# ocean1100/stereo_match

Hardware: AMD Instinct MI355X
Metric: stereo pairs/sec + Mpix·disp/sec, KITTI 1242×375 D=128 SGM, 1/2/4/8 GPU (higher is better)
Workload: dtype u8

## Files before the change

stereo_match_amd/csrc/sm_api.hip:

```cpp
#include <hip/hip_runtime.h>

#include <algorithm>
#include <cmath>
#include <cstdarg>
#include <cstdio>
#include <cstring>
#include <string>
#include <thread>
#include <type_traits>
#include <vector>

#include "../../include/stereo_match_amd.h"
#include "sm_cost.hpp"
#include "sm_paths.hpp"
#include "sm_post.hpp"
#include "sm_wls.hpp"
#include "sm_speckle.hpp"
#include "sm_reproject.hpp"
#include "sm_rectify.hpp"
#include "sm_nlm.hpp"
#include "sm_cloud.hpp"
#include "sm_bm.hpp"
#include "sm_wide.hpp"
#include "sm_sweep_host.hpp"
// ... 311 lines not shown
        return SM_OK;
    }
    int finish()
    {
        HIP_TRY(ctx, hipStreamSynchronize(ctx->stream));
        for (const Out& o : outs) std::memcpy(o.dst, (const uint8_t*)ctx->pin + o.off, o.bytes);
        return SM_OK;
    }
};
inline size_t stage_bytes(size_t bytes, int n = 1) { return (size_t)n * ((bytes + 255) & ~size_t(255)); }

int grid_for(size_t n)
{
    size_t g = (n + 255) / 256;
    return (int)std::min<size_t>(std::max<size_t>(g, 1), 8192);
}

size_t elem_bytes(const Norm& n) { return n.cost == SM_COST_CENSUS ? 1 : 2; }

const int kVdx[6] = {1, 0, -1, 1, 0, -1};
enum { DIRS_ALL = 0, DIRS_EW = 1, DIRS_EW_UP = 2 };
const int kVdy[6] = {1, 1, 1, -1, -1, -1};

constexpr size_t kRowLds = 65536;
constexpr size_t kSetBudget = size_t(32) << 30;
constexpr int kMaxGroup = 16;
bool sweep_fit_variant(sm_ctx* ctx, const Norm& n, int mode, int variant, struct SweepFit& f);
int sweep_min_pairs(sm_ctx* ctx, const Norm& n);
constexpr size_t kMallBudget = size_t(224) << 20;
constexpr int kMallMinPairs = 3;

struct Src {
    const uint8_t* L = nullptr;
    const uint8_t* R = nullptr;
    size_t pair_stride = 0;
    const float* vol = nullptr;
    size_t vol_pair = 0;
    float offset = 0.f, scale = 1.f;
    Src advance(int i) const
    {
        Src s = *this;
        if (L) s.L += (size_t)i * pair_stride;
        if (R) s.R += (size_t)i * pair_stride;
        if (vol) s.vol += (size_t)i * vol_pair;
        return s;
    }
};

int hybrid_slots(const Norm& n);

struct Geo {
    int H, W, stride, G;
    size_t vol, slot_bytes, L_pair, census_pair, cost_pair;
    bool sweep;
    bool lines;
    bool hybrid;
};

bool row_mode(const sm_ctx* ctx, const Norm& n)
{
    return SM_ABLATIONS && (ctx->dbg_flags & DBG_ROW) && n.D % 64 == 0 && n.D == n.Dv;
}
bool overlap(const sm_ctx* ctx) { return (ctx->dbg_flags & DBG_OVERLAP) != 0; }
bool use_cost8(const sm_ctx* ctx, const Norm& n)
{
    return n.cost == SM_COST_CENSUS && !(ctx->dbg_flags & DBG_NO_C8) && n.D <= 256;
}
hipStream_t stream_b(const sm_ctx* ctx)
{
    return ctx->wta_override ? ctx->wta_override : overlap(ctx) ? ctx->side : ctx->stream;
}

template <int DPLV, bool CENSUS, int VL, bool H16 = false>
int launch_paths_t(sm_ctx* ctx, const Norm& n, const Geo& g, BufSet& bs, int dirset)
{
    using LT = typename std::conditional<CENSUS, uint8_t, uint16_t>::type;
    constexpr int D = 16 * DPLV;
    constexpr bool WIDE = D % 64 == 0 && !H16;
    constexpr int LANESH = WIDE ? 64 : 16;
    constexpr int DPLH = D / LANESH;
    smk::PathsArgs pa{};
    pa.cl = (const uint64_t*)bs.census[0].p;
    pa.cr = (const uint64_t*)bs.census[1].p;
    pa.census_pair = g.census_pair;
    pa.cost = (const uint16_t*)bs.cost.p;
    pa.cost_pair = g.cost_pair;
    pa.cost8 = nullptr;
    if (use_cost8(ctx, n)) {
        pa.cost8 = (const uint8_t*)bs.cost.p;
        pa.cost_pair = g.vol;
    }
    pa.L = (uint8_t*)bs.L.p;
    pa.slot_bytes = g.slot_bytes;
    pa.L_pair_bytes = g.L_pair;
    pa.H = g.H;
    pa.W = g.W;
    pa.width1 = n.width1;
    pa.D = n.D;
    pa.minD = n.minD;
    pa.minX1 = n.minX1;
    pa.P1 = n.P1;
    pa.P2 = n.P2;
    pa.dbg = ctx->dbg_flags;
    const int lines_per_wg = 4 * (64 / LANESH);
    pa.hblocks = row_mode(ctx, n) ? 0 : (g.H + lines_per_wg - 1) / lines_per_wg;
    pa.nv = dirset == DIRS_ALL ? n.ndirs - 2 : dirset == DIRS_EW ? 0 : 3;
    const int k0 = dirset == DIRS_EW_UP ? 3 : 0;
    int blocks = 0;
    constexpr int LPWV = 64 / VL;
    for (int k = 0; k < pa.nv; k++) {
        const int dx = kVdx[k0 + k];
        pa.v_dx[k] = dx;
        pa.v_dy[k] = kVdy[k0 + k];
        pa.v_slot[k] = 2 + k;
        pa.v_line_lo[k] = dx > 0 ? -(g.H - 1) : 0;
        pa.v_nlines[k] = dx == 0 ? n.width1 : n.width1 + g.H - 1;
        pa.v_blk_start[k] = blocks;
        blocks += ((pa.v_nlines[k] + 8 * LPWV - 1) / (8 * LPWV)) * 2;
    }
    for (int k = pa.nv; k <= 6; k++) pa.v_blk_start[k] = blocks;
    dim3 grid(2 * pa.hblocks + blocks, g.G);
    if (ctx->fb_guard) {
        pa.guard = ctx->fb_guard;
        pa.nblocks = (int)grid.x;
        pa.npairs = g.G;
        grid = dim3(std::min<unsigned>(grid.x * g.G, 128u), 1);
    }
    StageTimer t(ctx, ctx->stream,
                 ctx->fb_guard ? SM_STAGE_FALLBACK : dirset == DIRS_EW ? SM_STAGE_HORIZONTAL : SM_STAGE_PATHS, g.G);
    if (ctx->fb_guard)
        hipLaunchKernelGGL((smk::k_sgm_paths<VL, DPLV * 16 / VL, LANESH, DPLH, CENSUS, LT, true>), grid, dim3(256), 0,
                           ctx->stream, pa);
    else
        hipLaunchKernelGGL((smk::k_sgm_paths<VL, DPLV * 16 / VL, LANESH, DPLH, CENSUS, LT>), grid, dim3(256), 0,
                           ctx->stream, pa);
    HIP_TRY(ctx, hipGetLastError());
    return SM_OK;
}

#ifndef WTA_NT
#define WTA_NT 1024
#endif
template <int DPLV, bool CENSUS>
int launch_wta_t(sm_ctx* ctx, const Norm& n, const Geo& g, BufSet& bs)
{
    using LT = typename std::conditional<CENSUS, uint8_t, uint16_t>::type;
    StageTimer t(ctx, stream_b(ctx), ctx->fb_guard ? SM_STAGE_FALLBACK : SM_STAGE_WTA, g.G);
#if SM_ABLATIONS
    constexpr int D = 16 * DPLV;
    if constexpr (D % 64 == 0) {
        if (row_mode(ctx, n) && !ctx->fb_guard) {
            if (ctx->wta_dst) return fail(ctx, SM_E_UNSUPPORTED, "the row-WTA ablation has no WTA-index output");
            smk::RowArgs ra{};
            ra.cl = (const uint64_t*)bs.census[0].p;
            ra.cr = (const uint64_t*)bs.census[1].p;
            ra.census_pair = g.census_pair;
            ra.cost = (const uint16_t*)bs.cost.p;
            ra.cost_pair = g.cost_pair;
            ra.L = (uint8_t*)bs.L.p;
            ra.slot_bytes = g.slot_bytes;
            ra.L_pair_bytes = g.L_pair;
            ra.H = g.H;
            ra.W = g.W;
            ra.width1 = n.width1;
            ra.D = n.D;
            ra.minD = n.minD;
            ra.minX1 = n.minX1;
            ra.P1 = n.P1;
            ra.P2 = n.P2;
            ra.uniq = n.uniq;
            ra.disp12 = n.disp12;
            ra.store_w = (ctx->dbg_flags & DBG_STORE_W) ? 1 : 0;
            ra.disp = (int16_t*)bs.raw.p;
            const size_t smem = (1024 + (size_t)g.W * 6 + 15) & ~size_t(15);
            if (n.ndirs == 8)
                hipLaunchKernelGGL((smk::k_row_wta<D / 64, 8, CENSUS, LT>), dim3(g.H, g.G), dim3(64), smem, stream_b(ctx), ra);
            else
                hipLaunchKernelGGL((smk::k_row_wta<D / 64, 5, CENSUS, LT>), dim3(g.H, g.G), dim3(64), smem, stream_b(ctx), ra);
            HIP_TRY(ctx, hipGetLastError());
            return SM_OK;
        }
    }
#endif
    smk::WtaArgs wa{};
    wa.L = (const uint8_t*)bs.L.p;
    wa.slot_bytes = g.slot_bytes;
    wa.L_pair_bytes = g.L_pair;
    const bool part_only = g.lines && !ctx->fb_guard;
    wa.nslots = part_only ? 0 : g.hybrid ? hybrid_slots(n) : n.ndirs;
    wa.part = (g.hybrid || part_only) ? (const uint16_t*)bs.part.p : nullptr;
    wa.part_pair = g.vol;
    wa.H = g.H;
    wa.W = g.W;
    wa.width1 = n.width1;
    wa.D = n.D;
    wa.Dv = n.Dv;
    wa.minD = n.minD;
    wa.minX1 = n.minX1;
    wa.uniq = n.uniq;
    wa.disp12 = n.disp12;
    wa.disp = (int16_t*)bs.raw.p;
    wa.wta = ctx->wta_dst;
    wa.lane8 = n.ndirs == 5;
    wa.skip = ctx->fb_guard ? nullptr : ctx->wta_skip;
    dim3 grid(g.H, g.G);
    const size_t smem = (size_t)g.W * (ctx->wta_dst ? 10 : 8) + 16;
    if (smem > kRowLds)
        return fail(ctx, SM_E_UNSUPPORTED, "width %d: the WTA row kernel's %zu B of LDS exceed %zu%s", g.W, smem,
                    kRowLds, ctx->wta_dst ? " (with the WTA index output)" : "");
    if (ctx->fb_guard) {
        wa.guard = ctx->fb_guard;
        wa.fallbacks = (uint32_t*)ctx->sweep_err.p + ERR_FALLBACKS;
        wa.npairs = g.G;
        grid = dim3(std::min(g.H * g.G, 64), 1);
    }
    if (ctx->fb_guard)
        hipLaunchKernelGGL((smk::k_wta<DPLV, LT, 1024, true>), grid, dim3(1024), smem, stream_b(ctx), wa);
    else if (wa.nslots == 0 && wa.part)
        hipLaunchKernelGGL((smk::k_wta<DPLV, LT, WTA_NT, false, DPLV % 2 == 0>), grid, dim3(WTA_NT), smem, stream_b(ctx),
                           wa);
    else
        hipLaunchKernelGGL((smk::k_wta<DPLV, LT, WTA_NT>), grid, dim3(WTA_NT), smem, stream_b(ctx), wa);
    HIP_TRY(ctx, hipGetLastError());
    return SM_OK;
}

template <int DPLV, bool CENSUS>
int launch_paths_dpl(sm_ctx* ctx, const Norm& n, const Geo& g, BufSet& bs, int dirset)
{
    if constexpr ((16 * DPLV) % 64 == 0) {
        if (ctx->dbg_flags & DBG_H64) {
            if (DPLV == 8 && !(ctx->dbg_flags & DBG_VL16))
                return launch_paths_t<DPLV, CENSUS, 8>(ctx, n, g, bs, dirset);
            return launch_paths_t<DPLV, CENSUS, 16>(ctx, n, g, bs, dirset);
        }
    }
    if constexpr (DPLV == 8) {
        if (!(ctx->dbg_flags & DBG_VL16)) return launch_paths_t<DPLV, CENSUS, 8, true>(ctx, n, g, bs, dirset);
    }
    return launch_paths_t<DPLV, CENSUS, 16, true>(ctx, n, g, bs, dirset);
}

enum { DISPATCH_PATHS = 0, DISPATCH_WTA = 1, DISPATCH_HORIZONTAL = 2, DISPATCH_HYBRID = 3 };

int dispatch(sm_ctx* ctx, const Norm& n, const Geo& g, BufSet& bs, int what)
{
    const bool census = n.cost == SM_COST_CENSUS;
    const int h = what == DISPATCH_HORIZONTAL ? DIRS_EW : what == DISPATCH_HYBRID ? DIRS_EW_UP : DIRS_ALL;
    switch (n.dpl) {
#define CASE(k)                                                                                               \
    case k:                                                                                                   \
        if (what == DISPATCH_WTA)                                                                             \
            return census ? launch_wta_t<k, true>(ctx, n, g, bs) : launch_wta_t<k, false>(ctx, n, g, bs);     \
        return census ? launch_paths_dpl<k, true>(ctx, n, g, bs, h) : launch_paths_dpl<k, false>(ctx, n, g, bs, h);
        CASE(1) CASE(2) CASE(3) CASE(4) CASE(5) CASE(6) CASE(7) CASE(8)
        CASE(9) CASE(10) CASE(11) CASE(12) CASE(13) CASE(14) CASE(15) CASE(16)
#undef CASE
    default: return fail(ctx, SM_E_UNSUPPORTED, "numDisparities %d not built", n.D);
    }
}

int ensure_event(sm_ctx* ctx, hipEvent_t& e);
bool use_sweep(const sm_ctx* ctx, const Norm& n, int H);

int hybrid_slots(const Norm& n) { return n.ndirs == 8 ? 5 : 2; }

bool use_hybrid(const sm_ctx* ctx, const Norm& n, int H)
{
    if (!SM_ABLATIONS || (n.ndirs != 8 && n.ndirs != 5) || !(ctx->dbg_flags & DBG_HYBRID) ||
        (ctx->dbg_flags & (DBG_LEGACY | DBG_SWEEP8)))
        return false;
    sm_ctx tmp = *ctx;
    tmp.dbg_flags = (ctx->dbg_flags & ~DBG_HYBRID) | DBG_SWEEP8;
    return use_sweep(&tmp, n, H);
}

bool use_sweep(const sm_ctx* ctx, const Norm& n, int H)
{
    if (ctx->dbg_flags & (DBG_LEGACY | DBG_ROW)) return false;
    if (n.cost == SM_COST_CENSUS && !use_cost8(ctx, n)) return false;
    const int cmax = n.cost == SM_COST_CENSUS ? 64 : n.cost == SM_COST_VOLUME ? smk::VOL_CMAX : 0;
    if (cmax + n.P2 > 16383) return false;
    if (H > 65535 || n.width1 <= 0) return false;
    const size_t W = (size_t)(n.maxX1 - std::min(n.minD, 0));
    if (W * 6 + 16 > kRowLds) return false;
    return (uint64_t)H * n.width1 * n.D * 2 <= smk::kMaxRecords;
}

struct SweepJob {
    const uint8_t* cost;
    size_t cost_pair;
    const uint8_t* ew;
    size_t ew_pair, ew_slot;
    uint16_t* part;
    size_t part_pair;
    uint32_t* key2;
    uint32_t* pre;
    uint32_t* err;
    int G;
    uint8_t* st = nullptr;
    size_t st_pair = 0;
    int ewarm = 0;
    int ewguess = 0;
    int nband = 1, band_h = 0, vwarm = 0, vguess = 0;
    uint8_t* vst = nullptr;
    size_t vst_pair = 0;
};

int stream_cus(hipStream_t st, int ncu)
{
    uint32_t mask[32] = {0};
    const uint32_t words = (uint32_t)std::min(32, (ncu + 31) / 32);
    if (hipExtStreamGetCUMask(st, words, mask) != hipSuccess) return ncu;
    int c = 0;
    for (uint32_t i = 0; i < words; i++) c += __builtin_popcount(mask[i]);
    return c > 0 ? std::min(c, ncu) : ncu;
}

int ensure_sweep_err(sm_ctx* ctx)
{
    if (ctx->sweep_err.p) return SM_OK;
    int rc = ensure(ctx, ctx->sweep_err, SWEEP_STATS ? (size_t(8) << 20) : 256);
    if (rc != SM_OK) return rc;
    HIP_TRY(ctx, hipMemsetAsync(ctx->sweep_err.p, 0, SWEEP_STATS ? (size_t(8) << 20) : 256, ctx->stream));
    return SM_OK;
}

int sweep_variant(const sm_ctx* ctx)
{
    if (SM_ABLATIONS && (ctx->dbg_flags & DBG_SWEEP_V2)) return 6;
    if (SM_ABLATIONS && (ctx->dbg_flags & DBG_SWEEP2_NW)) return 3;
    return (ctx->dbg_flags & DBG_NARROW_SWEEPS) ? 1 : 0;
}

struct SweepFit {
    smk::SweepInfo si{};
    int nwg = 0, cap = 0, ncu = 0;
};
bool sweep_fit_variant(sm_ctx* ctx, const Norm& n, int mode, int variant, SweepFit& f)
{
    if (smk::sweep_info(n.D, (int)elem_bytes(n), mode, variant, ctx->device, &f.si) != hipSuccess) return false;
    int ncu = 0;
    if (hipDeviceGetAttribute(&ncu, hipDeviceAttributeMultiprocessorCount, ctx->device) != hipSuccess) return false;
    f.ncu = stream_cus(ctx->stream, std::max(ncu, 1));
    const int per_cu = f.si.blocks_per_cu >= 3 ? f.si.blocks_per_cu - 1 : std::max(f.si.blocks_per_cu, 1);
    f.cap = per_cu * f.ncu;
    f.nwg = (n.width1 + f.si.cw - 1) / f.si.cw;
    return f.nwg <= f.cap;
}

int sweep_min_pairs(sm_ctx* ctx, const Norm& n)
{
    if (n.cost != SM_COST_CENSUS) return 3;
    SweepFit f;
    if (!sweep_fit_variant(ctx, n, 2, 0, f) || f.nwg <= 0) return 7;
    return std::max(2, std::min(7, (200 + f.nwg - 1) / f.nwg));
}

double sweep_model(const SweepFit& f, int G)
{
    const int per_launch = std::max(1, std::min(G, f.cap / std::max(f.nwg, 1)));
    const int launches = (G + per_launch - 1) / per_launch;
    const int per_cu = (per_launch * f.nwg + f.ncu - 1) / std::max(f.ncu, 1);
    return (double)launches * per_cu * (f.si.threads / 64 - 1) * std::max(f.si.dpl, 1);
}

bool sweep_capacity(sm_ctx* ctx, const Norm& n, int mode, int G, SweepFit& f)
{
    if (ctx->tune_sweep_ncw && sweep_variant(ctx) <= 1) {
        for (int v : {0, 1, 2}) {
            SweepFit t;
            if (sweep_fit_variant(ctx, n, mode, v, t) && t.si.ncw == ctx->tune_sweep_ncw) {
                f = t;
                return true;
            }
        }
        return false;
    }
    const int variant = sweep_variant(ctx);
    if (!sweep_fit_variant(ctx, n, mode, variant, f)) {
        if (!(variant == 0 && f.si.impl == 1 && sweep_fit_variant(ctx, n, mode, 1, f))) return false;
    } else if (variant == 0 && f.si.impl == 1 && G > 0 && !(ctx->dbg_flags & DBG_WIDE_SWEEPS)) {
        SweepFit nf;
        if (sweep_fit_variant(ctx, n, mode, 1, nf) && sweep_model(nf, G) < sweep_model(f, G)) f = nf;
    }
    if (variant == 0 && G > 0 && !(ctx->dbg_flags & DBG_WIDE_SWEEPS)) {
        SweepFit lf;
        if (sweep_fit_variant(ctx, n, mode, 2, lf) && sweep_model(lf, G) < sweep_model(f, G)) f = lf;
    }
    return true;
}

bool sweeps_fit(sm_ctx* ctx, const Norm& n, bool hybrid, bool lines = false)
{
    const int m8[2] = {0, 2}, m5[1] = {1}, mh[1] = {0}, l8[2] = {3, 4}, l5[1] = {3};
    const int* modes = hybrid ? mh : lines ? (n.ndirs == 8 ? l8 : l5) : n.ndirs == 8 ? m8 : m5;
    const int count = !hybrid && n.ndirs == 8 ? 2 : 1;
    for (int k = 0; k < count; k++) {
        SweepFit f;
        if (!sweep_capacity(ctx, n, modes[k], 0, f)) return false;
        if (lines && modes[k] == 3 && f.nwg > smk::patch_max_strips(n.D)) return false;
        if (lines && modes[k] == 3 && f.si.ncw < 11) return false;
    }
    return true;
}

int sweep_pass(sm_ctx* ctx, const Norm& n, const Geo& g, const SweepJob& j, int mode)
{
    SweepFit f;
    const bool banded = j.nband > 1;
    if (banded ? !(sweep_fit_variant(ctx, n, mode, 0, f) && f.si.impl == 1) : !sweep_capacity(ctx, n, mode, j.G, f)) {
        if (f.nwg > f.cap)
            return fail(ctx, SM_E_UNSUPPORTED, "sweep: %d strips exceed %d resident workgroups", f.nwg, f.cap);
        return fail(ctx, SM_E_UNSUPPORTED, "sweep: numDisparities %d not built", n.D);
    }
    const smk::SweepInfo& si = f.si;
    const int nwg = f.nwg, cap = f.cap;
    const int nb = banded ? j.nband : 1;
    const int nblk = banded ? (j.band_h + j.vwarm + si.hb - 1) / si.hb : (g.H + si.hb - 1) / si.hb;
    const int per_launch = (ctx->dbg_flags & DBG_SWEEP1) ? 1 : std::max(1, std::min(j.G, cap / (nwg * nb)));
    const size_t hop_pair = (size_t)nwg * nb * 2 * nblk * si.ngr;
    const size_t hop_bytes = hop_pair * 8 * per_launch;
    if (hop_pair * 8 > smk::kMaxRecords) return fail(ctx, SM_E_UNSUPPORTED, "sweep: boundary buffer too large");
    int rc;
    if (ctx->hop.n < hop_bytes || !ctx->hop.p) {
        if ((rc = ensure(ctx, ctx->hop, hop_bytes)) != SM_OK) return rc;
        HIP_TRY(ctx, hipMemsetAsync(ctx->hop.p, 0, ctx->hop.n, ctx->stream));
        ctx->hop_epoch = 0;
    }
    if ((rc = ensure_sweep_err(ctx)) != SM_OK) return rc;
    for (int p0 = 0; p0 < j.G; p0 += per_launch) {
        const int np = std::min(per_launch, j.G - p0);
        if (++ctx->hop_epoch > 0xFFFFu) {
            HIP_TRY(ctx, hipMemsetAsync(ctx->hop.p, 0, ctx->hop.n, ctx->stream));
            ctx->hop_epoch = 1;
        }
        smk::SweepArgs a{};
        a.cost = j.cost + (size_t)p0 * j.cost_pair;
        a.cost_pair = j.cost_pair;
        a.ew = j.ew ? j.ew + (size_t)p0 * j.ew_pair : nullptr;
        a.ew_pair = j.ew_pair;
        a.ew_slot = j.ew_slot;
        a.part = j.part ? (uint16_t*)((uint8_t*)j.part + (size_t)p0 * j.part_pair) : nullptr;
        a.part_pair = j.part_pair;
        a.hop = (unsigned long long*)ctx->hop.p;
        a.hop_pair = hop_pair;
        a.st = j.st ? j.st + (size_t)p0 * j.st_pair : nullptr;
        a.st_pair = j.st_pair;
        a.ewarm = j.ewarm;
        a.ewguess = j.ewguess;
        a.nband = nb;
        a.band_h = j.band_h;
        a.vwarm = j.vwarm;
        a.vguess = j.vguess;
        a.hop_nblk = nblk;
        a.vst = j.vst ? j.vst + (size_t)p0 * j.vst_pair : nullptr;
        a.vst_pair = j.vst_pair;
        if (ctx->tune_sweep_xcd > 0) {
            a.xcd_total = np * nwg * nb;
            a.xcd_per = (a.xcd_total + 7) / 8;
        }
        a.rec = j.key2 ? j.key2 + (size_t)p0 * g.H * g.W : nullptr;
        a.nb = j.pre ? j.pre + (size_t)p0 * g.H * g.W : nullptr;
        a.err = j.err;
        a.H = g.H;
        a.W = g.W;
        a.W1 = n.width1;
        a.D = n.D;
        a.Dv = n.Dv;
        a.minD = n.minD;
        a.minX1 = n.minX1;
        a.P1 = n.P1;
        a.P2 = n.P2;
        a.uniq = n.uniq;
        a.inv_ku = n.uniq < 100 ? 1.0f / (float)(100 - n.uniq) : 0.f;
        a.nwg = nwg;
        a.epoch = ctx->hop_epoch;
#if SWEEP_STATS
        a.stats = (unsigned long long*)((char*)ctx->sweep_err.p + 1024);
#endif
        a.dbg = (ctx->dbg_flags >> 24) & 7;
        HIP_TRY(ctx, smk::sweep_launch(n.D, (int)elem_bytes(n), mode, si.impl, a, np, ctx->stream));
    }
    return SM_OK;
}

struct StreamSwap {
    sm_ctx* c;
    hipStream_t old;
    StreamSwap(sm_ctx* c_, hipStream_t s) : c(c_), old(c_->stream) { c->stream = s; }
    ~StreamSwap() { c->stream = old; }
};

int ew_lanes(const sm_ctx* ctx, const Norm& n)
{
    if (ctx->tune_ew_lanes) return ctx->tune_ew_lanes;
    if (ctx->dbg_flags & DBG_OLD_EW) return -1;
    if (n.D % 64 == 0) return 32;
    if (n.D % 32 == 0) return 16;
    return elem_bytes(n) == 1 ? 0 : -1;
}

int launch_ew(sm_ctx* ctx, const Norm& n, const Geo& g, BufSet& bs)
{
    const size_t et = elem_bytes(n);
    const int vl = ew_lanes(ctx, n);
    if (vl < 0) return dispatch(ctx, n, g, bs, DISPATCH_HORIZONTAL);
    smk::EwArgs a{};
    a.cost = (const uint8_t*)bs.cost.p;
    a.cost_pair = g.vol * et;
    a.out = (uint8_t*)bs.L.p;
    a.out_pair = g.L_pair;
    a.out_slot = g.slot_bytes;
    a.H = g.H;
    a.W1 = n.width1;
    a.P1 = n.P1;
    a.P2 = n.P2;
    a.wpb = ctx->tune_ew_waves;
    a.prio = ctx->tune_ew_prio;
    StageTimer t(ctx, ctx->stream, SM_STAGE_HORIZONTAL, g.G);
    const hipError_t e = smk::ew_launch(n.D, (int)et, vl, a, g.G, ctx->stream);
    if (e == hipErrorInvalidValue) return fail(ctx, SM_E_UNSUPPORTED, "E/W lines: numDisparities %d not built", n.D);
    HIP_TRY(ctx, e);
    return SM_OK;
}

int run_sweep(sm_ctx* ctx, const Norm& n, const Geo& g, BufSet& bs, hipStream_t wta_stream, uint32_t* err)
{
    const int G = g.G;
    int rc;
    const size_t et = elem_bytes(n);
    SweepJob j{};
    j.cost = (const uint8_t*)bs.cost.p;
    j.cost_pair = g.vol * et;
    j.ew = (const uint8_t*)bs.L.p;
    j.ew_pair = g.L_pair;
    j.ew_slot = g.slot_bytes;
    j.G = G;
    if ((rc = ensure(ctx, bs.key2, (size_t)G * g.H * g.W * 4)) != SM_OK) return rc;
    if ((rc = ensure(ctx, bs.pre, (size_t)G * g.H * g.W * 4)) != SM_OK) return rc;
    j.key2 = (uint32_t*)bs.key2.p;
    j.pre = (uint32_t*)bs.pre.p;
    j.err = err;
    {
        StageTimer t(ctx, ctx->stream, SM_STAGE_PATHS, G);
        if (n.ndirs == 8) {
            if ((rc = ensure_event(ctx, ctx->ev_fork)) != SM_OK) return rc;
            if ((rc = ensure_event(ctx, ctx->ev_join)) != SM_OK) return rc;
            HIP_TRY(ctx, hipEventRecord(ctx->ev_fork, ctx->stream));
            if ((rc = ensure(ctx, bs.part, (size_t)G * g.vol * 2)) != SM_OK) return rc;
            j.part = (uint16_t*)bs.part.p;
            j.part_pair = g.vol * 2;
            {
                StageTimer ts(ctx, ctx->stream, SM_STAGE_SWEEP, G);
                if ((rc = sweep_pass(ctx, n, g, j, 0)) != SM_OK) return rc;
            }
            HIP_TRY(ctx, hipStreamWaitEvent(ctx->side, ctx->ev_fork, 0));
            const hipStream_t main = ctx->stream;
            ctx->stream = ctx->side;
            rc = launch_ew(ctx, n, g, bs);
            ctx->stream = main;
            if (rc != SM_OK) return rc;
            HIP_TRY(ctx, hipEventRecord(ctx->ev_join, ctx->side));
            HIP_TRY(ctx, hipStreamWaitEvent(ctx->stream, ctx->ev_join, 0));
        } else if ((rc = launch_ew(ctx, n, g, bs)) != SM_OK) {
            return rc;
        }
    }
    if (wta_stream != ctx->stream) {
        HIP_TRY(ctx, hipEventRecord(bs.paths_done, ctx->stream));
        HIP_TRY(ctx, hipStreamWaitEvent(wta_stream, bs.paths_done, 0));
    }
    StreamSwap sw(ctx, wta_stream);
    StageTimer t(ctx, ctx->stream, SM_STAGE_WTA, G);
    StageTimer ts(ctx, ctx->stream, SM_STAGE_SWEEP_WTA, G);
    return sweep_pass(ctx, n, g, j, n.ndirs == 8 ? 2 : 1);
}

int sweep_finish(sm_ctx* ctx, const Norm& n, const Geo& g, BufSet& bs, hipStream_t ws, uint32_t* gflag)
{
    const bool fb = !(ctx->dbg_flags & DBG_NO_FALLBACK);
    int rc;
    if (fb && ws != ctx->stream) {
        if (ctx->dbg_flags & DBG_FORCE_FALLBACK) HIP_TRY(ctx, hipMemsetAsync(gflag, 1, 1, ws));
        HIP_TRY(ctx, smk::lr_rows_launch((const uint32_t*)bs.key2.p, (const uint32_t*)bs.pre.p, (int16_t*)bs.raw.p,
                                         ctx->wta_dst, g.G, g.H, g.W, n.Dv, n.minD, n.minX1, n.maxX1, n.disp12,
                                         gflag, ws));
        StreamSwap sw(ctx, ws);
        ctx->wta_override = ws;
        ctx->fb_guard = gflag;
        rc = dispatch(ctx, n, g, bs, DISPATCH_PATHS);
        if (rc == SM_OK) rc = dispatch(ctx, n, g, bs, DISPATCH_WTA);
        ctx->fb_guard = nullptr;
        ctx->wta_override = nullptr;
        return rc;
    }
    hipStream_t fs = ctx->side;
    if (fb) {
        if (ctx->dbg_flags & DBG_FORCE_FALLBACK) HIP_TRY(ctx, hipMemsetAsync(gflag, 1, 1, ws));
        if ((rc = ensure_event(ctx, ctx->ev_fb_fork)) != SM_OK) return rc;
        if ((rc = ensure_event(ctx, ctx->ev_fb_join)) != SM_OK) return rc;
        HIP_TRY(ctx, hipEventRecord(ctx->ev_fb_fork, ws));
        HIP_TRY(ctx, hipStreamWaitEvent(fs, ctx->ev_fb_fork, 0));
        StreamSwap sw(ctx, fs);
        ctx->wta_override = fs;
        ctx->fb_guard = gflag;
        rc = dispatch(ctx, n, g, bs, DISPATCH_PATHS);
        if (rc == SM_OK) rc = dispatch(ctx, n, g, bs, DISPATCH_WTA);
        ctx->fb_guard = nullptr;
        ctx->wta_override = nullptr;
        if (rc != SM_OK) return rc;
        HIP_TRY(ctx, hipEventRecord(ctx->ev_fb_join, fs));
    }
    HIP_TRY(ctx, smk::lr_rows_launch((const uint32_t*)bs.key2.p, (const uint32_t*)bs.pre.p, (int16_t*)bs.raw.p,
                                     ctx->wta_dst, g.G, g.H, g.W, n.Dv, n.minD, n.minX1, n.maxX1, n.disp12,
                                     fb ? gflag : nullptr, ws));
    if (fb) HIP_TRY(ctx, hipStreamWaitEvent(ws, ctx->ev_fb_join, 0));
    return SM_OK;
}

bool use_lines(sm_ctx* ctx, const Norm& n)
{
    if (ctx->tune_sweep_lines < 0 || ctx->tune_ew_lanes || (ctx->dbg_flags & DBG_OLD_EW)) return false;
    return sweeps_fit(ctx, n, false, true);
}

int ew_warmup(const sm_ctx* ctx, const Norm& n)
{
    if (ctx->tune_ew_warmup > 0) return ctx->tune_ew_warmup;
    (void)n;
    return 16;
}

long long path_max(const Norm& n)
{
    if (n.cost == SM_COST_CENSUS) return 62 + n.P2;
    if (n.cost == SM_COST_VOLUME) return smk::VOL_CMAX + n.P2;
    const long long side = 2 * (n.bs / 2) + 1;
    return side * side * (2 * n.ftzero + (255 >> 2)) + n.P2;
}

int line_bands(const sm_ctx* ctx, const Norm& n, int H, int G)
{
    if (n.ndirs != 5 || ctx->tune_bands == 1 || 5 * path_max(n) > 65535) return 1;
    SweepFit f;
    if (!sweep_fit_variant(const_cast<sm_ctx*>(ctx), n, 3, 0, f) || f.si.impl != 1 || f.nwg <= 0) return 1;
    int nb = ctx->tune_bands >= 2 ? ctx->tune_bands : std::min(f.cap / std::max(1, G * f.nwg), H / 24);
    nb = std::min(nb, H);
    if (nb < 2) return 1;
    const int bh = (H + nb - 1) / nb;
    return (H + bh - 1) / bh;
}

int band_warmup(const sm_ctx* ctx, const Norm& n)
{
    if (ctx->tune_band_warmup > 0) return ctx->tune_band_warmup;
    return elem_bytes(n) == 1 ? 16 : 24;
}

int run_lines(sm_ctx* ctx, const Norm& n, const Geo& g, BufSet& bs, hipStream_t ws, uint32_t* gflag)
{
    const int G = g.G;
    const size_t et = elem_bytes(n);
    int rc;
    SweepJob j{};
    j.cost = (const uint8_t*)bs.cost.p;
    j.cost_pair = g.vol * et;
    j.G = G;
    j.err = gflag;
    if ((rc = ensure(ctx, bs.part, (size_t)G * g.vol * 2)) != SM_OK) return rc;
    j.part = (uint16_t*)bs.part.p;
    j.part_pair = g.vol * 2;
    SweepFit f;
    j.nband = line_bands(ctx, n, g.H, G);
    if (j.nband > 1 ? !sweep_fit_variant(ctx, n, 3, 0, f) : !sweep_capacity(ctx, n, 3, G, f))
        return fail(ctx, SM_E_UNSUPPORTED, "sweep lines: no instance fits");
    j.st_pair = ((size_t)g.H * f.nwg * 4 * n.D * et + 255) & ~size_t(255);
    if ((rc = ensure(ctx, bs.st, j.st_pair * G)) != SM_OK) return rc;
    j.st = (uint8_t*)bs.st.p;
    j.ewarm = ew_warmup(ctx, n);
    j.ewguess = ctx->tune_ew_guess;
    if (j.nband > 1 && ctx->tune_ew_warmup <= 0 && et == 2) j.ewarm = 54;
    if (j.nband > 1) {
        j.band_h = (g.H + j.nband - 1) / j.nband;
        j.vwarm = band_warmup(ctx, n);
        j.vguess = ctx->tune_band_guess;
        j.vst_pair = ((size_t)j.nband * 6 * n.width1 * n.D * et + 255) & ~size_t(255);
        if ((rc = ensure(ctx, bs.vst, j.vst_pair * G)) != SM_OK) return rc;
        j.vst = (uint8_t*)bs.vst.p;
        ctx->band_groups++;
    }
    ctx->line_groups++;
    ctx->line_strips += (long long)f.nwg * G;
    const bool fb_side = n.ndirs == 5 && ws == ctx->stream && !(ctx->dbg_flags & DBG_NO_FALLBACK);
    {
        StageTimer t(ctx, ctx->stream, SM_STAGE_PATHS, G);
        {
            StageTimer ts(ctx, ctx->stream, SM_STAGE_SWEEP, G);
            if ((rc = sweep_pass(ctx, n, g, j, 3)) != SM_OK) return rc;
        }
        if (ctx->sweep_done_ev) {
            HIP_TRY(ctx, hipEventRecord(ctx->sweep_done_ev, ctx->stream));
            ctx->sweep_done_hit = true;
        }
        smk::EwPatchArgs pa{};
        pa.cost = j.cost;
        pa.cost_pair = j.cost_pair;
        pa.part = j.part;
        pa.part_pair = j.part_pair * 1;
        pa.st = j.st;
        pa.st_pair = j.st_pair;
        pa.H = g.H;
        pa.W1 = n.width1;
        pa.nwg = f.nwg;
        pa.cw = f.si.cw;
        pa.P1 = n.P1;
        pa.P2 = n.P2;
        pa.guard = gflag;
        pa.fixes = reinterpret_cast<unsigned long long*>((uint32_t*)ctx->sweep_err.p + ERR_EW_REPAIRS);
        pa.atom = EW_PATCH_ATOM && et == 2 && 5 * path_max(n) < 65536 ? 1 : 0;
        auto ew_patch = [&](hipStream_t st) -> int {
            const hipError_t e = smk::ew_patch_launch(n.D, (int)et, pa, G, st);
            if (e == hipErrorInvalidValue) return fail(ctx, SM_E_UNSUPPORTED, "E/W patch: numDisparities %d not built", n.D);
            HIP_TRY(ctx, e);
            return SM_OK;
        };
        const bool ew_side = fb_side && pa.atom && j.nband > 1;
        if (fb_side) {
            if (ctx->dbg_flags & DBG_FORCE_FALLBACK) HIP_TRY(ctx, hipMemsetAsync(gflag, 1, 1, ctx->stream));
            if ((rc = ensure_event(ctx, ctx->ev_fb_fork)) != SM_OK) return rc;
            if ((rc = ensure_event(ctx, ctx->ev_fb_join)) != SM_OK) return rc;
            HIP_TRY(ctx, hipEventRecord(ctx->ev_fb_fork, ctx->stream));
            HIP_TRY(ctx, hipStreamWaitEvent(ctx->side, ctx->ev_fb_fork, 0));
            if (ew_side) {
                if ((rc = ensure_event(ctx, ctx->ev_ew_done)) != SM_OK) return rc;
                {
                    StageTimer th(ctx, ctx->side, SM_STAGE_HORIZONTAL, G);
                    if ((rc = ew_patch(ctx->side)) != SM_OK) return rc;
                }
                HIP_TRY(ctx, hipEventRecord(ctx->ev_ew_done, ctx->side));
            }
            StreamSwap sw(ctx, ctx->side);
            ctx->wta_override = ctx->side;
            ctx->fb_guard = gflag;
            rc = dispatch(ctx, n, g, bs, DISPATCH_PATHS);
            if (rc == SM_OK) rc = dispatch(ctx, n, g, bs, DISPATCH_WTA);
            ctx->fb_guard = nullptr;
            ctx->wta_override = nullptr;
            if (rc != SM_OK) return rc;
            HIP_TRY(ctx, hipEventRecord(ctx->ev_fb_join, ctx->side));
        }
        if (!ew_side) {
            StageTimer th(ctx, ctx->stream, SM_STAGE_HORIZONTAL, G);
            if ((rc = ew_patch(ctx->stream)) != SM_OK) return rc;
        }
        if (j.nband > 1) {
            smk::BandPatchArgs ba{};
            ba.cost = j.cost;
            ba.cost_pair = j.cost_pair;
            ba.part = j.part;
            ba.part_pair = j.part_pair;
            ba.vst = j.vst;
            ba.vst_pair = j.vst_pair;

            ba.H = g.H;
            ba.W1 = n.width1;
            ba.nband = j.nband;
            ba.band_h = j.band_h;
            ba.P1 = n.P1;
            ba.P2 = n.P2;
            ba.guard = gflag;
            ba.fixes = reinterpret_cast<unsigned long long*>((uint32_t*)ctx->sweep_err.p + ERR_BAND_REPAIRS);
            const hipError_t eb = smk::band_patch_launch(n.D, (int)et, ba, G, ctx->stream);
            if (eb == hipErrorInvalidValue) return fail(ctx, SM_E_UNSUPPORTED, "band patch: numDisparities %d not built", n.D);
            HIP_TRY(ctx, eb);
            if (ew_side) HIP_TRY(ctx, hipStreamWaitEvent(ctx->stream, ctx->ev_ew_done, 0));
        }
    }
    if (ws != ctx->stream) {
        HIP_TRY(ctx, hipEventRecord(bs.paths_done, ctx->stream));
        HIP_TRY(ctx, hipStreamWaitEvent(ws, bs.paths_done, 0));
    }
    if (n.ndirs == 8) {
        if ((rc = ensure(ctx, bs.key2, (size_t)G * g.H * g.W * 4)) != SM_OK) return rc;
        if ((rc = ensure(ctx, bs.pre, (size_t)G * g.H * g.W * 4)) != SM_OK) return rc;
        j.key2 = (uint32_t*)bs.key2.p;
        j.pre = (uint32_t*)bs.pre.p;
        {
            StreamSwap sw(ctx, ws);
            StageTimer t(ctx, ctx->stream, SM_STAGE_WTA, G);
            StageTimer ts(ctx, ctx->stream, SM_STAGE_SWEEP_WTA, G);
            if ((rc = sweep_pass(ctx, n, g, j, 4)) != SM_OK) return rc;
        }
        return sweep_finish(ctx, n, g, bs, ws, gflag);
    }
    StreamSwap sw(ctx, ws);
    ctx->wta_override = ws;
    {
        StageTimer ts(ctx, ws, SM_STAGE_SWEEP_WTA, G);
        ctx->wta_skip = fb_side ? gflag : nullptr;
        rc = dispatch(ctx, n, g, bs, DISPATCH_WTA);
        ctx->wta_skip = nullptr;
    }
    if (fb_side) {
        if (rc == SM_OK) HIP_TRY(ctx, hipStreamWaitEvent(ws, ctx->ev_fb_join, 0));
    } else if (rc == SM_OK && !(ctx->dbg_flags & DBG_NO_FALLBACK)) {
        if (ctx->dbg_flags & DBG_FORCE_FALLBACK) HIP_TRY(ctx, hipMemsetAsync(gflag, 1, 1, ws));
        ctx->fb_guard = gflag;
        rc = dispatch(ctx, n, g, bs, DISPATCH_PATHS);
        if (rc == SM_OK) rc = dispatch(ctx, n, g, bs, DISPATCH_WTA);
        ctx->fb_guard = nullptr;
    }
    ctx->wta_override = nullptr;
    return rc;
}

int run_hybrid(sm_ctx* ctx, const Norm& n, const Geo& g, BufSet& bs)
{
    const int G = g.G;
    int rc;
    SweepJob j{};
    j.cost = (const uint8_t*)bs.cost.p;
    j.cost_pair = g.vol * elem_bytes(n);
    j.G = G;
    if ((rc = ensure_sweep_err(ctx)) != SM_OK) return rc;
    j.err = (uint32_t*)ctx->sweep_err.p + ERR_STICKY;
    if ((rc = ensure(ctx, bs.part, (size_t)G * g.vol * 2)) != SM_OK) return rc;
    j.part = (uint16_t*)bs.part.p;
    j.part_pair = g.vol * 2;
    if ((rc = ensure_event(ctx, ctx->ev_fork)) != SM_OK) return rc;
    if ((rc = ensure_event(ctx, ctx->ev_join)) != SM_OK) return rc;
    StageTimer t(ctx, ctx->stream, SM_STAGE_PATHS, G);
    HIP_TRY(ctx, hipEventRecord(ctx->ev_fork, ctx->stream));
    HIP_TRY(ctx, hipStreamWaitEvent(ctx->side, ctx->ev_fork, 0));
    const hipStream_t main = ctx->stream;
    ctx->stream = ctx->side;
    {
        StageTimer ts(ctx, ctx->stream, SM_STAGE_SWEEP, G);
        rc = sweep_pass(ctx, n, g, j, 0);
    }
    ctx->stream = main;
    if (rc != SM_OK) return rc;
    HIP_TRY(ctx, hipEventRecord(ctx->ev_join, ctx->side));
    if ((rc = dispatch(ctx, n, g, bs, n.ndirs == 8 ? DISPATCH_HYBRID : DISPATCH_HORIZONTAL)) != SM_OK) return rc;
    HIP_TRY(ctx, hipStreamWaitEvent(ctx->stream, ctx->ev_join, 0));
    return SM_OK;
}

int check_sweep_errors(sm_ctx* ctx)
{
    if (ctx->twin) {
        int rc = check_sweep_errors(ctx->twin);
        if (rc != SM_OK) return fail(ctx, rc, "%s", ctx->twin->err.c_str());
    }
    if (!ctx->sweep_err.p) return SM_OK;
    uint32_t e = 0;
    uint32_t* w = (uint32_t*)ctx->sweep_err.p + ERR_STICKY;
    HIP_TRY(ctx, hipMemcpy(&e, w, 4, hipMemcpyDeviceToHost));
    if (e) {
        HIP_TRY(ctx, hipMemset(w, 0, 4));
        return fail(ctx, SM_E_HIP, "sweep: strip-boundary hand-off timed out (workgroups not co-resident?)");
    }
    return SM_OK;
}

int cost_nt(const Geo& g, size_t elem_bytes)
{
    return (size_t)g.G * g.vol * elem_bytes > ((size_t)224 << 20) ? 1 : 0;
}

#ifndef SGBM_COST2_WGS
#define SGBM_COST2_WGS 2048
#endif
template <int S, int CPT>
int launch_cost2_s(sm_ctx* ctx, const Norm& n, const Geo& g, const smk::SgbmCostArgs& sc)
{
    const int NP = n.D / 2, CG = std::max(1, 256 / NP), bd = NP * CG, TX = CG * CPT, NHC = TX + 2 * S;
    const int rpairs = TX + 2 * S + n.D - 1;
    if (NP > 256 || NHC > 4 * bd || rpairs > 4 * bd)
        return fail(ctx, SM_E_UNSUPPORTED, "sgbm cost: numDisparities %d not built", n.D);
    const bool one = NHC <= bd && rpairs <= bd;
    const int rph = (rpairs + 1) / 2;
    const size_t lds = (size_t)NHC * 16 + (size_t)((NHC + 1) & ~1) * 8 + (size_t)2 * rph * 24 + (size_t)2 * ((CG * ((NHC + CG - 1) / CG)) | 1) * NP * 4;
    smk::SgbmCost2Args c2{};
    c2.planes = sc.planes;
    c2.C = sc.C;
    c2.C_pair = sc.C_pair;
    c2.H = sc.H;
    c2.W = sc.W;
    c2.width1 = sc.width1;
    c2.D = sc.D;
    c2.minD = sc.minD;
    c2.minX1 = sc.minX1;
    c2.Yc = sc.Yc;
    c2.nt = cost_nt(g, 2);
    const int strips = (n.width1 + TX - 1) / TX;
    const int wgs = ctx->tune_cost_wgs > 0 ? ctx->tune_cost_wgs : SGBM_COST2_WGS;
    const int want = std::max(1, wgs / std::max(1, strips * g.G));
    c2.band = std::max({(sc.Yc + want - 1) / want, 8, 4 * S});
    const int bands = (sc.Yc + c2.band - 1) / c2.band;
    if (one)
        hipLaunchKernelGGL((smk::k_sgbm_cost2<S, CPT, 1>), dim3(strips, bands, g.G), dim3(bd), lds, ctx->stream, c2);
    else
        hipLaunchKernelGGL((smk::k_sgbm_cost2<S, CPT, 4>), dim3(strips, bands, g.G), dim3(bd), lds, ctx->stream, c2);
    HIP_TRY(ctx, hipGetLastError());
    return SM_OK;
}

int launch_sgbm_cost2(sm_ctx* ctx, const Norm& n, const Geo& g, const smk::SgbmCostArgs& sc)
{
    if (ctx->dbg_flags & DBG_COST_TILE) return SM_OK;
    switch (n.bs / 2) {
    case 0: return launch_cost2_s<0, 8>(ctx, n, g, sc);
    case 1: return launch_cost2_s<1, 8>(ctx, n, g, sc);
    case 2: return launch_cost2_s<2, 8>(ctx, n, g, sc);
    case 3: return launch_cost2_s<3, 8>(ctx, n, g, sc);
    case 4: return launch_cost2_s<4, 8>(ctx, n, g, sc);
    case 5: return launch_cost2_s<5, 8>(ctx, n, g, sc);
    default: return fail(ctx, SM_E_UNSUPPORTED, "blockSize %d not built", n.bs);
    }
}

int group_size(const sm_ctx* ctx, const Norm& n, int H, int npairs, bool sweep, bool hybrid)
{
    const size_t cells = (size_t)H * std::max(n.width1, 1) * n.D;
    const size_t per = sweep    ? cells * (n.ndirs * elem_bytes(n) + (n.ndirs == 8 ? 2 : 0))
                       : hybrid ? cells * (hybrid_slots(n) * elem_bytes(n) + 2)
                                : cells * elem_bytes(n) * n.ndirs;
    size_t g = std::max<size_t>(1, kSetBudget / std::max<size_t>(per, 1));
    const size_t half = overlap(ctx) ? std::max(1, (npairs + 1) / 2) : kMaxGroup;
    const int cap = (ctx->dbg_flags >> 16) & 7;
    if (cap) return (int)std::min<size_t>({g, (size_t)cap, half});
    g = std::min<size_t>({g, (size_t)kMaxGroup, half});
    if (!sweep && !hybrid && elem_bytes(n) == 1 && !(ctx->dbg_flags & DBG_NO_MALL_GROUPS)) {
        const size_t fit = kMallBudget / std::max<size_t>(cells, 1);
        const size_t ngroups = fit ? ((size_t)npairs + fit - 1) / fit : 0;
        if (fit >= (size_t)kMallMinPairs && fit < g && ngroups <= 2)
            g = std::max<size_t>(1, ((size_t)npairs + ngroups - 1) / ngroups);
    }
    return (int)g;
}

int ensure_event(sm_ctx* ctx, hipEvent_t& e)
{
    if (!e) HIP_TRY(ctx, hipEventCreateWithFlags(&e, hipEventDisableTiming));
    return SM_OK;
}

int run_speckles(sm_ctx* ctx, hipStream_t st, int16_t* img, int G, int H, int W, int newval, int maxsize,
                 int maxdiff)
{
    StageTimer t(ctx, st, SM_STAGE_SPECKLE, G);
    const size_t npx = (size_t)H * W;
    int rc;
    if ((rc = ensure(ctx, ctx->sp_parent, G * npx * 4)) != SM_OK) return rc;
    if ((rc = ensure(ctx, ctx->sp_count, G * npx * 4)) != SM_OK) return rc;
    smk::SpeckleArgs sa{};
    sa.img = img;
    sa.parent = (int*)ctx->sp_parent.p;
    sa.count = (int*)ctx->sp_count.p;
    sa.H = H;
    sa.W = W;
    sa.newval = newval;
    sa.maxsize = maxsize;
    sa.maxdiff = maxdiff;
    const dim3 grid((unsigned)((npx + 255) / 256), G);
    hipLaunchKernelGGL(smk::k_speckle_init, grid, dim3(256), 0, st, sa);
    hipLaunchKernelGGL(smk::k_speckle_union, grid, dim3(256), 0, st, sa);
    hipLaunchKernelGGL(smk::k_speckle_count, grid, dim3(256), 0, st, sa);
    hipLaunchKernelGGL(smk::k_speckle_apply, grid, dim3(256), 0, st, sa);
    HIP_TRY(ctx, hipGetLastError());
    return SM_OK;
}

int finish_group(sm_ctx* ctx, const Geo& g, const Norm& n, BufSet& bs, int s, int16_t* d_out, hipStream_t sb)
{
    const int H = g.H, W = g.W, G = g.G;
    int rc;
    {
        StageTimer t(ctx, sb, SM_STAGE_MEDIAN, G);
        hipLaunchKernelGGL(smk::k_median3, dim3((W + 255) / 256, H, G), dim3(256), 0, sb,
                           (const int16_t*)bs.raw.p, d_out, H, W, (size_t)H * W);
        HIP_TRY(ctx, hipGetLastError());
    }
    if (n.speckle_ws > 0) {
        if ((rc = run_speckles(ctx, sb, d_out, G, H, W, (n.minD - 1) * 16, n.speckle_ws, 16 * n.speckle_range)) !=
            SM_OK)
            return rc;
    }
    if (sb != ctx->stream) {
        HIP_TRY(ctx, hipEventRecord(bs.wta_done, sb));
        bs.pending = true;
    }
    ctx->last_width1 = n.width1;
    ctx->last_index = G - 1;
    ctx->last_L_pair = g.L_pair;
    ctx->last_set = s;
    return SM_OK;
}

template <int DPL>
int wide_paths_wta(sm_ctx* ctx, const Geo& g, const Norm& n, BufSet& bs)
{
    smk::WidePathArgs pa{};
    pa.C = (const int16_t*)bs.cost.p;
    pa.vol = g.vol;
    pa.L = (uint8_t*)bs.L.p;
    pa.slot_bytes = g.slot_bytes;
    pa.L_pair_bytes = g.L_pair;
    pa.H = g.H;
    pa.width1 = n.width1;
    pa.D = n.D;
    pa.P1 = n.P1;
    pa.P2 = n.P2;
    pa.ndirs = n.ndirs;
    const int dys[8] = {0, 0, 1, 1, 1, -1, -1, -1}, dxs[8] = {1, -1, 1, 0, -1, 1, 0, -1};
    int blocks = 0;
    for (int k = 0; k < n.ndirs; k++) {
        pa.blk_start[k] = blocks;
        const int nl = dys[k] == 0 ? g.H : dxs[k] == 0 ? n.width1 : n.width1 + g.H - 1;
        blocks += (nl + 15) / 16;
    }
    for (int k = n.ndirs; k <= 8; k++) pa.blk_start[k] = blocks;
// ... 2383 lines not shown
```

stereo_match_amd/csrc/sm_ew.hpp:

```cpp
#pragma once
#include "sm_pk.hpp"
#include "sm_sweep_host.hpp"

namespace smk {

#ifndef SWEEP_STREAM_AUX
#define SWEEP_STREAM_AUX 2
#endif
#ifndef EW_H16
#define EW_H16 1
#endif
#ifndef EW_STEPN
#define EW_STEPN 1
#endif

template <int VL, int NP, typename CT, typename LT, int PF>
__global__ void __launch_bounds__(256) k_ew(EwArgs a)
{
    constexpr int LPW = 64 / VL, DPL = 2 * NP, D = VL * DPL;
    constexpr int CB = DPL * (int)sizeof(CT);
    switch (a.prio) {
    case 1: __builtin_amdgcn_s_setprio(1); break;
    case 2: __builtin_amdgcn_s_setprio(2); break;
    case 3: __builtin_amdgcn_s_setprio(3); break;
    default: break;
    }
    const int lane = threadIdx.x & 63, wave = threadIdx.x >> 6;
    const int g = lane % VL, kl = lane / VL;
    const int dir = (int)blockIdx.x >= a.nrb ? 1 : 0;
    const int H = a.H, W1 = a.W1;
    const int y0 = (((int)blockIdx.x - dir * a.nrb) * a.wpb + wave) * LPW;
    if (y0 >= H) return;
    const bool line_ok = y0 + kl < H;
    const int y = min(y0 + kl, H - 1);
    const size_t pair = blockIdx.y;
    const uint64_t cells = (uint64_t)H * W1 * D;
    const rsrc_t rc = make_rsrc(a.cost + pair * a.cost_pair, cells * sizeof(CT));
    const rsrc_t ro = make_rsrc(a.out + pair * a.out_pair + (size_t)dir * a.out_slot, cells * sizeof(LT));
    const uint32_t estep = dir ? (uint32_t)(-D) : (uint32_t)D;
    uint32_t e = ((uint32_t)y * (uint32_t)W1 + (uint32_t)(dir ? W1 - 1 : 0)) * (uint32_t)D + (uint32_t)(g * DPL);
    const uint32_t P1p = (uint32_t)a.P1 * 0x10001u, P2p = (uint32_t)a.P2 * 0x10001u;
    constexpr bool H16 = sizeof(CT) == 1 && EW_H16;
    constexpr uint32_t EDGE = H16 ? 0x7BFF7BFFu : (kBig | (kBig << 16));
    const uint32_t eL = g == 0 ? EDGE : 0u, eR = g == VL - 1 ? EDGE : 0u;

    RawBytes<CB> ring[PF];
#pragma unroll
    for (int k = 0; k < PF; k++) {
        ring[k].load(rc, k < W1 ? (e + (uint32_t)k * estep) * (uint32_t)sizeof(CT) : kOOB);
        asm volatile("" ::: "memory");
    }
    uint32_t Lp[NP];
#pragma unroll
    for (int k = 0; k < NP; k++) Lp[k] = 0;
    uint32_t minLp = 0;
    for (int s0 = 0; s0 < W1; s0 += PF) {
#pragma unroll
        for (int k = 0; k < PF; k++) {
            const int s = s0 + k;
#pragma unroll
            for (int j = 0; j < RawBytes<CB>::WORDS; j++) asm volatile("" : "+v"(ring[k].w[j]) : "v"(minLp));
            uint32_t C[NP];
            unpack_ct_pk<CT, DPL>(ring[k], C);
#pragma unroll
            for (int i = 0; i < NP; i++) asm volatile("" : "+v"(C[i])::"memory");
            ring[k].load(rc, s + PF < W1 ? (e + (uint32_t)PF * estep) * (uint32_t)sizeof(CT) : kOOB);
            uint32_t Ln[NP], mn;
            if constexpr (EW_STEPN) {
                uint32_t Lp1[1][NP], m1[1] = {minLp}, C1[1][NP], Ln1[1][NP], mn1[1];
#pragma unroll
                for (int i = 0; i < NP; i++) {
                    Lp1[0][i] = Lp[i];
                    C1[0][i] = C[i];
                }
                sweep_step2n<VL, NP, H16, 1>(Lp1, m1, C1, P1p, P2p, eL, eR, Ln1, mn1);
#pragma unroll
                for (int i = 0; i < NP; i++) Ln[i] = Ln1[0][i];
                mn = mn1[0];
            } else {
                mn = sweep_step2<VL, NP, H16>(Lp, minLp, C, P1p, P2p, eL, eR, Ln);
            }
            store_pk<LT, NP, SWEEP_STREAM_AUX>(ro, (line_ok && s < W1) ? e * (uint32_t)sizeof(LT) : kOOB, Ln);
            e += estep;
#pragma unroll
            for (int i = 0; i < NP; i++) Lp[i] = Ln[i];
            minLp = mn;
        }
    }
}

#ifndef EW_PATCH_NO_CARRY
#define EW_PATCH_NO_CARRY 0
#endif
#ifndef EW_PATCH_B64
#define EW_PATCH_B64 1
#endif
#ifndef EW_PATCH_RC
#define EW_PATCH_RC 0
#endif
template <int VL, int NP, typename CT, bool ATOM = false>
__global__ void __launch_bounds__(256) k_ew_patch(EwPatchArgs a)
{
    constexpr int LPW = 64 / VL, DPL = 2 * NP, D = VL * DPL;
    constexpr int CB = DPL * (int)sizeof(CT);
    constexpr bool H16 = sizeof(CT) == 1 && EW_H16;
    constexpr bool SAT = sizeof(CT) == 2;
    constexpr uint32_t EDGE = H16 ? 0x7BFF7BFFu : (kBig | (kBig << 16));
    constexpr int KU = 8;
    constexpr int CHUNK = LPW * KU;
    constexpr int RC = EW_PATCH_RC ? EW_PATCH_RC : sizeof(CT) == 1 ? 8 : 16;
    if (a.guard && __hip_atomic_load(a.guard, __ATOMIC_RELAXED, __HIP_MEMORY_SCOPE_AGENT) != 0u) return;
    const int lane = threadIdx.x & 63, wave = threadIdx.x >> 6;
    const int g = lane % VL, kl = lane / VL;
    const int yw = (int)blockIdx.x * 4 + wave;
    const int y = ATOM ? yw >> 1 : yw;
    const int dir0 = ATOM ? (yw & 1) : 0, dir1 = ATOM ? dir0 + 1 : 2;
    const size_t pair = blockIdx.y;
    const int H = a.H, W1 = a.W1, nwg = a.nwg, CW = a.cw;
    if (y >= H) return;
    const uint64_t cells = (uint64_t)H * W1 * D;
    const rsrc_t rc = make_rsrc(a.cost + pair * a.cost_pair, cells * sizeof(CT));
    const rsrc_t rp = make_rsrc((const uint8_t*)a.part + pair * a.part_pair, cells * 2);
    uint32_t* const pw = reinterpret_cast<uint32_t*>((uint8_t*)a.part + pair * a.part_pair);
    auto atom_add = [&](uint32_t word, uint32_t first, uint32_t second) {
        const int lo = (int)(second & 0xFFFFu) - (int)(first & 0xFFFFu);
        const int hi = (int)(second >> 16) - (int)(first >> 16);
        const uint32_t add = (uint32_t)(hi * 65536 + lo);
        if (add) __hip_atomic_fetch_add(pw + word, add, __ATOMIC_RELAXED, __HIP_MEMORY_SCOPE_AGENT);
    };
    const rsrc_t rs = make_rsrc(a.st + pair * a.st_pair, a.st_pair);
    const uint32_t P1p = (uint32_t)a.P1 * 0x10001u, P2p = (uint32_t)a.P2 * 0x10001u;
    const uint32_t eL = g == 0 ? EDGE : 0u, eR = g == VL - 1 ? EDGE : 0u;
    auto soff = [&](int k, int dir, int which) -> uint32_t {
        return (((((uint32_t)y * (uint32_t)nwg + (uint32_t)k) * 2u + (uint32_t)dir) * 2u + (uint32_t)which) *
                    (uint32_t)D + (uint32_t)(g * DPL)) * (uint32_t)sizeof(CT);
    };
    auto cell = [&](int c) -> uint32_t { return ((uint32_t)y * (uint32_t)W1 + (uint32_t)c) * (uint32_t)D + (uint32_t)(g * DPL); };
    auto line_all = [&](bool ok) -> bool { return group_min<VL>(ok ? 1u : 0u) != 0u; };
    auto same_state = [&](const uint32_t (&x)[NP], const uint32_t (&z)[NP]) -> bool {
        bool ok = true;
#pragma unroll
        for (int i = 0; i < NP; i++) ok &= x[i] == z[i];
        return line_all(ok);
    };
    auto state_min = [&](const uint32_t (&x)[NP]) -> uint32_t {
        uint32_t m = x[0];
#pragma unroll
        for (int i = 1; i < NP; i++) m = pk_min(m, x[i]);
        m = ::min(m & 0xFFFFu, m >> 16);
        return group_min<VL>(m) * 0x10001u;
    };
    auto load_state = [&](uint32_t off, uint32_t (&v)[NP]) {
        RawBytes<CB> b;
        b.load(rs, off);
        unpack_ct_pk<CT, DPL>(b, v);
    };
    auto walk = [&](int k, int dir, uint32_t aoff, uint32_t toff, uint32_t (&T)[NP], bool check) -> int {
        const int x0 = k * CW, ncol = ::min(CW, W1 - x0);
        RawBytes<CB> cc[RC];
        RawBytes<DPL * 2> pb[RC];
        auto issue1 = [&](int u, int o) {
            const int c = dir ? x0 + CW - 1 - o : x0 + o;
            cc[u].load(rc, o < ncol ? cell(c) * (uint32_t)sizeof(CT) : kOOB);
            if constexpr (!ATOM) pb[u].load(rp, o < ncol ? cell(c) * 2u : kOOB);
        };
        auto issue = [&](int o0) {
#pragma unroll
            for (int u = 0; u < RC; u++) issue1(u, o0 + u);
        };
        issue(0);
        uint32_t A[NP];
        load_state(aoff, A);
        if (toff != kOOB) load_state(toff, T);
        if (check && same_state(A, T)) return 2;
        uint32_t Lq[2][NP], mq[2];
#pragma unroll
        for (int q = 0; q < NP; q++) {
            Lq[0][q] = A[q];
            Lq[1][q] = T[q];
        }
        mq[0] = state_min(Lq[0]);
        mq[1] = state_min(Lq[1]);
        bool met = false;
        for (int o0 = 0; o0 < ncol && !met; o0 += RC) {
            if (o0 > 0) issue(o0);
#pragma unroll
            for (int u = 0; u < RC; u++) {
                const int o = o0 + u;
                if (o >= ncol || met) continue;
                const int c = dir ? x0 + CW - 1 - o : x0 + o;
                uint32_t C2[2][NP], Ln[2][NP], mn[2], pv_[NP];
                unpack_ct_pk<CT, DPL>(cc[u], C2[0]);
#pragma unroll
                for (int q = 0; q < NP; q++) pv_[q] = ATOM ? 0u : pb[u].w[q];
#pragma unroll
                for (int q = 0; q < NP; q++) C2[1][q] = C2[0][q];
                sweep_step2n<VL, NP, H16, 2>(Lq, mq, C2, P1p, P2p, eL, eR, Ln, mn);
                if (same_state(Ln[0], Ln[1])) {
                    met = true;
                    continue;
                }
                if constexpr (ATOM) {
#pragma unroll
                    for (int q = 0; q < NP; q++) atom_add(cell(c) / 2u + (uint32_t)q, Ln[0][q], Ln[1][q]);
                }
                uint32_t P[NP];
#pragma unroll
                for (int q = 0; q < NP && !ATOM; q++) {
                    if constexpr (SAT) {
                        const uint32_t pv = pv_[q];
                        const uint32_t x = pk_adds(pk_sub(pv, Ln[0][q]), Ln[1][q]);
                        const uint32_t sat = pk_sub(pk_min(pk_add(pv, 0x00010001u), 0x00010001u), 0x00010001u);
                        P[q] = pkw(__builtin_elementwise_max(pkv(x), pkv(sat)));
                    } else {
                        P[q] = pk_add(pk_sub(pv_[q], Ln[0][q]), Ln[1][q]);
                    }
                }
                if constexpr (!ATOM) bstore_n<uint32_t, NP>(rp, cell(c) * 2u, P);
#pragma unroll
                for (int q = 0; q < NP; q++) {
                    Lq[0][q] = Ln[0][q];
                    Lq[1][q] = Ln[1][q];
                }
                mq[0] = mn[0];
                mq[1] = mn[1];
            }
        }
        if (!met) {
#pragma unroll
            for (int q = 0; q < NP; q++) T[q] = pk_sub(Lq[1][q], mq[1]);
        }
        return met ? 1 : 0;
    };
    constexpr int DPLW = D % 128 == 0 ? D / 64 : 2, NPW = DPLW / 2;
    constexpr int CBW = DPLW * (int)sizeof(CT);
    auto soff64 = [&](int k, int dir, int which) -> uint32_t {
        return (((((uint32_t)y * (uint32_t)nwg + (uint32_t)k) * 2u + (uint32_t)dir) * 2u + (uint32_t)which) *
                    (uint32_t)D + (uint32_t)(lane * DPLW)) * (uint32_t)sizeof(CT);
    };
    auto cell64 = [&](int c) -> uint32_t {
        return ((uint32_t)y * (uint32_t)W1 + (uint32_t)c) * (uint32_t)D + (uint32_t)(lane * DPLW);
    };
    auto load_state64 = [&](uint32_t off, uint32_t (&v)[NPW]) {
        RawBytes<CBW> b;
        b.load(rs, off);
        unpack_ct_pk<CT, DPLW>(b, v);
    };
    auto same_state64 = [&](const uint32_t (&x)[NPW], const uint32_t (&z)[NPW]) -> bool {
        bool ok = true;
#pragma unroll
        for (int i = 0; i < NPW; i++) ok &= x[i] == z[i];
        return __all(ok);
    };
    auto state_min64 = [&](const uint32_t (&x)[NPW]) -> uint32_t {
        uint32_t m = x[0];
#pragma unroll
        for (int i = 1; i < NPW; i++) m = pk_min(m, x[i]);
        m = ::min(m & 0xFFFFu, m >> 16);
        return Line<64>::min(m) * 0x10001u;
    };
    auto walk64 = [&](int k, int dir, uint32_t aoff, uint32_t toff, uint32_t (&T)[NPW], bool check) -> int {
        const int x0 = k * CW, ncol = ::min(CW, W1 - x0);
        RawBytes<CBW> cc[RC];
        RawBytes<DPLW * 2> pb[RC];
        auto issue1 = [&](int u, int o) {
            const int c = dir ? x0 + CW - 1 - o : x0 + o;
            cc[u].load(rc, o < ncol ? cell64(c) * (uint32_t)sizeof(CT) : kOOB);
            if constexpr (!ATOM) pb[u].load(rp, o < ncol ? cell64(c) * 2u : kOOB);
        };
        auto issue = [&](int o0) {
#pragma unroll
            for (int u = 0; u < RC; u++) issue1(u, o0 + u);
        };
        issue(0);
        uint32_t A[NPW];
        load_state64(aoff, A);
        if (toff != kOOB) load_state64(toff, T);
        if (check && same_state64(A, T)) return 2;
        uint32_t Lq[2][NPW], mq[2];
#pragma unroll
        for (int q = 0; q < NPW; q++) {
            Lq[0][q] = A[q];
            Lq[1][q] = T[q];
        }
        mq[0] = state_min64(Lq[0]);
        mq[1] = state_min64(Lq[1]);
        bool met = false;
        for (int o0 = 0; o0 < ncol && !met; o0 += RC) {
            if (o0 > 0) issue(o0);
#pragma unroll
            for (int u = 0; u < RC; u++) {
                const int o = o0 + u;
                if (o >= ncol || met) continue;
                const int c = dir ? x0 + CW - 1 - o : x0 + o;
                uint32_t C2[2][NPW], Ln[2][NPW], mn[2], pv_[NPW];
                unpack_ct_pk<CT, DPLW>(cc[u], C2[0]);
#pragma unroll
                for (int q = 0; q < NPW; q++) pv_[q] = ATOM ? 0u : pb[u].w[q];
#pragma unroll
                for (int q = 0; q < NPW; q++) C2[1][q] = C2[0][q];
                sweep_step2n<64, NPW, H16, 2>(Lq, mq, C2, P1p, P2p, 0u, 0u, Ln, mn);
                if (same_state64(Ln[0], Ln[1])) {
                    met = true;
                    continue;
                }
                if constexpr (ATOM) {
#pragma unroll
                    for (int q = 0; q < NPW; q++) atom_add(cell64(c) / 2u + (uint32_t)q, Ln[0][q], Ln[1][q]);
                }
                uint32_t P[NPW];
#pragma unroll
                for (int q = 0; q < NPW && !ATOM; q++) {
                    if constexpr (SAT) {
                        const uint32_t pv = pv_[q];
                        const uint32_t x = pk_adds(pk_sub(pv, Ln[0][q]), Ln[1][q]);
                        const uint32_t sat = pk_sub(pk_min(pk_add(pv, 0x00010001u), 0x00010001u), 0x00010001u);
                        P[q] = pkw(__builtin_elementwise_max(pkv(x), pkv(sat)));
                    } else {
                        P[q] = pk_add(pk_sub(pv_[q], Ln[0][q]), Ln[1][q]);
                    }
                }
                if constexpr (!ATOM) bstore_n<uint32_t, NPW>(rp, cell64(c) * 2u, P);
#pragma unroll
                for (int q = 0; q < NPW; q++) {
                    Lq[0][q] = Ln[0][q];
                    Lq[1][q] = Ln[1][q];
                }
                mq[0] = mn[0];
                mq[1] = mn[1];
            }
        }
        if (!met) {
#pragma unroll
            for (int q = 0; q < NPW; q++) T[q] = pk_sub(Lq[1][q], mq[1]);
        }
        return met ? 1 : 0;
    };
    auto lines_or = [&](uint64_t v) -> uint64_t {
        uint64_t m = 0;
#pragma unroll
        for (int l = 0; l < LPW; l++) {
            const uint32_t lo = __builtin_amdgcn_readlane((uint32_t)v, l * VL);
            const uint32_t hi = __builtin_amdgcn_readlane((uint32_t)(v >> 32), l * VL);
            m |= ((uint64_t)hi << 32) | lo;
        }
        return m;
    };
    auto order_partial = [&]() {
        __builtin_amdgcn_fence(__ATOMIC_RELEASE, "workgroup");
        __builtin_amdgcn_fence(__ATOMIC_ACQUIRE, "workgroup");
    };
    __shared__ uint64_t openm[4][kPatchMaxChunks];
    uint32_t nfix = 0, nopen = 0;
    for (int dir = dir0; dir < dir1; dir++) {
        auto strip_of = [&](int i) { return dir ? nwg - 1 - i : i; };
        int first_open = nwg;
        for (int i0 = 1, ch = 0; i0 < nwg; i0 += CHUNK, ch++) {
            RawBytes<CB> sb[KU], eb[KU];
#pragma unroll
            for (int u = 0; u < KU; u++) {
                const int i = i0 + kl + LPW * u;
                sb[u].load(rs, i < nwg ? soff(strip_of(i), dir, 0) : kOOB);
                eb[u].load(rs, i < nwg ? soff(strip_of(i - 1), dir, 1) : kOOB);
            }
            uint64_t bad = 0;
#pragma unroll
            for (int u = 0; u < KU; u++) {
                bool ok = true;
#pragma unroll
                for (int q = 0; q < RawBytes<CB>::WORDS; q++) ok &= sb[u].w[q] == eb[u].w[q];
                ok = line_all(ok);
                if (!ok && i0 + kl + LPW * u < nwg) bad |= 1ull << (kl + LPW * u);
            }
            const uint64_t m = lines_or(bad);
            uint64_t open = 0;
            uint64_t rest = m;
            while (rest) {
                int mine = -1;
#pragma unroll
                for (int l = 0; l < LPW; l++) {
                    if (rest && l == kl) mine = __builtin_ctzll(rest);
                    if (rest) rest &= rest - 1;
                }
                if (mine >= 0) {
                    const int i = i0 + mine, k = strip_of(i);
                    uint32_t T[NP];
                    nfix++;
                    if (walk(k, dir, soff(k, dir, 0), soff(strip_of(i - 1), dir, 1), T, false) == 0) {
                        store_pk<CT, NP>(rs, soff(k, dir, 0), T);
                        open |= 1ull << mine;
                    }
                }
            }
            open = lines_or(open);
            nopen += (uint32_t)__builtin_popcountll(open);
            if (lane == 0) openm[wave][ch] = open;
            if (open && first_open == nwg) first_open = i0 + __builtin_ctzll(open);
        }
        if (first_open < nwg && !EW_PATCH_NO_CARRY && D % 128 == 0 && EW_PATCH_B64) {
            order_partial();
            bool carry = false;
            uint32_t T[NPW];
#pragma unroll
            for (int q = 0; q < NPW; q++) T[q] = 0;
            for (int i = first_open; i < nwg; i++) {
                const int k = strip_of(i);
                if (carry) {
                    const int r = walk64(k, dir, soff64(strip_of(i - 1), dir, 1), kOOB, T, true);
                    nfix += r != 2 && kl == 0;
                    if (r != 0) carry = false;
                }
                const bool open_i = ((openm[wave][(i - 1) / CHUNK] >> ((i - 1) % CHUNK)) & 1ull) != 0;
                if (!carry && open_i) {
                    load_state64(soff64(k, dir, 0), T);
                    carry = true;
                }
            }
        } else if (first_open < nwg && !EW_PATCH_NO_CARRY) {
            order_partial();
            if (kl == 0) {
                bool carry = false;
                uint32_t T[NP];
#pragma unroll
                for (int q = 0; q < NP; q++) T[q] = 0;
                for (int i = first_open; i < nwg; i++) {
                    const int k = strip_of(i);
                    if (carry) {
                        const int r = walk(k, dir, soff(strip_of(i - 1), dir, 1), kOOB, T, true);
                        nfix += r != 2;
                        if (r != 0) carry = false;
                    }
                    const bool open_i = ((openm[wave][(i - 1) / CHUNK] >> ((i - 1) % CHUNK)) & 1ull) != 0;
                    if (!carry && open_i) {
                        load_state(soff(k, dir, 0), T);
                        carry = true;
                    }
                }
            }
        }
        if (!ATOM && dir == 0) order_partial();
    }
    if (a.fixes) {
        nfix = group_sum_u32_wave(g == 0 ? nfix : 0u);
        if (lane == 0 && nfix) atomicAdd(a.fixes, (unsigned long long)nfix);
        if (lane == 0 && nopen) atomicAdd(a.fixes + 1, (unsigned long long)nopen);
    }
}

template <int VL, int NP, typename CT>
__global__ void __launch_bounds__(256) k_band_patch(BandPatchArgs a)
{
    constexpr int LPW = 64 / VL, DPL = 2 * NP, D = VL * DPL, CB = DPL * (int)sizeof(CT);
    constexpr bool H16 = sizeof(CT) == 1 && EW_H16;
    constexpr uint32_t EDGE = H16 ? 0x7BFF7BFFu : (kBig | (kBig << 16));
    constexpr int RC = 8;
    if (a.guard && __hip_atomic_load(a.guard, __ATOMIC_RELAXED, __HIP_MEMORY_SCOPE_AGENT) != 0u) return;
    const int lane = threadIdx.x & 63, wave = threadIdx.x >> 6;
    const int g = lane % VL, kl = lane / VL;
    const int bi = (int)blockIdx.y + 1;
    const size_t pair = blockIdx.z;
    const int H = a.H, W1 = a.W1;
    const int y0 = bi * a.band_h;
    const int id = ((int)blockIdx.x * 4 + wave) * LPW + kl;
    const bool on = id < 3 * W1 && y0 < H;
    const int dir = on ? id / W1 : 0, x = on ? id % W1 : 0;
    const int dx = dir == 0 ? 0 : dir == 1 ? 1 : -1;
    const int nr = !on ? 0 : dx == 0 ? H - y0 : dx > 0 ? min(H - y0, W1 - 1 - x) : min(H - y0, x);
    const uint64_t cells = (uint64_t)H * W1 * D;
    const rsrc_t rc = make_rsrc(a.cost + pair * a.cost_pair, cells * sizeof(CT));
    const rsrc_t rv = make_rsrc(a.vst + pair * a.vst_pair, a.vst_pair);
    uint32_t* part = reinterpret_cast<uint32_t*>(reinterpret_cast<uint8_t*>(a.part) + pair * a.part_pair);
    const uint32_t P1p = (uint32_t)a.P1 * 0x10001u, P2p = (uint32_t)a.P2 * 0x10001u;
    const uint32_t eL = g == 0 ? EDGE : 0u, eR = g == VL - 1 ? EDGE : 0u;
    auto voff = [&](int band, int which, int col) -> uint32_t {
        return (((((uint32_t)band * 2u + (uint32_t)which) * 3u + (uint32_t)dir) * (uint32_t)W1 + (uint32_t)col) *
                    (uint32_t)D + (uint32_t)(g * DPL)) * (uint32_t)sizeof(CT);
    };
    auto cost_off = [&](int r) -> uint32_t {
        return r < nr ? (((uint32_t)(y0 + r) * (uint32_t)W1 + (uint32_t)(x + dx * (r + 1))) * (uint32_t)D +
                         (uint32_t)(g * DPL)) * (uint32_t)sizeof(CT)
                      : kOOB;
    };
    auto line_all = [&](bool ok) -> bool { return group_min<VL>(ok ? 1u : 0u) != 0u; };
    auto state_min = [&](const uint32_t (&v)[NP]) -> uint32_t {
        uint32_t m = v[0];
#pragma unroll
        for (int i = 1; i < NP; i++) m = pk_min(m, v[i]);
        m = ::min(m & 0xFFFFu, m >> 16);
        return group_min<VL>(m) * 0x10001u;
    };
    RawBytes<CB> sb, tb, cc[RC];
    sb.load(rv, on ? voff(bi, 0, x) : kOOB);
    tb.load(rv, on ? voff(bi - 1, 1, x) : kOOB);
#pragma unroll
    for (int u = 0; u < RC; u++) cc[u].load(rc, cost_off(u));
    uint32_t Lq[2][NP], mq[2];
    unpack_ct_pk<CT, DPL>(sb, Lq[0]);
    unpack_ct_pk<CT, DPL>(tb, Lq[1]);
    bool same = true;
#pragma unroll
    for (int i = 0; i < NP; i++) same &= Lq[0][i] == Lq[1][i];
    same = line_all(same);
    uint32_t nfix = 0, nlong = 0;
    if (on && !same && nr > 0) {
        nfix++;
        mq[0] = state_min(Lq[0]);
        mq[1] = state_min(Lq[1]);
        const int rb = min(H, y0 + a.band_h) - y0;
        bool met = false;
        int r0 = 0;
        for (; r0 < nr && !met; r0 += RC) {
            if (r0 > 0) {
#pragma unroll
                for (int u = 0; u < RC; u++) cc[u].load(rc, cost_off(r0 + u));
            }
#pragma unroll
            for (int u = 0; u < RC; u++) {
                const int r = r0 + u;
                if (r >= nr || met) continue;
                uint32_t C2[2][NP], Ln[2][NP], mn[2];
                unpack_ct_pk<CT, DPL>(cc[u], C2[0]);
#pragma unroll
                for (int q = 0; q < NP; q++) C2[1][q] = C2[0][q];
                sweep_step2n<VL, NP, H16, 2>(Lq, mq, C2, P1p, P2p, eL, eR, Ln, mn);
                bool eq = true;
#pragma unroll
                for (int q = 0; q < NP; q++) eq &= Ln[0][q] == Ln[1][q];
                if (line_all(eq)) {
                    met = true;
                    continue;
                }
                nlong |= r >= rb ? 1u : 0u;
                const size_t w0 = (((size_t)(y0 + r) * (size_t)W1 + (size_t)(x + dx * (r + 1))) * D + g * DPL) / 2;
#pragma unroll
                for (int q = 0; q < NP; q++) {
                    const int lo = (int)(Ln[1][q] & 0xFFFFu) - (int)(Ln[0][q] & 0xFFFFu);
                    const int hi = (int)(Ln[1][q] >> 16) - (int)(Ln[0][q] >> 16);
                    const uint32_t add = (uint32_t)(hi * 65536 + lo);
                    if (add) __hip_atomic_fetch_add(part + w0 + q, add, __ATOMIC_RELAXED, __HIP_MEMORY_SCOPE_AGENT);
                }
#pragma unroll
                for (int q = 0; q < NP; q++) {
                    Lq[0][q] = Ln[0][q];
                    Lq[1][q] = Ln[1][q];
                }
                mq[0] = mn[0];
                mq[1] = mn[1];
            }
        }
    }
    if (a.fixes) {
        nfix = group_sum_u32_wave(g == 0 ? nfix : 0u);
        nlong = group_sum_u32_wave(g == 0 ? nlong : 0u);
        if (lane == 0 && nfix) atomicAdd(a.fixes, (unsigned long long)nfix);
        if (lane == 0 && nlong) atomicAdd(a.fixes + 1, (unsigned long long)nlong);
    }
}

}
```

stereo_match_amd/csrc/sm_pk.hpp:

```cpp
#pragma once
#include "sm_common.hpp"

namespace smk {

template <int VL>
__device__ __forceinline__ uint32_t line_or(uint32_t v)
{
    v |= perm_dpp<DPP_QP_XOR1>(v);
    v |= perm_dpp<DPP_QP_XOR2>(v);
    v |= perm_dpp<DPP_ROW_HALF_MIRROR>(v);
    if constexpr (VL >= 16) v |= perm_dpp<DPP_ROW_MIRROR>(v);
    if constexpr (VL == 32) v = row_pair_combine(v, [](uint32_t a, uint32_t b) { return a | b; });
    return v;
}

template <int N>
__device__ __forceinline__ uint32_t group_min(uint32_t v)
{
    static_assert(N == 1 || N == 2 || N == 4 || N == 8 || N == 16 || N == 32, "lane group of 1-32 lanes");
    if constexpr (N >= 2) v = ::min(v, perm_dpp<DPP_QP_XOR1>(v));
    if constexpr (N >= 4) v = ::min(v, perm_dpp<DPP_QP_XOR2>(v));
    if constexpr (N >= 8) v = ::min(v, perm_dpp<DPP_ROW_HALF_MIRROR>(v));
    if constexpr (N >= 16) v = ::min(v, perm_dpp<DPP_ROW_MIRROR>(v));
    if constexpr (N >= 32) v = row_pair_combine(v, [](uint32_t a, uint32_t b) { return ::min(a, b); });
    return v;
}

template <int N>
__device__ __forceinline__ uint32_t group_sum(uint32_t v)
{
    static_assert(N == 1 || N == 2 || N == 4 || N == 8 || N == 16 || N == 32, "lane group of 1-32 lanes");
    if constexpr (N >= 2) v += perm_dpp<DPP_QP_XOR1>(v);
    if constexpr (N >= 4) v += perm_dpp<DPP_QP_XOR2>(v);
    if constexpr (N >= 8) v += perm_dpp<DPP_ROW_HALF_MIRROR>(v);
    if constexpr (N >= 16) v += perm_dpp<DPP_ROW_MIRROR>(v);
    if constexpr (N >= 32) v = row_pair_combine(v, [](uint32_t a, uint32_t b) { return a + b; });
    return v;
}

template <int N>
__device__ __forceinline__ uint32_t group_max(uint32_t v)
{
    static_assert(N == 1 || N == 2 || N == 4 || N == 8 || N == 16 || N == 32, "lane group of 1-32 lanes");
    if constexpr (N >= 2) v = ::max(v, perm_dpp<DPP_QP_XOR1>(v));
    if constexpr (N >= 4) v = ::max(v, perm_dpp<DPP_QP_XOR2>(v));
    if constexpr (N >= 8) v = ::max(v, perm_dpp<DPP_ROW_HALF_MIRROR>(v));
    if constexpr (N >= 16) v = ::max(v, perm_dpp<DPP_ROW_MIRROR>(v));
    if constexpr (N >= 32) v = row_pair_combine(v, [](uint32_t a, uint32_t b) { return ::max(a, b); });
    return v;
}

template <int VL, int DPL>
__device__ __forceinline__ uint32_t sweep_step(const uint32_t (&Lp)[DPL], uint32_t minLp, const uint32_t (&C)[DPL],
                                               uint32_t P1, uint32_t P2, uint32_t (&Ln)[DPL])
{
    const uint32_t lm = Line<VL>::prev(kBig, Lp[DPL - 1]);
    const uint32_t lq = Line<VL>::next(kBig, Lp[0]);
    const uint32_t delta = minLp + P2;
    uint32_t mn = 0xFFFFFFFFu;
#pragma unroll
    for (int i = 0; i < DPL; i++) {
        const uint32_t a1 = i == 0 ? lm : Lp[i - 1];
        const uint32_t a2 = i == DPL - 1 ? lq : Lp[i + 1];
        uint32_t v = min(min(a1, a2) + P1, Lp[i]);
        v = min(v, delta);
        Ln[i] = C[i] + v - minLp;
        mn = min(mn, Ln[i]);
    }
    return group_min<VL>(mn);
}

typedef unsigned short pk16 __attribute__((ext_vector_type(2)));
__device__ __forceinline__ pk16 pkv(uint32_t w) { return __builtin_bit_cast(pk16, w); }
__device__ __forceinline__ uint32_t pkw(pk16 v) { return __builtin_bit_cast(uint32_t, v); }
__device__ __forceinline__ uint32_t pk_min(uint32_t a, uint32_t b) { return pkw(__builtin_elementwise_min(pkv(a), pkv(b))); }
__device__ __forceinline__ uint32_t pk_add(uint32_t a, uint32_t b) { return pkw(pkv(a) + pkv(b)); }
__device__ __forceinline__ uint32_t pk_sub(uint32_t a, uint32_t b) { return pkw(pkv(a) - pkv(b)); }
__device__ __forceinline__ uint32_t pk_adds(uint32_t a, uint32_t b)
{
    return pkw(__builtin_elementwise_add_sat(pkv(a), pkv(b)));
}

__device__ __forceinline__ uint32_t pk_window_push(uint32_t u, uint32_t s)
{
    uint32_t r;
    asm("v_pk_mad_u16 %0, %1, -1, %2 clamp" : "=v"(r) : "v"(u), "v"(s));
    return r;
}

template <int VL, int NP>
__device__ __forceinline__ uint32_t sweep_step_pk(const uint32_t (&Lp)[NP], uint32_t minLp, const uint32_t (&C)[NP],
                                                  uint32_t P1p, uint32_t P2, uint32_t (&Ln)[NP])
{
    constexpr uint32_t EDGE = kBig | (kBig << 16);
    const uint32_t lm = Line<VL>::prev(EDGE, Lp[NP - 1]);
    const uint32_t lq = Line<VL>::next(EDGE, Lp[0]);
    const uint32_t mm = minLp * 0x10001u, dl = (minLp + P2) * 0x10001u;
    uint32_t mn = 0xFFFFFFFFu;
    uint32_t a1 = __builtin_amdgcn_alignbit(Lp[0], lm, 16);
#pragma unroll
    for (int k = 0; k < NP; k++) {
        const uint32_t a2 = __builtin_amdgcn_alignbit(k + 1 < NP ? Lp[k + 1] : lq, Lp[k], 16);
        uint32_t v = pk_min(pk_add(pk_min(a1, a2), P1p), Lp[k]);
        v = pk_min(v, dl);
        Ln[k] = pk_add(C[k], pk_sub(v, mm));
        mn = pk_min(mn, Ln[k]);
        a1 = a2;
    }
    return group_min<VL>(::min(mn & 0xFFFFu, mn >> 16));
}

typedef _Float16 h16x2 __attribute__((ext_vector_type(2)));
__device__ __forceinline__ h16x2 hv(uint32_t w) { return __builtin_bit_cast(h16x2, w); }
__device__ __forceinline__ uint32_t hw(h16x2 v) { return __builtin_bit_cast(uint32_t, v); }
__device__ __forceinline__ uint32_t h2min(uint32_t a, uint32_t b) { return hw(__builtin_elementwise_minimum(hv(a), hv(b))); }
__device__ __forceinline__ uint32_t h2min3(uint32_t a, uint32_t b, uint32_t c)
{
    return hw(__builtin_elementwise_minimum(__builtin_elementwise_minimum(hv(a), hv(b)), hv(c)));
}
__device__ __forceinline__ uint32_t h2add(uint32_t a, uint32_t b) { return hw(hv(a) + hv(b)); }
__device__ __forceinline__ uint32_t h2sub(uint32_t a, uint32_t b) { return hw(hv(a) - hv(b)); }

template <int VL, int NP>
__device__ __forceinline__ uint32_t sweep_step_h16(const uint32_t (&Lp)[NP], uint32_t minLp, const uint32_t (&C)[NP],
                                                   uint32_t P1p, uint32_t P2, uint32_t (&Ln)[NP])
{
    constexpr uint32_t EDGE = 0x7BFF7BFFu;
    const uint32_t lm = Line<VL>::prev(EDGE, Lp[NP - 1]);
    const uint32_t lq = Line<VL>::next(EDGE, Lp[0]);
    const uint32_t mm = minLp * 0x10001u, dl = (minLp + P2) * 0x10001u;
    uint32_t a1 = __builtin_amdgcn_alignbit(Lp[0], lm, 16);
#pragma unroll
    for (int k = 0; k < NP; k++) {
        const uint32_t a2 = __builtin_amdgcn_alignbit(k + 1 < NP ? Lp[k + 1] : lq, Lp[k], 16);
        const uint32_t v = h2min3(h2add(h2min(a1, a2), P1p), Lp[k], dl);
        Ln[k] = h2add(h2sub(v, mm), C[k]);
        a1 = a2;
    }
    uint32_t mn;
    if constexpr (NP == 1) {
        mn = Ln[0];
    } else {
        mn = h2min(Ln[0], Ln[1]);
#pragma unroll
        for (int k = 2; k < NP; k += 2) mn = k + 1 < NP ? h2min3(mn, Ln[k], Ln[k + 1]) : h2min(mn, Ln[k]);
    }
    return group_min<VL>(::min(mn & 0xFFFFu, mn >> 16));
}

template <int VL, int NP, bool H16, bool DS = false>
__device__ __forceinline__ uint32_t sweep_step2(const uint32_t (&Lp)[NP], uint32_t mmp, const uint32_t (&C)[NP],
                                                uint32_t P1p, uint32_t P2p, uint32_t eL, uint32_t eR,
                                                uint32_t (&Ln)[NP])
{
    static_assert(!DS || H16, "deferred subtraction (sweep_step2n): census f16 form only");
    constexpr uint32_t EDGE = H16 ? 0x7BFF7BFFu : (kBig | (kBig << 16));
    uint32_t lm, lq;
    if constexpr (VL == 16) {
        lm = perm_dpp<DPP_ROW_SHR1>(Lp[NP - 1]) | eL;
        lq = perm_dpp<DPP_ROW_SHL1>(Lp[0]) | eR;
    } else if constexpr (VL == 8 || VL == 4) {
        const uint32_t pm = perm_dpp<DPP_ROW_SHR1>(Lp[NP - 1]), pq = perm_dpp<DPP_ROW_SHL1>(Lp[0]);
        lm = eL ? EDGE : pm;
        lq = eR ? EDGE : pq;
    } else if constexpr (VL == 32) {
        const uint32_t pm = perm_dpp<DPP_WAVE_SHR1>(Lp[NP - 1]), pq = perm_dpp<DPP_WAVE_SHL1>(Lp[0]);
        lm = eL ? EDGE : pm;
        lq = eR ? EDGE : pq;
    } else {
        lm = Line<VL>::prev(EDGE, Lp[NP - 1]);
        lq = Line<VL>::next(EDGE, Lp[0]);
    }
    const uint32_t dl = H16 ? h2add(mmp, P2p) : pk_add(mmp, P2p);
    uint32_t a1 = __builtin_amdgcn_alignbit(Lp[0], lm, 16);
#pragma unroll
    for (int k = 0; k < NP; k++) {
        const uint32_t a2 = __builtin_amdgcn_alignbit(k + 1 < NP ? Lp[k + 1] : lq, Lp[k], 16);
        if constexpr (H16) {
            const uint32_t v = h2min3(h2add(h2min(a1, a2), P1p), Lp[k], dl);
            Ln[k] = DS ? h2add(v, C[k]) : h2add(h2sub(v, mmp), C[k]);
        } else {
            uint32_t v = pk_min(pk_add(pk_min(a1, a2), P1p), Lp[k]);
            v = pk_min(v, dl);
            Ln[k] = pk_add(C[k], pk_sub(v, mmp));
        }
        a1 = a2;
    }
    uint32_t mn = Ln[0];
    if constexpr (H16) {
#pragma unroll
        for (int k = 1; k < NP; k += 2) mn = k + 1 < NP ? h2min3(mn, Ln[k], Ln[k + 1]) : h2min(mn, Ln[k]);
        mn = h2min(mn, __builtin_amdgcn_alignbit(mn, mn, 16));
    } else {
#pragma unroll
        for (int k = 1; k < NP; k++) mn = pk_min(mn, Ln[k]);
        mn = pk_min(mn, __builtin_amdgcn_alignbit(mn, mn, 16));
    }
    return group_min<VL>(mn);
}

template <int N, int ND>
__device__ __forceinline__ void group_min_n(uint32_t (&v)[ND])
{
    static_assert(N == 1 || N == 2 || N == 4 || N == 8 || N == 16 || N == 32 || N == 64, "lane group of 1-64 lanes");
    if constexpr (N >= 2) {
#pragma unroll
        for (int n = 0; n < ND; n++) v[n] = ::min(v[n], perm_dpp<DPP_QP_XOR1>(v[n]));
    }
    if constexpr (N >= 4) {
#pragma unroll
        for (int n = 0; n < ND; n++) v[n] = ::min(v[n], perm_dpp<DPP_QP_XOR2>(v[n]));
    }
    if constexpr (N >= 8) {
#pragma unroll
        for (int n = 0; n < ND; n++) v[n] = ::min(v[n], perm_dpp<DPP_ROW_HALF_MIRROR>(v[n]));
    }
    if constexpr (N >= 16) {
#pragma unroll
        for (int n = 0; n < ND; n++) v[n] = ::min(v[n], perm_dpp<DPP_ROW_MIRROR>(v[n]));
    }
    if constexpr (N >= 32) {
#pragma unroll
        for (int n = 0; n < ND; n++) v[n] = row_pair_combine(v[n], [](uint32_t a, uint32_t b) { return ::min(a, b); });
    }
    if constexpr (N >= 64) {
#pragma unroll
        for (int n = 0; n < ND; n++) {
            const auto r = __builtin_amdgcn_permlane32_swap(v[n], v[n], false, false);
            v[n] = ::min((uint32_t)r[0], (uint32_t)r[1]);
        }
    }
}

template <int VL, int NP, bool H16, int ND, bool DS = false>
__device__ __forceinline__ void sweep_step2n(const uint32_t (&Lp)[ND][NP], const uint32_t (&mmp)[ND],
                                             const uint32_t (&C)[ND][NP], uint32_t P1p, uint32_t P2p, uint32_t eL,
                                             uint32_t eR, uint32_t (&Ln)[ND][NP], uint32_t (&mn)[ND])
{
    static_assert(!DS || H16, "deferred subtraction: census f16 form only");
    constexpr uint32_t EDGE = H16 ? 0x7BFF7BFFu : (kBig | (kBig << 16));
    uint32_t lm[ND], lq[ND], dl[ND], a1[ND];
#pragma unroll
    for (int n = 0; n < ND; n++) {
        if constexpr (VL == 16) {
            lm[n] = perm_dpp<DPP_ROW_SHR1>(Lp[n][NP - 1]) | eL;
            lq[n] = perm_dpp<DPP_ROW_SHL1>(Lp[n][0]) | eR;
        } else if constexpr (VL == 8 || VL == 4) {
            const uint32_t pm = perm_dpp<DPP_ROW_SHR1>(Lp[n][NP - 1]), pq = perm_dpp<DPP_ROW_SHL1>(Lp[n][0]);
            lm[n] = eL ? EDGE : pm;
            lq[n] = eR ? EDGE : pq;
        } else if constexpr (VL == 32) {
            const uint32_t pm = perm_dpp<DPP_WAVE_SHR1>(Lp[n][NP - 1]), pq = perm_dpp<DPP_WAVE_SHL1>(Lp[n][0]);
            lm[n] = eL ? EDGE : pm;
            lq[n] = eR ? EDGE : pq;
        } else {
            lm[n] = Line<VL>::prev(EDGE, Lp[n][NP - 1]);
            lq[n] = Line<VL>::next(EDGE, Lp[n][0]);
        }
    }
#pragma unroll
    for (int n = 0; n < ND; n++) {
        dl[n] = H16 ? h2add(mmp[n], P2p) : pk_add(mmp[n], P2p);
        a1[n] = __builtin_amdgcn_alignbit(Lp[n][0], lm[n], 16);
    }
    uint32_t v[ND][NP];
#pragma unroll
    for (int k = 0; k < NP; k++) {
#pragma unroll
        for (int n = 0; n < ND; n++)
            v[n][k] = __builtin_amdgcn_alignbit(k + 1 < NP ? Lp[n][k + 1] : lq[n], Lp[n][k], 16);
    }
#pragma unroll
    for (int k = NP - 1; k >= 0; k--) {
#pragma unroll
        for (int n = 0; n < ND; n++) {
            const uint32_t lo = k == 0 ? a1[n] : v[n][k - 1];
            v[n][k] = H16 ? h2min(lo, v[n][k]) : pk_min(lo, v[n][k]);
        }
    }
    if constexpr (H16) {
#pragma unroll
        for (int k = 0; k < NP; k++)
#pragma unroll
            for (int n = 0; n < ND; n++) v[n][k] = h2add(v[n][k], P1p);
#pragma unroll
        for (int k = 0; k < NP; k++)
#pragma unroll
            for (int n = 0; n < ND; n++) v[n][k] = h2min3(v[n][k], Lp[n][k], dl[n]);
        if constexpr (!DS) {
#pragma unroll
            for (int k = 0; k < NP; k++)
#pragma unroll
                for (int n = 0; n < ND; n++) v[n][k] = h2sub(v[n][k], mmp[n]);
        }
#pragma unroll
        for (int k = 0; k < NP; k++)
#pragma unroll
            for (int n = 0; n < ND; n++) Ln[n][k] = h2add(v[n][k], C[n][k]);
    } else {
#pragma unroll
        for (int k = 0; k < NP; k++)
#pragma unroll
            for (int n = 0; n < ND; n++) v[n][k] = pk_add(v[n][k], P1p);
#pragma unroll
        for (int k = 0; k < NP; k++)
#pragma unroll
            for (int n = 0; n < ND; n++) v[n][k] = pk_min(v[n][k], Lp[n][k]);
#pragma unroll
        for (int k = 0; k < NP; k++)
#pragma unroll
            for (int n = 0; n < ND; n++) v[n][k] = pk_min(v[n][k], dl[n]);
#pragma unroll
        for (int k = 0; k < NP; k++)
#pragma unroll
            for (int n = 0; n < ND; n++) v[n][k] = pk_sub(v[n][k], mmp[n]);
#pragma unroll
        for (int k = 0; k < NP; k++)
#pragma unroll
            for (int n = 0; n < ND; n++) Ln[n][k] = pk_add(C[n][k], v[n][k]);
    }
#pragma unroll
    for (int n = 0; n < ND; n++) mn[n] = Ln[n][0];
    if constexpr (H16) {
#pragma unroll
        for (int k = 1; k < NP; k += 2) {
#pragma unroll
            for (int n = 0; n < ND; n++) mn[n] = k + 1 < NP ? h2min3(mn[n], Ln[n][k], Ln[n][k + 1]) : h2min(mn[n], Ln[n][k]);
        }
#pragma unroll
        for (int n = 0; n < ND; n++) mn[n] = h2min(mn[n], __builtin_amdgcn_alignbit(mn[n], mn[n], 16));
    } else {
#pragma unroll
        for (int k = 1; k < NP; k++) {
#pragma unroll
            for (int n = 0; n < ND; n++) mn[n] = pk_min(mn[n], Ln[n][k]);
        }
#pragma unroll
        for (int n = 0; n < ND; n++) mn[n] = pk_min(mn[n], __builtin_amdgcn_alignbit(mn[n], mn[n], 16));
    }
    group_min_n<VL, ND>(mn);
}

template <typename LT, int NP, int AUX = 0>
__device__ __forceinline__ void store_pk(rsrc_t r, uint32_t off, const uint32_t (&w)[NP])
{
    if constexpr (sizeof(LT) == 2) {
        bstore_n<uint32_t, NP, AUX>(r, off, w);
    } else {
        constexpr int NW = NP / 2;
        if constexpr (NW > 0) {
            uint32_t b[NW];
#pragma unroll
            for (int j = 0; j < NW; j++) b[j] = __builtin_amdgcn_perm(w[2 * j + 1], w[2 * j], 0x06040200u);
            bstore_n<uint32_t, NW, AUX>(r, off, b);
        }
        if constexpr (NP % 2)
            __builtin_amdgcn_raw_buffer_store_b16((uint16_t)((w[NP - 1] & 0xFFu) | ((w[NP - 1] >> 8) & 0xFF00u)), r,
                                                  off + 4 * NW, 0, AUX);
    }
}

template <typename CT, int DPL>
__device__ __forceinline__ void unpack_ct_pk(const RawBytes<DPL * (int)sizeof(CT)>& r, uint32_t (&C)[DPL / 2])
{
#pragma unroll
    for (int k = 0; k < DPL / 2; k++) {
        if constexpr (sizeof(CT) == 2) C[k] = r.w[k];
        else C[k] = __builtin_amdgcn_perm(0u, r.w[k >> 1], (k & 1) ? 0x0c030c02u : 0x0c010c00u);
    }
}

}
```

stereo_match_amd/csrc/sm_sweep.hpp:

```cpp
#pragma once
#include "sm_common.hpp"
#include "sm_sweep_host.hpp"
#include "sm_pk.hpp"

#include <type_traits>

namespace smk {

typedef __attribute__((address_space(1))) unsigned long long gu64;

constexpr uint32_t SW_SPIN_LIMIT = 1u << 19;

#if SWEEP_STATS
#define SW_T0(v) const uint64_t v = __builtin_readcyclecounter()
#define SW_ACC(acc, v) acc += __builtin_readcyclecounter() - v
#else
#define SW_T0(v) (void)0
#define SW_ACC(acc, v) (void)0
#endif

#ifndef SWEEP_STREAM_AUX
#define SWEEP_STREAM_AUX 2
#endif

#ifndef SWEEP_COST_AUX
#define SWEEP_COST_AUX 0
#endif

#ifndef SWEEP_ROW_SYNC
#define SWEEP_ROW_SYNC 1
#endif
#ifndef SWEEP_ROW_SLEEP
#define SWEEP_ROW_SLEEP 1
#endif

#ifndef SWEEP_U32
#define SWEEP_U32 0
#endif
#ifndef SWEEP_H16
#define SWEEP_H16 1
#endif
#ifndef SWEEP_DS
#define SWEEP_DS 1
#endif
#ifndef SWEEP_DS_LINES
#define SWEEP_DS_LINES 1
#endif
#ifndef SWEEP_DS_LANE0
#define SWEEP_DS_LANE0 0
#endif
#define SWEEP_DS_RN 16
static_assert(62 * SWEEP_DS_RN + 62 + 193 + 192 < 2048, "DS renormalisation interval too long for the f16 form");
#ifndef SWEEP_STEPN
#define SWEEP_STEPN 1
#endif
#ifndef SWEEP_LDS_FIRST
#define SWEEP_LDS_FIRST 1
#endif

constexpr int kNarrowNcw = 7;
#ifndef SWEEP_LAT_NCW
#define SWEEP_LAT_NCW 5
#endif
constexpr int kLatNcw = SWEEP_LAT_NCW;
constexpr bool lat_built(int D) { return D % 32 == 0 && D >= 64 && D <= 224; }
#ifndef SWEEP_HM
#define SWEEP_HM 2
#endif
template <int VL, int DPL, int NCW_ = kNarrowNcw>
struct SweepGeo {
    static constexpr int LPW = 64 / VL;
    static constexpr int HM = (DPL % 2 == 0 && !SWEEP_U32 && NCW_ >= 2 + 2 * SWEEP_HM) ? SWEEP_HM : 1;
    static constexpr int NCW = NCW_;
    static constexpr int THREADS = (NCW + 1) * 64;
    static constexpr int HW = HM * LPW;
    static constexpr int HB = HW;
    static constexpr int NCOL = (NCW - 2) * LPW + 2 * HW;
    static constexpr int COLS = NCOL + 2;
    static constexpr int CW = (NCW - 2) * LPW;
    static constexpr int D = VL * DPL;
    static constexpr int NG = (DPL + 1) / 2;
    static constexpr int NDAT = NG * HW * VL;
    static constexpr int SNG = NDAT + HW;
    static constexpr int PF = ((DPL >= 10 && NCW_ >= 11) || VL == 32) ? 2 : 4;
    static_assert(NCW - 2 >= 2 * HM, "the snapshot's own waves of the two sides are distinct");
    static_assert(HB % PF == 0, "the input ring is indexed by the row within a block");
};

constexpr int wide_ncw(int D, int ct_bytes)
{
    if (ct_bytes == 1 && D == 256) return 15;
    if (ct_bytes == 1) return (D <= 96 || D == 128 || D == 160 || D == 192) ? 11 : 0;
    if (D == 16 || D == 32 || D == 96) return 13;
    return (D == 48 || D == 80 || D == 128 || D == 160) ? 11 : 0;
}

#ifndef SWEEP_NLW
#define SWEEP_NLW 4
#endif
#ifndef SWEEP_HALO_POLL
#define SWEEP_HALO_POLL 1
#endif
#ifndef SWEEP_LINE_PRIO
#define SWEEP_LINE_PRIO 2
#endif
#ifndef SWEEP_LPF8
#define SWEEP_LPF8 12
#endif
#ifndef SWEEP_LPF16
#define SWEEP_LPF16 12
#endif
constexpr int largest_divisor_upto(int n, int cap)
{
    for (int p = cap < n ? cap : n; p > 1; p--)
        if (n % p == 0) return p;
    return 1;
}
#ifndef SWEEP_LEAD_BLOCKS
#define SWEEP_LEAD_BLOCKS 1
#endif
#ifndef SWEEP_LINE_NOBAR
#define SWEEP_LINE_NOBAR 1
#endif
#ifndef SWEEP_NOBAR_MODES
#define SWEEP_NOBAR_MODES 21
#endif
constexpr int kMaxLds = 163840;
#ifndef SWEEP_ROWSYNC_M1
#define SWEEP_ROWSYNC_M1 0
#endif
template <int DPL, int MODE>
constexpr bool sweep_nobar()
{
    return SWEEP_ROW_SYNC && (MODE != 1 || SWEEP_ROWSYNC_M1) && DPL % 2 == 0 && !SWEEP_U32 &&
           (MODE == 3 ? SWEEP_LINE_NOBAR != 0 : ((SWEEP_NOBAR_MODES >> MODE) & 1) != 0);
}
template <int DPL, int MODE>
constexpr bool sweep_halo_poll() { return sweep_nobar<DPL, MODE>() && SWEEP_HALO_POLL; }
template <int VL, int DPL, int NCW_, int MODE, int CTB = 1>
struct LineGeo {
    using G = SweepGeo<VL, DPL, NCW_>;
    static constexpr bool ON = MODE == 3;
    static constexpr bool DSO = CTB == 1 && SWEEP_DS && SWEEP_DS_LINES && SWEEP_H16 && VL != 8;
    static constexpr bool HPOLL = sweep_halo_poll<DPL, MODE>();
    static constexpr int POLLER = HPOLL ? 0 : 1;
    static constexpr int NLW = !ON ? 0 : (SWEEP_NLW < 16 - POLLER - NCW_ ? SWEEP_NLW : 16 - POLLER - NCW_);
    static constexpr int RPW = G::LPW / 2;
    static constexpr int BASE = 8 * G::COLS * G::D + 16 * G::COLS + 4 * NCW_ + 4 * 16 + 512 + 4 * G::D;
    static constexpr int ROWB = G::CW * G::D * 2 + (DSO ? G::CW * 8 : 0);
    static constexpr int FIT = (kMaxLds - BASE) / ROWB;
    static constexpr int LEAD0 = SWEEP_LEAD_BLOCKS * G::HB;
    static constexpr int LEAD = LEAD0 + RPW <= FIT ? LEAD0 : (FIT > RPW ? (FIT - RPW) / RPW * RPW : 0);
    static constexpr int LR = SWEEP_LINE_NOBAR ? FIT : LEAD + 2 * RPW <= FIT ? LEAD + 2 * RPW : LEAD + RPW;
    static constexpr bool BUILT = ON && NLW >= 3 && DPL % 2 == 0 && !SWEEP_U32 &&
                                  (SWEEP_LINE_NOBAR ? RPW <= FIT : LEAD + RPW <= FIT) &&
                                  G::CW % 2 == 0 && G::HB % RPW == 0 && RPW >= 1;
    template <typename CT>
    static constexpr int lpf()
    {
        return largest_divisor_upto(G::CW / 2, VL == 8 ? 9 : sizeof(CT) == 1 ? SWEEP_LPF8 : SWEEP_LPF16);
    }
};
template <int VL, int DPL, int NCW_, int MODE>
constexpr int sweep_threads()
{
    using LG = LineGeo<VL, DPL, NCW_, MODE>;
    return SweepGeo<VL, DPL, NCW_>::THREADS + 64 * (LG::NLW - (LG::HPOLL ? 1 : 0));
}

template <int NP>
__device__ __forceinline__ void lds_get_pk(const uint16_t* p, uint32_t (&v)[NP])
{
    if constexpr (NP % 4 == 0) {
#pragma unroll
        for (int k = 0; k < NP / 4; k++) {
            const uint4 q = reinterpret_cast<const uint4*>(p)[k];
            v[4 * k] = q.x; v[4 * k + 1] = q.y; v[4 * k + 2] = q.z; v[4 * k + 3] = q.w;
        }
    } else if constexpr (NP % 2 == 0) {
#pragma unroll
        for (int k = 0; k < NP / 2; k++) {
            const uint2 q = reinterpret_cast<const uint2*>(p)[k];
            v[2 * k] = q.x; v[2 * k + 1] = q.y;
        }
    } else {
#pragma unroll
        for (int k = 0; k < NP; k++) v[k] = reinterpret_cast<const uint32_t*>(p)[k];
    }
}

template <int NP>
__device__ __forceinline__ void lds_put_pk(uint16_t* p, const uint32_t (&v)[NP])
{
    if constexpr (NP % 4 == 0) {
#pragma unroll
        for (int k = 0; k < NP / 4; k++)
            reinterpret_cast<uint4*>(p)[k] = make_uint4(v[4 * k], v[4 * k + 1], v[4 * k + 2], v[4 * k + 3]);
    } else if constexpr (NP % 2 == 0) {
#pragma unroll
        for (int k = 0; k < NP / 2; k++) reinterpret_cast<uint2*>(p)[k] = make_uint2(v[2 * k], v[2 * k + 1]);
    } else {
#pragma unroll
        for (int k = 0; k < NP; k++) reinterpret_cast<uint32_t*>(p)[k] = v[k];
    }
}

template <int DPL>
__device__ __forceinline__ void lds_put(uint16_t* p, const uint32_t (&v)[DPL])
{
    if constexpr (DPL % 2 == 0) {
        uint32_t w[DPL / 2];
#pragma unroll
        for (int k = 0; k < DPL / 2; k++) w[k] = __builtin_amdgcn_perm(v[2 * k + 1], v[2 * k], 0x05040100u);
        if constexpr (DPL % 8 == 0) {
#pragma unroll
            for (int k = 0; k < DPL / 8; k++)
                reinterpret_cast<uint4*>(p)[k] = make_uint4(w[4 * k], w[4 * k + 1], w[4 * k + 2], w[4 * k + 3]);
        } else if constexpr (DPL % 4 == 0) {
#pragma unroll
            for (int k = 0; k < DPL / 4; k++) reinterpret_cast<uint2*>(p)[k] = make_uint2(w[2 * k], w[2 * k + 1]);
        } else {
#pragma unroll
            for (int k = 0; k < DPL / 2; k++) reinterpret_cast<uint32_t*>(p)[k] = w[k];
        }
    } else {
#pragma unroll
        for (int i = 0; i < DPL; i++) p[i] = (uint16_t)v[i];
    }
}

template <int DPL>
__device__ __forceinline__ void lds_get(const uint16_t* p, uint32_t (&v)[DPL])
{
    if constexpr (DPL % 8 == 0) {
#pragma unroll
        for (int k = 0; k < DPL / 8; k++) {
            const uint4 q = reinterpret_cast<const uint4*>(p)[k];
            const uint32_t w[4] = {q.x, q.y, q.z, q.w};
#pragma unroll
            for (int j = 0; j < 4; j++) {
                v[8 * k + 2 * j] = w[j] & 0xFFFFu;
                v[8 * k + 2 * j + 1] = w[j] >> 16;
            }
        }
    } else if constexpr (DPL % 4 == 0) {
#pragma unroll
        for (int k = 0; k < DPL / 4; k++) {
            const uint2 q = reinterpret_cast<const uint2*>(p)[k];
            v[4 * k] = q.x & 0xFFFFu;
            v[4 * k + 1] = q.x >> 16;
            v[4 * k + 2] = q.y & 0xFFFFu;
            v[4 * k + 3] = q.y >> 16;
        }
    } else if constexpr (DPL % 2 == 0) {
#pragma unroll
        for (int k = 0; k < DPL / 2; k++) {
            const uint32_t q = reinterpret_cast<const uint32_t*>(p)[k];
            v[2 * k] = q & 0xFFFFu;
            v[2 * k + 1] = q >> 16;
        }
    } else {
#pragma unroll
        for (int i = 0; i < DPL; i++) v[i] = p[i];
    }
}

template <typename CT, int DPL>
__device__ __forceinline__ void unpack_ct(const RawBytes<DPL * (int)sizeof(CT)>& r, uint32_t (&C)[DPL])
{
#pragma unroll
    for (int i = 0; i < DPL; i++) C[i] = r.template get<CT>(i);
}

__device__ __forceinline__ void lds_barrier()
{
    __builtin_amdgcn_fence(__ATOMIC_RELEASE, "workgroup", "local");
    __builtin_amdgcn_s_barrier();
    __builtin_amdgcn_fence(__ATOMIC_ACQUIRE, "workgroup", "local");
}

#ifndef SWEEP_EARLY_XCHG
#define SWEEP_EARLY_XCHG 1
#endif

template <int N>
__device__ __forceinline__ void poll_set(const gu64* const (&src)[N], const bool (&need)[N], uint32_t tag,
                                         uint32_t (&v)[N], bool& dead, uint32_t* err)
{
    for (uint32_t spins = 0;; spins++) {
        unsigned long long x[N];
#pragma unroll
        for (int k = 0; k < N; k++) x[k] = __hip_atomic_load(src[k], __ATOMIC_RELAXED, __HIP_MEMORY_SCOPE_AGENT);
        bool ok = true;
#pragma unroll
        for (int k = 0; k < N; k++) {
            v[k] = (uint32_t)x[k];
            ok &= !need[k] || (uint32_t)(x[k] >> 32) == tag;
        }
        if (__all(ok) || dead) return;
        if (spins >= SW_SPIN_LIMIT) {
            if ((threadIdx.x & 63) == 0) atomicOr(err, 1u);
            dead = true;
            return;
        }
        __builtin_amdgcn_s_sleep(2);
    }
}

template <int N>
__device__ __forceinline__ void poll_granules(const gu64* src, bool need, uint32_t tag, uint32_t (&v)[N], bool& dead,
                                              uint32_t* err)
{
    const gu64* p[N];
    bool nd[N];
#pragma unroll
    for (int k = 0; k < N; k++) {
        p[k] = src + k;
        nd[k] = need;
    }
    poll_set<N>(p, nd, tag, v, dead, err);
}

template <int VL, int DPL, typename CT, int MODE, int NCW_ = kNarrowNcw>
__global__ void __launch_bounds__((sweep_threads<VL, DPL, NCW_, MODE>())) k_sweep(SweepArgs a)
{
    using G = SweepGeo<VL, DPL, NCW_>;
    using LG = LineGeo<VL, DPL, NCW_, MODE, (int)sizeof(CT)>;
    constexpr bool UP = MODE == 2 || MODE == 4;
    constexpr bool WTA = MODE == 1 || MODE == 2 || MODE == 4;
    constexpr bool EWIN = MODE == 1 || MODE == 2;
    constexpr bool PARTR = MODE == 2 || MODE == 4;
    constexpr bool LINES = MODE == 3;
    constexpr bool HPOLL = LG::HPOLL;
    static_assert(!LINES || LG::BUILT, "MODE 3 instance not built for this geometry");
    static_assert(MODE < 3 || (DPL % 2 == 0 && !SWEEP_U32), "MODES 3 / 4 run the packed row loops only");
    constexpr int NTH = sweep_threads<VL, DPL, NCW_, MODE>();
#ifndef SWEEP_PRIO
#define SWEEP_PRIO 2
#endif
#ifndef SWEEP_DYNPRIO
#define SWEEP_DYNPRIO 1
#endif
    constexpr int PRIO_HI = 3, PRIO_LO = MODE == 0 ? 2 : 1;
    if constexpr (MODE == 0 && SWEEP_PRIO > 0) __builtin_amdgcn_s_setprio(SWEEP_PRIO);
    constexpr bool ROWSYNC = SWEEP_ROW_SYNC && (MODE != 1 || SWEEP_ROWSYNC_M1);
    constexpr bool NOBAR = sweep_nobar<DPL, MODE>();
    static_assert(!LINES || ROWSYNC, "the line waves mirror the row-synchronised barrier pattern");
    constexpr int LPW = G::LPW, NCW = G::NCW, HB = G::HB, NCOL = G::NCOL, COLS = G::COLS, CW = G::CW, D = G::D;
    constexpr int NG = G::NG, SNG = G::SNG, PF = G::PF, HM = G::HM, HW = G::HW;
    constexpr int CB = DPL * (int)sizeof(CT);
    __shared__ __attribute__((aligned(16))) uint16_t lv[2][2][COLS][D];
    __shared__ uint32_t lmin[2][2][COLS];
    __shared__ __attribute__((aligned(16))) uint16_t srow[WTA ? NCW - 2 : 1][WTA ? LPW : 1][WTA ? D : 2];
    __shared__ uint32_t rowcnt[NCW];
    constexpr int RING_D = LINES ? D : 2;
    __shared__ __attribute__((aligned(16))) uint16_t ring_pad[(LINES ? LG::LR : 1) * (LINES ? CW : 1) * RING_D + 2 * RING_D];
    auto& ring = *reinterpret_cast<uint16_t(*)[LINES ? LG::LR : 1][LINES ? CW : 1][RING_D]>(ring_pad + RING_D);
    __shared__ __attribute__((aligned(8))) uint32_t roff[LINES && LG::DSO ? LG::LR : 1][LINES && LG::DSO ? CW : 1][2];
    __shared__ uint32_t linecnt[LINES ? LG::NLW : 1], conscnt[NCW];
    __shared__ uint32_t pollcnt;

    int bx = blockIdx.x, by = blockIdx.y;
    if (a.xcd_per > 0) {
        const int item = (int)(blockIdx.x & 7u) * a.xcd_per + (int)(blockIdx.x >> 3);
        if (item >= a.xcd_total) return;
        const int per_pair = a.nwg * (a.nband > 1 ? a.nband : 1);
        by = item / per_pair;
        bx = item - by * per_pair;
    }
    const int nband = LINES && a.nband > 1 ? a.nband : 1;
    const int band = nband > 1 ? bx / a.nwg : 0;
    const int wg = bx - band * a.nwg, pair = by;
    const int H = a.H, W1 = a.W1;
    const int y0b = nband > 1 ? band * a.band_h : 0;
    const int y1b = nband > 1 ? min(H, y0b + a.band_h) : H;
    const int ys = band > 0 ? max(0, y0b - a.vwarm) : 0;
    const int nrow = y1b - ys, wrows = y0b - ys;
    const int nblk = (nrow + HB - 1) / HB;
    const int nblk_rec = nband > 1 ? a.hop_nblk : nblk;
    const bool vguess = a.vguess && band > 0;
    auto in_domain_slot = [&](int q) { const int x = wg * CW + (q - 1) - HW; return x >= 0 && x < W1; };

    for (int i = threadIdx.x; i < 2 * 2 * COLS * D / 2; i += NTH) {
        uint32_t v = 0;
        if (vguess) {
            const int q = (i / (D / 2)) % COLS, d0 = 2 * (i % (D / 2));
            if (in_domain_slot(q)) v = (uint32_t)(d0 % 5 + 3 * (q & 1)) | ((uint32_t)((d0 + 1) % 5 + 3 * (q & 1)) << 16);
        }
        reinterpret_cast<uint32_t*>(&lv[0][0][0][0])[i] = v;
    }
    for (int i = threadIdx.x; i < 2 * 2 * COLS; i += NTH) {
        const int q = i % COLS;
        (&lmin[0][0][0])[i] = vguess && in_domain_slot(q) ? (uint32_t)(3 * (q & 1)) * 0x10001u : 0u;
    }
    for (int i = threadIdx.x; i < NCW; i += NTH) rowcnt[i] = conscnt[i] = 0;
    if (threadIdx.x == 0) pollcnt = 0;

    if constexpr (LINES)
        for (int i = threadIdx.x; i < LG::NLW; i += NTH) linecnt[i] = 0;
    __syncthreads();

    const int lane = threadIdx.x & 63, wave = threadIdx.x >> 6;
    const bool has_left = wg > 0, has_right = wg + 1 < a.nwg;
    const uint32_t tag0 = a.epoch << 16;
    unsigned long long* hopp = a.hop + (size_t)pair * a.hop_pair;
    auto gbase = [&](int strip, int dir, int b) -> size_t {
        return ((size_t)((band * a.nwg + strip) * 2 + dir) * nblk_rec + b) * SNG;
    };

    if (!HPOLL && wave == NCW) {
        constexpr int NDAT = G::NDAT;
        constexpr int GPL = (2 * SNG + 63) / 64;
        int gdir[GPL], grec[GPL];
        bool gneed[GPL];
#pragma unroll
        for (int k = 0; k < GPL; k++) {
            const int r2 = k * 64 + lane;
            gdir[k] = r2 >= SNG ? 1 : 0;
            grec[k] = r2 - gdir[k] * SNG;
            gneed[k] = r2 < 2 * SNG && (gdir[k] == 0 ? has_left : has_right);
        }
        bool dead = (a.dbg & 1) != 0;
        [[maybe_unused]] uint64_t st_poll = 0, st_bar = 0;
        SW_T0(st_life);
        const bool xchg = (has_left || has_right) && !(a.dbg & 2);
        for (int b = 0; b < nblk; b++) {
            uint32_t v[GPL];
            auto poll = [&]() {
                if (b + 1 < nblk && xchg) {
                    const gu64* src[GPL];
#pragma unroll
                    for (int k = 0; k < GPL; k++)
                        src[k] = (const gu64*)(hopp + gbase(gneed[k] ? wg + (gdir[k] ? 1 : -1) : wg, gdir[k], b) + grec[k]);
                    SW_T0(tp);
                    poll_set<GPL>(src, gneed, tag0 | (uint32_t)(b + 1), v, dead, a.err);
                    SW_ACC(st_poll, tp);
#if SWEEP_STATS
                    if (a.stats && (lane == 0 || lane == 32)) {
                        const int dir = lane == 0 ? 0 : 1;
                        if (dir == 0 ? has_left : has_right)
                            a.stats[1024 + 3 * 65536 + (size_t)MODE * 65536 +
                                    ((size_t)(pair * a.nwg + wg + (dir ? 1 : -1)) * 2 + dir) * nblk + b] =
                                __builtin_amdgcn_s_memrealtime();
                    }
#endif
                }
            };
            if (NOBAR) {
                poll();
                SW_T0(tb);
                const uint32_t need = (uint32_t)((b + 1) * HB);
                for (uint32_t spins = 0; !(a.dbg & 4); spins++) {
                    const uint32_t n0 = __builtin_amdgcn_readfirstlane(
                        __hip_atomic_load(&rowcnt[0], __ATOMIC_RELAXED, __HIP_MEMORY_SCOPE_WORKGROUP));
                    const uint32_t n1 = __builtin_amdgcn_readfirstlane(
                        __hip_atomic_load(&rowcnt[NCW - 1], __ATOMIC_RELAXED, __HIP_MEMORY_SCOPE_WORKGROUP));
                    if (min(n0, n1) >= need) {
                        __builtin_amdgcn_fence(__ATOMIC_ACQUIRE, "workgroup", "local");
                        break;
                    }
                    if (spins >= SW_SPIN_LIMIT) {
                        if (lane == 0) atomicOr(a.err, 1u);
                        break;
                    }
                    __builtin_amdgcn_s_sleep(1);
                }
                SW_ACC(st_bar, tb);
            } else if (ROWSYNC) {
                if (SWEEP_EARLY_XCHG == 2) poll();
                SW_T0(tb);
                if (!(a.dbg & 4)) lds_barrier();
                SW_ACC(st_bar, tb);
            } else {
#pragma unroll 1
                for (int j = 0; j < HB; j++) {
                    if (SWEEP_EARLY_XCHG == 2 && j == HB - 1) poll();
                    if (!(a.dbg & 4)) lds_barrier();
                }
            }
            if (SWEEP_EARLY_XCHG != 2 && !NOBAR) poll();
            if (b + 1 < nblk) {
                if (xchg) {
                    const int wb = (b * HB + HB - 1) & 1;
#pragma unroll
                    for (int k = 0; k < GPL; k++) {
                        if (!gneed[k]) continue;
                        const int r = grec[k], dir = gdir[k];
                        if (r < NDAT) {
                            const int q = r / (HW * VL), pcol = (r / VL) % HW, gg = r % VL;
                            const int col = (dir == 0 ? pcol : NCOL - HW + pcol) + 1;
                            const int d = gg * DPL + 2 * q;
                            if (2 * q + 1 < DPL) *reinterpret_cast<uint32_t*>(&lv[wb][dir][col][d]) = v[k];
                            else lv[wb][dir][col][d] = (uint16_t)v[k];
                        } else {
                            const int pcol = r - NDAT;
                            lmin[wb][dir][(dir == 0 ? pcol : NCOL - HW + pcol) + 1] = v[k];
                        }
                    }
                }
                if (NOBAR) {
                    __builtin_amdgcn_fence(__ATOMIC_RELEASE, "workgroup", "local");
                    __hip_atomic_store(&pollcnt, (uint32_t)(b + 1), __ATOMIC_RELAXED, __HIP_MEMORY_SCOPE_WORKGROUP);
                } else {
                    SW_T0(tb2);
                    lds_barrier();
                    SW_ACC(st_bar, tb2);
                }
            }
        }
#if SWEEP_STATS
        if (a.stats && lane == 0) {
            atomicAdd(a.stats + 8 * MODE + 0, (unsigned long long)st_poll);
            atomicAdd(a.stats + 8 * MODE + 1, (unsigned long long)st_bar);
            atomicAdd(a.stats + 8 * MODE + 6, (unsigned long long)(__builtin_readcyclecounter() - st_life));
            const uint32_t xcc = __builtin_amdgcn_s_getreg((3 << 11) | 20) & 15u;
            const uint32_t lin = blockIdx.x + blockIdx.y * gridDim.x;
            atomicAdd(a.stats + 8 * MODE + 7, (unsigned long long)(xcc == lin % 8 ? 1 : 0) | (1ull << 32));
            if (MODE == 0 && lin < 2048) reinterpret_cast<uint8_t*>(a.stats + 128)[lin] = (uint8_t)(xcc | 0x80);
        }
#endif
        return;
    }

    if constexpr (LINES) {
        if (wave >= NCW + LG::POLLER) {
            constexpr int NLW = LG::NLW, RPW = LG::RPW, LR = LG::LR, LEAD = LG::LEAD;
            constexpr int NP = DPL / 2;
            constexpr int CB = DPL * (int)sizeof(CT);
            constexpr bool H16 = sizeof(CT) == 1 && SWEEP_H16;
            constexpr bool DSL = LG::DSO;
            constexpr uint32_t EDGE2 = H16 ? 0x7BFF7BFFu : (kBig | (kBig << 16));
            constexpr int LPF = LG::template lpf<CT>();
            static_assert(!DSL || LPF <= SWEEP_DS_RN, "DS lines renormalise once per chunk");
            const int li = wave - NCW - LG::POLLER;
            const int kl = lane / VL, g = lane % VL;
            const int dir = kl & 1, r = kl >> 1;
            const int H = a.H, W1 = a.W1, x0 = wg * CW;
            const uint32_t P1p = (uint32_t)a.P1 * 0x10001u, P2p = (uint32_t)a.P2 * 0x10001u;
            const uint32_t eL = g == 0 ? EDGE2 : 0u, eR = g == VL - 1 ? EDGE2 : 0u;
            const uint64_t cells = (uint64_t)H * W1 * D;
            const rsrc_t rc = make_rsrc(a.cost + (size_t)pair * a.cost_pair, cells * sizeof(CT));
            const rsrc_t rs = make_rsrc(a.st + (size_t)pair * a.st_pair, a.st_pair);
            __builtin_amdgcn_s_setprio(SWEEP_LINE_PRIO);
            int bn = 0;
            [[maybe_unused]] uint64_t lst_cons = 0, lst_bar = 0;
            SW_T0(lst_life);
            auto barriers_to = [&](int y0) {
                if constexpr (NOBAR) return;
                while (bn < nblk && (bn + 1) * HB + LEAD <= y0) {
                    SW_T0(tb);
                    if (!(a.dbg & 4)) lds_barrier();
                    if (bn + 1 < nblk) lds_barrier();
                    SW_ACC(lst_bar, tb);
                    bn++;
                }
            };
            auto wait_cons_spin = [&](int need) {
                for (uint32_t spins = 0;; spins++) {
                    uint32_t m = 0xFFFFFFFFu;
#pragma unroll
                    for (int w2 = 1; w2 <= NCW - 2; w2++)
                        m = min(m, __hip_atomic_load(&conscnt[w2], __ATOMIC_RELAXED, __HIP_MEMORY_SCOPE_WORKGROUP));
                    m = __builtin_amdgcn_readfirstlane(m);
                    if (m >= (uint32_t)need) {
                        __builtin_amdgcn_fence(__ATOMIC_ACQUIRE, "workgroup", "local");
                        return;
                    }
                    if (spins >= SW_SPIN_LIMIT) {
                        if (lane == 0) atomicOr(a.err, 1u);
                        return;
                    }
                    __builtin_amdgcn_s_sleep(1);
                }
            };
            auto wait_cons = [&](int need) {
                if (need <= 0) return;
                SW_T0(tc);
                wait_cons_spin(need);
                SW_ACC(lst_cons, tc);
            };
            const int wch = (max(a.ewarm, 1) + LPF - 1) / LPF;
            const int w = wch * LPF, nsteps = w + CW;
            const int c0 = dir ? x0 + CW - 1 + w : x0 - w, cs = dir ? -1 : 1;
            const int jlo = dir ? max(c0 - (W1 - 1), 0) : max(-c0, 0);
            const int jhi = min(nsteps, dir ? c0 + 1 : W1 - c0);
            const int cstep = cs * D * (int)sizeof(CT);
            const int rstep = cs * D;
            for (int t = 0;; t++) {
                const int u0 = (t * NLW + li) * RPW;
                if (u0 >= y1b - y0b) break;
                barriers_to(u0);
                wait_cons(u0 + RPW - LR);
                const int y = y0b + u0 + r;
                const bool yl = y < y1b;
                const uint32_t jspan = yl && jhi > jlo ? (uint32_t)(jhi - jlo) : 0u;
                const uint32_t coff = (((uint32_t)y * (uint32_t)W1 + (uint32_t)c0) * (uint32_t)D + (uint32_t)(g * DPL)) *
                                      (uint32_t)sizeof(CT);
                uint16_t* rp = &ring[(u0 + r) % LR][dir ? CW - 1 : 0][g * DPL];
                uint32_t* rop = &roff[DSL ? (u0 + r) % LR : 0][DSL && dir ? CW - 1 : 0][DSL ? dir : 0];
                const int ostep = cs * 2;
                const uint32_t so = yl ? ((((uint32_t)y * (uint32_t)a.nwg + (uint32_t)wg) * 2u + (uint32_t)dir) * 2u *
                                              (uint32_t)D + (uint32_t)(g * DPL)) * (uint32_t)sizeof(CT)
                                       : kOOB;
                auto coff_at = [&](int j) -> uint32_t {
                    return (uint32_t)(j - jlo) < jspan ? coff + (uint32_t)(j * cstep) : kOOB;
                };
                RawBytes<CB> cr[LPF];
#pragma unroll
                for (int k = 0; k < LPF; k++) {
                    cr[k].load(rc, coff_at(k));
                    asm volatile("" ::: "memory");
                }
                uint32_t Lp[NP], mm = 0, old[NP];
#pragma unroll
                for (int i = 0; i < NP; i++) Lp[i] = old[i] = 0;
                if (a.ewguess && jlo == 0) {
#pragma unroll
                    for (int i = 0; i < NP; i++) {
                        const uint32_t d0 = (uint32_t)(g * DPL + 2 * i);
                        Lp[i] = ((d0 * 7u + (uint32_t)y) % 61u) | ((((d0 + 1u) * 7u + (uint32_t)y) % 61u) << 16);
                    }
                    uint32_t m = Lp[0];
#pragma unroll
                    for (int i = 1; i < NP; i++) m = pk_min(m, Lp[i]);
                    m = min(m & 0xFFFFu, m >> 16);
                    mm = group_min<VL>(m) * 0x10001u;
                }
                auto chunk = [&](int j0, auto ring_c) {
                    constexpr int RING = decltype(ring_c)::value;
#pragma unroll
                    for (int k = 0; k < LPF; k++) {
                        const int j = j0 + k;
#pragma unroll
                        for (int q = 0; q < RawBytes<CB>::WORDS; q++) asm volatile("" : "+v"(cr[k].w[q]) : "v"(mm));
                        uint32_t C[1][NP];
                        unpack_ct_pk<CT, DPL>(cr[k], C[0]);
#pragma unroll
                        for (int i = 0; i < NP; i++) asm volatile("" : "+v"(C[0][i])::"memory");
                        cr[k].load(rc, coff_at(j + LPF));
                        uint32_t Lq[1][NP], mq[1] = {mm}, Ln[1][NP], mn[1];
#pragma unroll
                        for (int i = 0; i < NP; i++) Lq[0][i] = Lp[i];
                        sweep_step2n<VL, NP, H16, 1, DSL>(Lq, mq, C, P1p, P2p, eL, eR, Ln, mn);
#pragma unroll
                        for (int i = 0; i < NP; i++) Lp[i] = Ln[0][i];
                        if constexpr (DSL && RING != 0) {
#if SWEEP_DS_LANE0
                            if (g == 0) rop[(j - w) * ostep] = mq[0];
#else
                            rop[(j - w) * ostep] = mq[0];
#endif
                        }
                        mm = mn[0];
                        if constexpr (RING != 0) {
                            uint16_t* p = rp + (j - w) * rstep;
                            if constexpr (RING == 2) {
                                uint32_t v[NP];
#pragma unroll
                                for (int i = 0; i < NP; i++) v[i] = pk_add(old[i], Lp[i]);
                                lds_put_pk<NP>(p, v);
                                lds_get_pk<NP>(p + rstep, old);
                            } else {
                                lds_put_pk<NP>(p, Lp);
                            }
                        }
                        if constexpr (DSL) {
                            if (k == LPF - 1) {
#pragma unroll
                                for (int i = 0; i < NP; i++) Lp[i] = pk_sub(Lp[i], mm);
                                mm = 0;
                            }
                        }
                    }
                };
                const int half = CW / 2 / LPF;
                auto min0 = [&](uint32_t (&v)[NP]) {
#pragma unroll
                    for (int i = 0; i < NP; i++) v[i] = DSL ? Lp[i] : pk_sub(Lp[i], mm);
                };
                uint32_t sv[NP];
                for (int c = 0; c < wch; c++) chunk(c * LPF, std::integral_constant<int, 0>{});
                min0(sv);
                store_pk<CT, NP>(rs, so, sv);
                for (int c = 0; c < half; c++) chunk(w + c * LPF, std::integral_constant<int, 1>{});
                lds_get_pk<NP>(rp + (CW / 2) * rstep, old);
                for (int c = 0; c < half; c++) chunk(w + (half + c) * LPF, std::integral_constant<int, 2>{});
                min0(sv);
                store_pk<CT, NP>(rs, yl ? so + (uint32_t)(D * sizeof(CT)) : kOOB, sv);
                __builtin_amdgcn_fence(__ATOMIC_RELEASE, "workgroup", "local");
                __hip_atomic_store(&linecnt[li], (uint32_t)(t + 1), __ATOMIC_RELAXED, __HIP_MEMORY_SCOPE_WORKGROUP);
            }
            barriers_to(0x7FFFFFFF);
#if SWEEP_STATS
            if (a.stats && lane == 0) {
                atomicAdd(a.stats + 41, (unsigned long long)lst_cons);
                atomicAdd(a.stats + 42, (unsigned long long)lst_bar);
                atomicAdd(a.stats + 43, (unsigned long long)(__builtin_readcyclecounter() - lst_life));
                atomicAdd(a.stats + 44, 1ull);
            }
#endif
            return;
        }
    }

    const int kl = lane / VL, g = lane % VL;
    const int c = wave == 0 ? kl : wave == NCW - 1 ? NCOL - HW + kl : HW + (wave - 1) * LPW + kl;
    const int x1 = wg * CW + c - HW;
    const bool active = x1 >= 0 && x1 < W1;
    const bool halo_l = wave == 0, halo_r = wave == NCW - 1, own = !halo_l && !halo_r;
    const int wx0 = wg * CW + wave * LPW - LPW;
    const bool wave_ragged = wx0 < 0 || wx0 + LPW > W1;
    const uint32_t P1 = (uint32_t)a.P1, P2 = (uint32_t)a.P2;
    const int wl = wave > 0 ? wave - 1 : wave, wr = wave < NCW - 1 ? wave + 1 : wave;
    bool sync_dead = (a.dbg & 4) != 0;
    auto publish_row = [&](int s) {
        __hip_atomic_store(&rowcnt[wave], (uint32_t)(s + 1), __ATOMIC_RELEASE, __HIP_MEMORY_SCOPE_WORKGROUP);
    };
    [[maybe_unused]] uint64_t st_wait = 0, st_bbar = 0;
    SW_T0(st_clife);
    auto wait_row_spin = [&](int s) {
        for (uint32_t spins = 0;; spins++) {
            const uint32_t nl = __builtin_amdgcn_readfirstlane(
                __hip_atomic_load(&rowcnt[wl], __ATOMIC_RELAXED, __HIP_MEMORY_SCOPE_WORKGROUP));
            const uint32_t nr = __builtin_amdgcn_readfirstlane(
                __hip_atomic_load(&rowcnt[wr], __ATOMIC_RELAXED, __HIP_MEMORY_SCOPE_WORKGROUP));
            if (min(nl, nr) >= (uint32_t)s) {
                __builtin_amdgcn_fence(__ATOMIC_ACQUIRE, "workgroup", "local");
                return;
            }
            if (spins >= SW_SPIN_LIMIT) {
                if (lane == 0) atomicOr(a.err, 1u);
                sync_dead = true;
                return;
            }
            if (SWEEP_ROW_SLEEP) __builtin_amdgcn_s_sleep(SWEEP_ROW_SLEEP);
        }
    };
    auto wait_row = [&](int s) {
        if (sync_dead) return;
        SW_T0(tw);
        wait_row_spin(s);
        SW_ACC(st_wait, tw);
    };
    [[maybe_unused]] uint64_t st_wl = 0;
    auto wait_lines_spin = [&](int s) {
        if constexpr (LINES) {
            const int li = (s / LG::RPW) % LG::NLW;
            const uint32_t need = (uint32_t)(s / (LG::RPW * LG::NLW) + 1);
            for (uint32_t spins = 0;; spins++) {
                const uint32_t nd = __builtin_amdgcn_readfirstlane(
                    __hip_atomic_load(&linecnt[li], __ATOMIC_RELAXED, __HIP_MEMORY_SCOPE_WORKGROUP));
                if (nd >= need) {
                    __builtin_amdgcn_fence(__ATOMIC_ACQUIRE, "workgroup", "local");
                    return;
                }
                if (spins >= SW_SPIN_LIMIT) {
                    if (lane == 0) atomicOr(a.err, 1u);
                    return;
                }
                __builtin_amdgcn_s_sleep(1);
            }
        } else {
            (void)s;
        }
    };
    auto wait_lines = [&](int s) {
        SW_T0(twl);
        wait_lines_spin(s);
        SW_ACC(st_wl, twl);
    };
    auto wait_poll = [&](int b) {
        if constexpr (NOBAR) {
            for (uint32_t spins = 0; !sync_dead; spins++) {
                const uint32_t n = __builtin_amdgcn_readfirstlane(
                    __hip_atomic_load(&pollcnt, __ATOMIC_RELAXED, __HIP_MEMORY_SCOPE_WORKGROUP));
                if (n >= (uint32_t)b) {
                    __builtin_amdgcn_fence(__ATOMIC_ACQUIRE, "workgroup", "local");
                    return;
                }
                if (spins >= SW_SPIN_LIMIT) {
                    if (lane == 0) atomicOr(a.err, 1u);
                    sync_dead = true;
                    return;
                }
                __builtin_amdgcn_s_sleep(1);
            }
        } else {
            (void)b;
        }
    };
    auto end_row = [&](int j, int s) {
        if (!ROWSYNC || j == HB - 1) {
            if (!(a.dbg & 4)) lds_barrier();
        } else {
            publish_row(s);
        }
    };

    const uint64_t cells = (uint64_t)H * W1 * D;
    const rsrc_t rc = make_rsrc(a.cost + (size_t)pair * a.cost_pair, cells * sizeof(CT));
    rsrc_t re = make_rsrc(nullptr, 0), rw = re, rp = re, rrec = re, rnb = re;
    if constexpr (EWIN) {
        re = make_rsrc(a.ew + (size_t)pair * a.ew_pair, cells * sizeof(CT));
        rw = make_rsrc(a.ew + (size_t)pair * a.ew_pair + a.ew_slot, cells * sizeof(CT));
    }
    if constexpr (WTA) {
        rrec = make_rsrc(a.rec + (size_t)pair * H * a.W, (uint64_t)H * a.W * 4);
        rnb = make_rsrc(a.nb + (size_t)pair * H * a.W, (uint64_t)H * a.W * 4);
    }
    const int ku = 100 - a.uniq;
    if constexpr (MODE != 1) rp = make_rsrc((const uint8_t*)a.part + (size_t)pair * a.part_pair, cells * 2);
    const rsrc_t rhop = make_rsrc(hopp, (uint64_t)a.hop_pair * 8);
    constexpr uint32_t NONE = 0xFFFFFFFFu;
    auto cell = [&](int y) -> uint32_t {
        return active ? ((uint32_t)y * (uint32_t)W1 + (uint32_t)x1) * (uint32_t)D + (uint32_t)(g * DPL) : NONE;
    };
    auto boff = [&](uint32_t e, int bytes) -> uint32_t { return e == NONE ? kOOB : e * (uint32_t)bytes; };

    uint32_t LV[DPL];
#pragma unroll
    for (int i = 0; i < DPL; i++) LV[i] = 0;
    uint32_t mV = 0;

    RawBytes<CB> rc_[PF], re_[PF], rw_[PF];
    RawBytes<DPL * 2> rp_[PF];
    auto issue = [&](int k, int s) {
        const uint32_t en = s < H ? cell(UP ? H - 1 - s : s) : NONE;
        const uint32_t eo = own ? en : NONE;
        rc_[k].template load<WTA ? SWEEP_COST_AUX : 0>(rc, boff(en, sizeof(CT)));
        if constexpr (EWIN) {
            re_[k].template load<SWEEP_STREAM_AUX>(re, boff(eo, sizeof(CT)));
            rw_[k].template load<SWEEP_STREAM_AUX>(rw, boff(eo, sizeof(CT)));
        }
        if constexpr (PARTR) rp_[k].template load<SWEEP_STREAM_AUX>(rp, boff(eo, 2));
    };
    if constexpr (DPL % 2 == 0 && !SWEEP_U32) {
        constexpr int NP = DPL / 2;
        const uint32_t P1p = P1 * 0x10001u, P2p = P2 * 0x10001u;
        constexpr uint32_t EDGE2 = (sizeof(CT) == 1 && SWEEP_H16) ? 0x7BFF7BFFu : (kBig | (kBig << 16));
        const uint32_t eL = g == 0 ? EDGE2 : 0u, eR = g == VL - 1 ? EDGE2 : 0u;
        constexpr bool SAT = sizeof(CT) == 2;
        constexpr bool H16 = !SAT && SWEEP_H16;
        constexpr bool DS = H16 && SWEEP_DS;
        static_assert(!DS || SWEEP_STEPN, "deferred subtraction runs the stage-wise steps");
        auto run = [&](auto role_c) {
            constexpr int ROLE = decltype(role_c)::value;
            constexpr bool HAS_A = ROLE != 2, HAS_B = ROLE != 0, OWN = ROLE == 1;
            constexpr int NS = OWN ? 1 : HM;
            auto cell_h = [&](int h, int y) -> uint32_t {
                const int xh = x1 + h * LPW;
                return xh >= 0 && xh < W1 ? ((uint32_t)y * (uint32_t)W1 + (uint32_t)xh) * (uint32_t)D + (uint32_t)(g * DPL)
                                          : NONE;
            };
            RawBytes<CB> rcs[PF][NS];
            auto issue_r = [&](int k, int s) {
                const int yy = UP ? H - 1 - s : ys + s;
#pragma unroll
                for (int h = 0; h < NS; h++)
                    rcs[k][h].template load<WTA ? SWEEP_COST_AUX : 0>(rc, boff(s < nrow ? cell_h(h, yy) : NONE, sizeof(CT)));
                if constexpr (OWN && EWIN) {
                    const uint32_t en = s < nrow ? cell(yy) : NONE;
                    re_[k].template load<SWEEP_STREAM_AUX>(re, boff(en, sizeof(CT)));
                    rw_[k].template load<SWEEP_STREAM_AUX>(rw, boff(en, sizeof(CT)));
                }
                if constexpr (OWN && PARTR) rp_[k].template load<SWEEP_STREAM_AUX>(rp, boff(s < nrow ? cell(yy) : NONE, 2));
            };
#pragma unroll
            for (int k = 0; k < PF; k++) issue_r(k, k);
            uint32_t LVp[NP];
#pragma unroll
            for (int i = 0; i < NP; i++) LVp[i] = 0;
            uint32_t mVl = 0;
            if (vguess && OWN && active) {
                const uint32_t o = (uint32_t)(3 * ((c + 1) & 1));
#pragma unroll
                for (int i = 0; i < NP; i++) {
                    const int d0 = g * DPL + 2 * i;
                    LVp[i] = ((uint32_t)(d0 % 5) + o) | (((uint32_t)((d0 + 1) % 5) + o) << 16);
                }
                mVl = o * 0x10001u;
            }
            auto vstore = [&](int which, const uint32_t (&sV)[NP], uint32_t mV_, const uint32_t (&sA)[NP], uint32_t mA_,
                              const uint32_t (&sB)[NP], uint32_t mB_) {
                if constexpr (LINES && OWN) {
                    const rsrc_t rv = make_rsrc(a.vst + (size_t)pair * a.vst_pair, a.vst_pair);
                    auto off = [&](int dir) -> uint32_t {
                        return active ? (((((uint32_t)band * 2u + (uint32_t)which) * 3u + (uint32_t)dir) * (uint32_t)W1 +
                                          (uint32_t)x1) * (uint32_t)D + (uint32_t)(g * DPL)) * (uint32_t)sizeof(CT)
                                      : kOOB;
                    };
                    uint32_t v[NP];
#pragma unroll
                    for (int i = 0; i < NP; i++) v[i] = pk_sub(sV[i], mV_);
                    store_pk<CT, NP>(rv, off(0), v);
#pragma unroll
                    for (int i = 0; i < NP; i++) v[i] = pk_sub(sA[i], mA_);
                    store_pk<CT, NP>(rv, off(1), v);
#pragma unroll
                    for (int i = 0; i < NP; i++) v[i] = pk_sub(sB[i], mB_);
                    store_pk<CT, NP>(rv, off(2), v);
                }
            };
            uint32_t dpk[NP];
#pragma unroll
            for (int i = 0; i < NP; i++) dpk[i] = (uint32_t)(g * DPL + 2 * i + 1) * 0x10001u + 0x10000u;
            if constexpr (SWEEP_DYNPRIO && !OWN) __builtin_amdgcn_s_setprio(PRIO_HI);
            for (int b = 0; b < nblk; b++) {
#pragma unroll
                for (int j = 0; j < HB; j++) {
                    const int k = j % PF;
                    const int s = b * HB + j;
                    if constexpr (SWEEP_DYNPRIO && OWN) __builtin_amdgcn_s_setprio(PRIO_HI);
                    const bool live = s < nrow;
                    const int y = UP ? H - 1 - s : ys + s;
                    const int rb = (s + 1) & 1, wb = s & 1;
                    const uint32_t e = live ? cell(y) : NONE;
                    uint32_t C[NS][NP], Ein[NP], Win[NP], Pin[NP];
#pragma unroll
                    for (int h = 0; h < NS; h++) unpack_ct_pk<CT, DPL>(rcs[k][h], C[h]);
                    if constexpr (OWN && EWIN) {
                        unpack_ct_pk<CT, DPL>(re_[k], Ein);
                        unpack_ct_pk<CT, DPL>(rw_[k], Win);
                    }
                    if constexpr (OWN && PARTR) unpack_ct_pk<uint16_t, DPL>(rp_[k], Pin);
#pragma unroll
                    for (int i = 0; i < NP; i++) {
#pragma unroll
                        for (int h = 0; h < NS; h++) asm volatile("" : "+v"(C[h][i])::"memory");
                        if constexpr (OWN && EWIN) asm volatile("" : "+v"(Ein[i]), "+v"(Win[i])::"memory");
                        if constexpr (OWN && PARTR) asm volatile("" : "+v"(Pin[i])::"memory");
                    }
                    issue_r(k, s + PF);
                    if (ROWSYNC && (j > 0 || NOBAR)) wait_row(s);
                    uint32_t LA[NS][NP], LB[NS][NP], mA[NS], mB[NS];
#pragma unroll
                    for (int h = 0; h < NS; h++) {
                        const int ch = c + h * LPW;
                        if constexpr (HAS_A) {
                            lds_get_pk<NP>(&lv[rb][0][ch][g * DPL], LA[h]);
                            mA[h] = lmin[rb][0][ch];
                        }
                        if constexpr (HAS_B) {
                            lds_get_pk<NP>(&lv[rb][1][ch + 2][g * DPL], LB[h]);
                            mB[h] = lmin[rb][1][ch + 2];
                        }
                    }
                    if constexpr (SWEEP_LDS_FIRST && MODE == 1) __builtin_amdgcn_sched_barrier(0);
                    uint32_t nV[NP], nA[NS][NP], nB[NS][NP], mnV = 0, mnA[NS], mnB[NS];
                    auto step = [&](const uint32_t(&Lp)[NP], uint32_t m, const uint32_t(&Ch)[NP], uint32_t(&Ln)[NP]) {
                        return sweep_step2<VL, NP, H16, DS>(Lp, m, Ch, P1p, P2p, eL, eR, Ln);
                    };
                    if constexpr (OWN) {
                        if constexpr (SWEEP_STEPN) {
                            uint32_t Lp1[1][NP], m1[1] = {mVl}, C1[1][NP], Ln1[1][NP], mn1[1];
#pragma unroll
                            for (int i = 0; i < NP; i++) {
                                Lp1[0][i] = LVp[i];
                                C1[0][i] = C[0][i];
                            }
                            sweep_step2n<VL, NP, H16, 1, DS>(Lp1, m1, C1, P1p, P2p, eL, eR, Ln1, mn1);
#pragma unroll
                            for (int i = 0; i < NP; i++) nV[i] = Ln1[0][i];
                            mnV = mn1[0];
                        } else {
                            mnV = step(LVp, mVl, C[0], nV);
                        }
                    }
                    if constexpr (SWEEP_STEPN && OWN && NS == 1) {
                        uint32_t Lp2[2][NP], m2[2], C2[2][NP], Ln2[2][NP], mn2[2];
#pragma unroll
                        for (int i = 0; i < NP; i++) {
                            Lp2[0][i] = LA[0][i];
                            Lp2[1][i] = LB[0][i];
                            C2[0][i] = C2[1][i] = C[0][i];
                        }
                        m2[0] = mA[0];
                        m2[1] = mB[0];
                        sweep_step2n<VL, NP, H16, 2, DS>(Lp2, m2, C2, P1p, P2p, eL, eR, Ln2, mn2);
#pragma unroll
                        for (int i = 0; i < NP; i++) {
                            nA[0][i] = Ln2[0][i];
                            nB[0][i] = Ln2[1][i];
                        }
                        mnA[0] = mn2[0];
                        mnB[0] = mn2[1];
                    } else if constexpr (SWEEP_STEPN && !OWN && NS > 1) {
                        uint32_t Lpn[NS][NP], mn_in[NS], Lnn[NS][NP], mnn[NS];
#pragma unroll
                        for (int h = 0; h < NS; h++) {
                            if constexpr (HAS_A) {
#pragma unroll
                                for (int i = 0; i < NP; i++) Lpn[h][i] = LA[h][i];
                                mn_in[h] = mA[h];
                            } else {
#pragma unroll
                                for (int i = 0; i < NP; i++) Lpn[h][i] = LB[h][i];
                                mn_in[h] = mB[h];
                            }
                        }
                        sweep_step2n<VL, NP, H16, NS, DS>(Lpn, mn_in, C, P1p, P2p, eL, eR, Lnn, mnn);
#pragma unroll
                        for (int h = 0; h < NS; h++) {
#pragma unroll
                            for (int i = 0; i < NP; i++) {
                                if constexpr (HAS_A) nA[h][i] = Lnn[h][i];
                                else nB[h][i] = Lnn[h][i];
                            }
                            if constexpr (HAS_A) mnA[h] = mnn[h];
                            else mnB[h] = mnn[h];
                        }
                    } else {
#pragma unroll
                        for (int h = 0; h < NS; h++) {
                            if constexpr (HAS_A) mnA[h] = step(LA[h], mA[h], C[h], nA[h]);
                            if constexpr (HAS_B) mnB[h] = step(LB[h], mB[h], C[h], nB[h]);
                        }
                    }
                    [[maybe_unused]] uint32_t offs = 0;
                    if constexpr (DS) {
                        if constexpr (OWN) offs = pk_add(pk_add(mVl, mA[0]), mB[0]);
                        if (j == HB - 1 || j % SWEEP_DS_RN == SWEEP_DS_RN - 1) {
                            if constexpr (OWN) {
                                offs = pk_sub(offs, pk_add(pk_add(mnV, mnA[0]), mnB[0]));
#pragma unroll
                                for (int i = 0; i < NP; i++) nV[i] = pk_sub(nV[i], mnV);
                                mnV = 0;
                            }
#pragma unroll
                            for (int h = 0; h < NS; h++) {
#pragma unroll
                                for (int i = 0; i < NP; i++) {
                                    if constexpr (HAS_A) nA[h][i] = pk_sub(nA[h][i], mnA[h]);
                                    if constexpr (HAS_B) nB[h][i] = pk_sub(nB[h][i], mnB[h]);
                                }
                                if constexpr (HAS_A) mnA[h] = 0;
                                if constexpr (HAS_B) mnB[h] = 0;
                            }
                        }
                    }
                    if constexpr (LINES && OWN) {
                        if (nband > 1 && (s == wrows - 1 || (s == nrow - 1 && band + 1 < nband)))
                            vstore(s == wrows - 1 ? 0 : 1, nV, mnV, nA[0], mnA[0], nB[0], mnB[0]);
                    }
                    auto snapshot = [&]() {
                        if (j == HB - 1 && b + 1 < nblk) {
                            const bool pa = wave >= NCW - 1 - HM && has_right, pb = wave <= HM && has_left;
                            if (pa || pb) {
                                const uint32_t tag = tag0 | (uint32_t)(b + 1);
                                const int pcol = (pa ? wave - (NCW - 1 - HM) : wave - 1) * LPW + kl;
                                const size_t rec = gbase(wg, pa ? 0 : 1, b);
#pragma unroll
                                for (int q = 0; q < NG; q++)
                                    __builtin_amdgcn_raw_buffer_store_b64(
                                        u32x2{pa ? nA[0][q] : nB[0][q], tag}, rhop,
                                        (uint32_t)((rec + (size_t)(q * HW + pcol) * VL + g) * 8), 0, 16);
                                if (g == 0)
                                    __builtin_amdgcn_raw_buffer_store_b64(u32x2{pa ? mnA[0] : mnB[0], tag}, rhop,
                                                                          (uint32_t)((rec + G::NDAT + pcol) * 8), 0, 16);
#if SWEEP_STATS
                                if (a.stats && lane == 0 && (wave == NCW - 2 || wave == 1))
                                    a.stats[1024 + (size_t)MODE * 65536 +
                                            ((size_t)(pair * a.nwg + wg) * 2 + (pa ? 0 : 1)) * nblk + b] =
                                        __builtin_amdgcn_s_memrealtime();
#endif
                            }
                        }
                    };
                    if constexpr (OWN && SWEEP_EARLY_XCHG) snapshot();
#pragma unroll
                    for (int h = 0; h < NS; h++) {
                        const int ch = c + h * LPW;
                        if constexpr (HAS_A) {
                            lds_put_pk<NP>(&lv[wb][0][ch + 1][g * DPL], nA[h]);
                            if (g == 0) lmin[wb][0][ch + 1] = mnA[h];
                        }
                        if constexpr (HAS_B) {
                            lds_put_pk<NP>(&lv[wb][1][ch + 1][g * DPL], nB[h]);
                            if (g == 0) lmin[wb][1][ch + 1] = mnB[h];
                        }
                    }
                    if constexpr (HPOLL && !OWN) {
                        if (j == HB - 1 && b + 1 < nblk) {
                            constexpr int dirh = HAS_A ? 0 : 1;
                            if ((dirh == 0 ? has_left : has_right) && !(a.dbg & 2)) {
                                constexpr int GH = (SNG + 63) / 64, NDAT = G::NDAT;
                                const gu64* src[GH];
                                bool need[GH];
                                uint32_t v[GH];
#pragma unroll
                                for (int k = 0; k < GH; k++) {
                                    const int r = k * 64 + lane;
                                    need[k] = r < SNG;
                                    src[k] = (const gu64*)(hopp + gbase(wg + (dirh ? 1 : -1), dirh, b) + (need[k] ? r : 0));
                                }
                                SW_T0(tp);
                                poll_set<GH>(src, need, tag0 | (uint32_t)(b + 1), v, sync_dead, a.err);
                                SW_ACC(st_bbar, tp);
#pragma unroll
                                for (int k = 0; k < GH; k++) {
                                    if (!need[k]) continue;
                                    const int r = k * 64 + lane;
                                    if (r < NDAT) {
                                        const int q = r / (HW * VL), pcol = (r / VL) % HW, gg = r % VL;
                                        const int col = (dirh == 0 ? pcol : NCOL - HW + pcol) + 1;
                                        const int d = gg * DPL + 2 * q;
                                        if (2 * q + 1 < DPL) *reinterpret_cast<uint32_t*>(&lv[wb][dirh][col][d]) = v[k];
                                        else lv[wb][dirh][col][d] = (uint16_t)v[k];
                                    } else {
                                        const int pcol = r - NDAT;
                                        lmin[wb][dirh][(dirh == 0 ? pcol : NCOL - HW + pcol) + 1] = v[k];
                                    }
                                }
                            }
                        }
                    }
                    if (!ROWSYNC || (j == HB - 1 && !NOBAR)) {
                        SW_T0(tb);
                        if (!(a.dbg & 4)) lds_barrier();
                        SW_ACC(st_bbar, tb);
                    } else {
                        publish_row(s);
                    }
                    if constexpr (SWEEP_DYNPRIO && OWN) __builtin_amdgcn_s_setprio(PRIO_LO);
                    if constexpr (OWN) {
#pragma unroll
                        for (int i = 0; i < NP; i++) LVp[i] = nV[i];
                        mVl = mnV;
                        if constexpr (!SWEEP_EARLY_XCHG) snapshot();
                        if constexpr (MODE == 0) {
                            uint32_t out[NP];
#pragma unroll
                            for (int i = 0; i < NP; i++) out[i] = pk_add(nV[i], nA[0][i]);
#pragma unroll
                            for (int i = 0; i < NP; i++) out[i] = pk_add(out[i], nB[0][i]);
                            if constexpr (DS) {
#pragma unroll
                                for (int i = 0; i < NP; i++) out[i] = pk_sub(out[i], offs);
                            }
                            bstore_n<uint32_t, NP, SWEEP_STREAM_AUX>(rp, boff(e, 2), out);
                        } else if constexpr (MODE == 3) {
                          const int u = s - wrows;
                          if (u >= 0) {
                            uint32_t out[NP], ewl[NP];
#pragma unroll
                            for (int i = 0; i < NP; i++) out[i] = pk_add(nV[i], nA[0][i]);
#pragma unroll
                            for (int i = 0; i < NP; i++) out[i] = pk_add(out[i], nB[0][i]);
                            if (live) wait_lines(u);
                            lds_get_pk<NP>(&ring[u % LG::LR][(wave - 1) * LPW + kl][g * DPL], ewl);
                            if constexpr (DS && LG::DSO) {
                                const uint2 ro = *reinterpret_cast<const uint2*>(&roff[u % LG::LR][(wave - 1) * LPW + kl][0]);
                                offs = pk_add(offs, pk_add(ro.x, ro.y));
                            }
#pragma unroll
                            for (int i = 0; i < NP; i++) out[i] = SAT ? pk_adds(out[i], ewl[i]) : pk_add(out[i], ewl[i]);
                            if constexpr (DS) {
#pragma unroll
                                for (int i = 0; i < NP; i++) out[i] = pk_sub(out[i], offs);
                            }
                            bstore_n<uint32_t, NP, SWEEP_STREAM_AUX>(rp, boff(e, 2), out);
                            __builtin_amdgcn_fence(__ATOMIC_RELEASE, "workgroup", "local");
                            __hip_atomic_store(&conscnt[wave], (uint32_t)(u + 1), __ATOMIC_RELAXED,
                                               __HIP_MEMORY_SCOPE_WORKGROUP);
                          }
                        } else {
                            uint32_t Sp[NP], ew[NP];
                            const bool pad = SAT && a.Dv < D;
                            if constexpr (SAT) {
                                if constexpr (EWIN) {
#pragma unroll
                                    for (int i = 0; i < NP; i++) ew[i] = pk_adds(Ein[i], Win[i]);
                                    if constexpr (PARTR) {
#pragma unroll
                                        for (int i = 0; i < NP; i++) ew[i] = pk_adds(ew[i], Pin[i]);
                                    }
                                } else {
#pragma unroll
                                    for (int i = 0; i < NP; i++) ew[i] = Pin[i];
                                }
#pragma unroll
                                for (int i = 0; i < NP; i++) Sp[i] = pk_adds(nV[i], nA[0][i]);
#pragma unroll
                                for (int i = 0; i < NP; i++) ew[i] = pk_adds(nB[0][i], ew[i]);
#pragma unroll
                                for (int i = 0; i < NP; i++) Sp[i] = pk_adds(Sp[i], ew[i]);
#pragma unroll
                                for (int i = 0; i < NP; i++) Sp[i] = pk_min(Sp[i], 0x7FFF7FFFu);
                                if (pad) {
#pragma unroll
                                    for (int i = 0; i < NP; i++) {
                                        const int d0 = g * DPL + 2 * i;
                                        Sp[i] |= (d0 >= a.Dv ? 0x0000FFFFu : 0u) | (d0 + 1 >= a.Dv ? 0xFFFF0000u : 0u);
                                    }
                                }
                            } else {
                                if constexpr (EWIN) {
#pragma unroll
                                    for (int i = 0; i < NP; i++) ew[i] = pk_add(Ein[i], Win[i]);
                                    if constexpr (PARTR) {
#pragma unroll
                                        for (int i = 0; i < NP; i++) ew[i] = pk_add(ew[i], Pin[i]);
                                    }
                                } else {
#pragma unroll
                                    for (int i = 0; i < NP; i++) ew[i] = Pin[i];
                                }
#pragma unroll
                                for (int i = 0; i < NP; i++) Sp[i] = pk_add(nV[i], nA[0][i]);
#pragma unroll
                                for (int i = 0; i < NP; i++) ew[i] = pk_add(nB[0][i], ew[i]);
#pragma unroll
                                for (int i = 0; i < NP; i++) Sp[i] = pk_add(Sp[i], ew[i]);
                                if constexpr (DS) {
#pragma unroll
                                    for (int i = 0; i < NP; i++) Sp[i] = pk_sub(Sp[i], offs);
                                }
                            }
                            uint32_t key = 0xFFFFFFFFu;
#pragma unroll
                            for (int i = 0; i < NP; i++)
                                key = min(key, min((Sp[i] << 16) | wta_rank(g * DPL + 2 * i, MODE == 1),
                                                   (Sp[i] & 0xFFFF0000u) | wta_rank(g * DPL + 2 * i + 1, MODE == 1)));
                            asm volatile("" ::: "memory");
                            lds_put_pk<NP>(&srow[(wave - 1) % (NCW - 2)][kl][g * DPL], Sp);
                            asm volatile("" ::: "memory");
                            key = group_min<VL>(key);
                            const uint32_t minS = key >> 16;
                            const int best = wta_unrank(key & 0xFFFF, MODE == 1);
                            const int bm = max(best - 1, 0), bq = min(best + 1, D - 1);
                            const uint32_t Sm = srow[(wave - 1) % (NCW - 2)][kl][bm];
                            const uint32_t Sq = srow[(wave - 1) % (NCW - 2)][kl][bq];
                            const uint32_t bm1p = (uint32_t)best * 0x10001u;
                            uint32_t tw[NP];
#pragma unroll
                            for (int i = 0; i < NP; i++) tw[i] = pk_sub(dpk[i], bm1p);
#pragma unroll
                            for (int i = 0; i < NP; i++) tw[i] = pkw(__builtin_elementwise_sub_sat(pkv(0x00030003u), pkv(tw[i])));
#pragma unroll
                            for (int i = 0; i < NP; i++) tw[i] = pk_window_push(tw[i], Sp[i]);
                            uint32_t m2p = tw[0];
#pragma unroll
                            for (int i = 1; i < NP; i++) m2p = pk_min(m2p, tw[i]);
                            const uint32_t m2 = group_min<VL>(min(m2p & 0xFFFFu, m2p >> 16));
                            const bool ok = !(__mul24((int)m2, ku) < __mul24((int)minS, 100) && (!pad || m2 <= 32767u)) &&
                                            minS < 32767u;
                            const uint32_t recw = ok ? ((minS << 16) | (uint32_t)best) : 0xFFFFFFFFu;
                            const uint32_t nbw = Sm | (Sq << 16);
                            const bool wpx = g == 0 && active && live;
                            const uint32_t px = (uint32_t)y * (uint32_t)a.W + (uint32_t)(x1 + a.minX1);
                            __builtin_amdgcn_raw_buffer_store_b32(recw, rrec, wpx ? px * 4 : kOOB, 0, 0);
                            __builtin_amdgcn_raw_buffer_store_b32(nbw, rnb, wpx ? px * 4 : kOOB, 0, 0);
                        }
                    }
                }
                if (b + 1 < nblk && !HPOLL) {
                    SW_T0(tb);
                    if constexpr (NOBAR) wait_poll(b + 1);
                    else lds_barrier();
                    SW_ACC(st_bbar, tb);
                }
            }
#if SWEEP_STATS
            if (a.stats && lane == 0) {
                atomicAdd(a.stats + 8 * MODE + 2, (unsigned long long)st_wait);
                atomicAdd(a.stats + 8 * MODE + 3, (unsigned long long)st_bbar);
                atomicAdd(a.stats + 8 * MODE + 4, (unsigned long long)(__builtin_readcyclecounter() - st_clife));
                atomicAdd(a.stats + 8 * MODE + 5, 1ull);
                if (LINES) atomicAdd(a.stats + 40, (unsigned long long)st_wl);
            }
#endif
        };
        if (halo_l) run(std::integral_constant<int, 0>{});
        else if (halo_r) run(std::integral_constant<int, 2>{});
        else run(std::integral_constant<int, 1>{});
        return;
    }

#pragma unroll
    for (int k = 0; k < PF; k++) issue(k, k);
    for (int b = 0; b < nblk; b++) {
#pragma unroll
        for (int j = 0; j < HB; j++) {
            const int k = j % PF;
            const int s = b * HB + j;
            const bool live = s < H;
            const int y = UP ? H - 1 - s : s;
            const int rb = (s + 1) & 1, wb = s & 1;
            const uint32_t e = live ? cell(y) : NONE;
            uint32_t C[DPL];
            unpack_ct<CT, DPL>(rc_[k], C);
            uint32_t Ein[DPL], Win[DPL], Pin[DPL];
#pragma unroll
            for (int i = 0; i < DPL; i++) Ein[i] = Win[i] = Pin[i] = 0;
            if constexpr (EWIN) {
                unpack_ct<CT, DPL>(re_[k], Ein);
                unpack_ct<CT, DPL>(rw_[k], Win);
            }
            if constexpr (PARTR) unpack_ct<uint16_t, DPL>(rp_[k], Pin);
#pragma unroll
            for (int i = 0; i < DPL; i++) {
                asm volatile("" : "+v"(C[i])::"memory");
                if constexpr (EWIN) asm volatile("" : "+v"(Ein[i]), "+v"(Win[i])::"memory");
                if constexpr (PARTR) asm volatile("" : "+v"(Pin[i])::"memory");
            }
            issue(k, s + PF);

            if (ROWSYNC && j > 0) wait_row(s);
            uint32_t nA[DPL], nB[DPL];
            uint32_t mnA = 0, mnB = 0;
            if (!halo_r) {
                uint32_t LA[DPL];
                lds_get<DPL>(&lv[rb][0][c][g * DPL], LA);
                mnA = sweep_step<VL, DPL>(LA, lmin[rb][0][c], C, P1, P2, nA);
                if (wave_ragged) {
#pragma unroll
                    for (int i = 0; i < DPL; i++) nA[i] = active ? nA[i] : 0u;
                    mnA = active ? mnA : 0u;
                }
                lds_put<DPL>(&lv[wb][0][c + 1][g * DPL], nA);
                if (g == 0) lmin[wb][0][c + 1] = mnA;
            }
            if (!halo_l) {
                uint32_t LB[DPL];
                lds_get<DPL>(&lv[rb][1][c + 2][g * DPL], LB);
                mnB = sweep_step<VL, DPL>(LB, lmin[rb][1][c + 2], C, P1, P2, nB);
                if (wave_ragged) {
#pragma unroll
                    for (int i = 0; i < DPL; i++) nB[i] = active ? nB[i] : 0u;
                    mnB = active ? mnB : 0u;
                }
                lds_put<DPL>(&lv[wb][1][c + 1][g * DPL], nB);
                if (g == 0) lmin[wb][1][c + 1] = mnB;
            }
            if (j == HB - 1 && b + 1 < nblk) {
                const bool pa = wave == NCW - 2 && has_right, pb = wave == 1 && has_left;
                if (pa || pb) {
                    const uint32_t tag = tag0 | (uint32_t)(b + 1);
                    const size_t rec = gbase(wg, pa ? 0 : 1, b);
#pragma unroll
                    for (int q = 0; q < NG; q++) {
                        const uint32_t lo = pa ? nA[2 * q] : nB[2 * q];
                        const uint32_t hi = 2 * q + 1 < DPL ? (pa ? nA[2 * q + 1] : nB[2 * q + 1]) : 0u;
                        __builtin_amdgcn_raw_buffer_store_b64(u32x2{lo | (hi << 16), tag}, rhop,
                                                              (uint32_t)((rec + (size_t)(q * HW + kl) * VL + g) * 8), 0, 16);
                    }
                    if (g == 0)
                        __builtin_amdgcn_raw_buffer_store_b64(u32x2{pa ? mnA : mnB, tag}, rhop,
                                                              (uint32_t)((rec + G::NDAT + kl) * 8), 0, 16);
                }
            }

            uint32_t out[DPL];
#pragma unroll
            for (int i = 0; i < DPL; i++) out[i] = 0;
            uint32_t recw = 0, nbw = 0;
            bool wpx = false;
            if (own) {
                uint32_t nV[DPL];
                const uint32_t mnV = sweep_step<VL, DPL>(LV, mV, C, P1, P2, nV);
#pragma unroll
                for (int i = 0; i < DPL; i++) LV[i] = nV[i];
                mV = mnV;
                if constexpr (MODE == 0) {
#pragma unroll
                    for (int i = 0; i < DPL; i++) out[i] = nV[i] + nA[i] + nB[i];
                } else {
                    uint32_t S[DPL];
                    uint32_t key = 0xFFFFFFFFu;
                    const bool pad = sizeof(CT) == 2 && a.Dv < D;
#pragma unroll
                    for (int i = 0; i < DPL; i++) {
                        uint32_t t = nV[i] + nA[i] + nB[i] + Ein[i] + Win[i];
                        if constexpr (PARTR) t += Pin[i];
                        if constexpr (sizeof(CT) == 2) t = min(t, 32767u);
                        if (pad && g * DPL + i >= a.Dv) t = 0xFFFFu;
                        S[i] = t;
                        key = min(key, (t << 16) | wta_rank(g * DPL + i, MODE == 1));
                    }
                    asm volatile("" ::: "memory");
                    lds_put<DPL>(&srow[(wave - 1) % (NCW - 2)][kl][g * DPL], S);
                    asm volatile("" ::: "memory");
                    key = group_min<VL>(key);
                    const uint32_t minS = key >> 16;
                    const int best = wta_unrank(key & 0xFFFF, MODE == 1);
                    uint32_t far = 0;
                    const int gb = g * DPL - best + 1;
                    if (ku > 0) {
                        const uint32_t lim = __umul24(minS, 100u);
#pragma unroll
                        for (int i = 0; i < DPL; i++)
                            far = max(far, __umul24(S[i], (uint32_t)ku) < lim && (sizeof(CT) == 1 || S[i] <= 32767u)
                                               ? (uint32_t)(gb + i) : 0u);
                    } else {
#pragma unroll
                        for (int i = 0; i < DPL; i++)
                            far = max(far, (int)S[i] * ku < (int)minS * 100 && (sizeof(CT) == 1 || S[i] <= 32767u)
                                               ? (uint32_t)(gb + i) : 0u);
                    }
                    far = group_max<VL>(far);
                    const bool ok = far <= 2u && minS < 32767u;
                    const int bm = max(best - 1, 0), bq = min(best + 1, D - 1);
                    const uint32_t Sm = srow[(wave - 1) % (NCW - 2)][kl][bm];
                    const uint32_t Sq = srow[(wave - 1) % (NCW - 2)][kl][bq];
                    recw = ok ? ((minS << 16) | (uint32_t)best) : 0xFFFFFFFFu;
                    nbw = Sm | (Sq << 16);
                    wpx = g == 0 && active && live;
                }
            }
            if constexpr (MODE == 0) {
                bstore_n<uint16_t, DPL, SWEEP_STREAM_AUX>(rp, own ? boff(e, 2) : kOOB, out);
            } else {
                const uint32_t px = (uint32_t)y * (uint32_t)a.W + (uint32_t)(x1 + a.minX1);
                __builtin_amdgcn_raw_buffer_store_b32(recw, rrec, wpx ? px * 4 : kOOB, 0, 0);
                __builtin_amdgcn_raw_buffer_store_b32(nbw, rnb, wpx ? px * 4 : kOOB, 0, 0);
            }
            end_row(j, s);
        }
        if (b + 1 < nblk) lds_barrier();
    }
}

#if !defined(SWEEP_MODE) || (SWEEP_MODE == 0 && !SWEEP_WIDE)
__global__ void __launch_bounds__(256) k_lr_rows(const uint32_t* __restrict__ rec, const uint32_t* __restrict__ nbs,
                                                 int16_t* __restrict__ out, int16_t* __restrict__ wta, int H, int W,
                                                 int D, int minD, int minX1, int maxX1, int disp12,
                                                 const uint32_t* guard)
{
    if (guard && __hip_atomic_load(guard, __ATOMIC_RELAXED, __HIP_MEMORY_SCOPE_AGENT) != 0u) return;
    extern __shared__ uint32_t key2[];
    int16_t* drow = reinterpret_cast<int16_t*>(key2 + W);
    const int y = blockIdx.x;
    const size_t row = ((size_t)blockIdx.y * H + y) * W;
    const int INVALID = (minD - 1) * 16;
    for (int X = threadIdx.x; X < W; X += 256) {
        key2[X] = 0xFFFFFFFFu;
        drow[X] = (int16_t)INVALID;
        if (wta && (X < minX1 || X >= maxX1)) wta[row + X] = -1;
    }
    __syncthreads();
    for (int X = minX1 + (int)threadIdx.x; X < maxX1; X += 256) {
        const uint32_t r = rec[row + X];
        if (wta) wta[row + X] = r != 0xFFFFFFFFu ? (int16_t)(r & 0xFFFF) : (int16_t)-1;
        if (r != 0xFFFFFFFFu) {
            const int best = (int)(r & 0xFFFF), minS = (int)(r >> 16);
            atomicMin(&key2[X - best - minD], (r & 0xFFFF0000u) | (uint32_t)(0xFFFF - X));
            int d16 = best * 16;
            if (best > 0 && best < D - 1) {
                const uint32_t nb = nbs[row + X];
                const int Sm = (int)(nb & 0xFFFF), Sq = (int)(nb >> 16);
                d16 += subpix_step(Sm, Sq, minS);
            }
            drow[X] = (int16_t)(d16 + minD * 16);
        }
    }
    __syncthreads();
    for (int X = threadIdx.x; X < W; X += 256) {
        int d1 = drow[X];
        if (X >= minX1 && X < maxX1 && d1 != INVALID) {
            const int _d = d1 >> 4, d_ = (d1 + 15) >> 4;
            const int _x = X - _d, x_ = X - d_;
            bool rej1 = false, rej2 = false;
            if (_x >= 0 && _x < W) {
                const uint32_t kk = key2[_x];
                const int d2 = kk == 0xFFFFFFFFu ? INVALID : (int)(0xFFFF - (kk & 0xFFFF)) - _x;
                rej1 = d2 >= minD && abs(d2 - _d) > disp12;
            }
            if (x_ >= 0 && x_ < W) {
                const uint32_t kk = key2[x_];
                const int d2 = kk == 0xFFFFFFFFu ? INVALID : (int)(0xFFFF - (kk & 0xFFFF)) - x_;
                rej2 = d2 >= minD && abs(d2 - d_) > disp12;
            }
            if (rej1 && rej2) d1 = INVALID;
        }
        out[row + X] = (int16_t)d1;
    }
}
#endif

}
```

stereo_match_amd/csrc/sm_sweep_host.hpp:

```cpp
#pragma once
#include <hip/hip_runtime.h>
#include <stdint.h>

namespace smk {

#ifndef SWEEP_STATS
#define SWEEP_STATS 0
#endif

struct SweepArgs {
    const uint8_t* cost;
    size_t cost_pair;
    const uint8_t* ew;
    size_t ew_pair, ew_slot;
    uint16_t* part;
    size_t part_pair;
    unsigned long long* hop;
    size_t hop_pair;
    uint32_t* rec;
    uint32_t* nb;
    uint32_t* err;
    int H, W, W1, D, minD, minX1, P1, P2, uniq;
    int Dv;
    float inv_ku;
    int nwg;
    uint32_t epoch;
    int dbg;
    unsigned long long* stats;
    uint8_t* st;
    size_t st_pair;
    int ewarm;
    int ewguess;
    int nband, band_h, vwarm;
    int vguess;
    int hop_nblk;
    uint8_t* vst;
    size_t vst_pair;
    int xcd_per, xcd_total;
};


struct SweepInfo {
    int cw;
    int hb;
    int ngr;
    int threads;
    int blocks_per_cu;
    int impl;
    int dpl;
    int ncw;
};

template <typename CT, int MODE, class F>
hipError_t with_d(int D, F& f);

hipError_t sweep_info_m0(int D, int ct_bytes, int variant, int device, SweepInfo* out);
hipError_t sweep_info_m1(int D, int ct_bytes, int variant, int device, SweepInfo* out);
hipError_t sweep_info_m2(int D, int ct_bytes, int variant, int device, SweepInfo* out);
hipError_t sweep_info_m3(int D, int ct_bytes, int variant, int device, SweepInfo* out);
hipError_t sweep_info_m4(int D, int ct_bytes, int variant, int device, SweepInfo* out);
hipError_t sweep_info_wide_m0(int D, int ct_bytes, int device, SweepInfo* out);
hipError_t sweep_info_wide_m1(int D, int ct_bytes, int device, SweepInfo* out);
hipError_t sweep_info_wide_m2(int D, int ct_bytes, int device, SweepInfo* out);
hipError_t sweep_info_wide_m3(int D, int ct_bytes, int device, SweepInfo* out);
hipError_t sweep_info_wide_m4(int D, int ct_bytes, int device, SweepInfo* out);
hipError_t sweep_info_lat_m0(int D, int ct_bytes, int device, SweepInfo* out);
hipError_t sweep_info_lat_m1(int D, int ct_bytes, int device, SweepInfo* out);
hipError_t sweep_info_lat_m2(int D, int ct_bytes, int device, SweepInfo* out);
hipError_t sweep_info_lat_m3(int D, int ct_bytes, int device, SweepInfo* out);
hipError_t sweep_info_lat_m4(int D, int ct_bytes, int device, SweepInfo* out);
hipError_t sweep_launch_lat_m0(int D, int ct_bytes, const SweepArgs& a, int npairs, hipStream_t stream);
hipError_t sweep_launch_lat_m1(int D, int ct_bytes, const SweepArgs& a, int npairs, hipStream_t stream);
hipError_t sweep_launch_lat_m2(int D, int ct_bytes, const SweepArgs& a, int npairs, hipStream_t stream);
hipError_t sweep_launch_lat_m3(int D, int ct_bytes, const SweepArgs& a, int npairs, hipStream_t stream);
hipError_t sweep_launch_lat_m4(int D, int ct_bytes, const SweepArgs& a, int npairs, hipStream_t stream);
hipError_t sweep_launch_m0(int D, int ct_bytes, int variant, const SweepArgs& a, int npairs, hipStream_t stream);
hipError_t sweep_launch_m1(int D, int ct_bytes, int variant, const SweepArgs& a, int npairs, hipStream_t stream);
hipError_t sweep_launch_m2(int D, int ct_bytes, int variant, const SweepArgs& a, int npairs, hipStream_t stream);
hipError_t sweep_launch_m3(int D, int ct_bytes, int variant, const SweepArgs& a, int npairs, hipStream_t stream);
hipError_t sweep_launch_m4(int D, int ct_bytes, int variant, const SweepArgs& a, int npairs, hipStream_t stream);
hipError_t sweep_launch_wide_m0(int D, int ct_bytes, const SweepArgs& a, int npairs, hipStream_t stream);
hipError_t sweep_launch_wide_m1(int D, int ct_bytes, const SweepArgs& a, int npairs, hipStream_t stream);
hipError_t sweep_launch_wide_m2(int D, int ct_bytes, const SweepArgs& a, int npairs, hipStream_t stream);
hipError_t sweep_launch_wide_m3(int D, int ct_bytes, const SweepArgs& a, int npairs, hipStream_t stream);
hipError_t sweep_launch_wide_m4(int D, int ct_bytes, const SweepArgs& a, int npairs, hipStream_t stream);

inline hipError_t sweep_info(int D, int ct_bytes, int mode, int variant, int device, SweepInfo* out)
{
    typedef hipError_t (*InfoW)(int, int, int, SweepInfo*);
    typedef hipError_t (*InfoV)(int, int, int, int, SweepInfo*);
    static const InfoW lat[5] = {sweep_info_lat_m0, sweep_info_lat_m1, sweep_info_lat_m2, sweep_info_lat_m3,
                                 sweep_info_lat_m4};
    static const InfoW wide[5] = {sweep_info_wide_m0, sweep_info_wide_m1, sweep_info_wide_m2, sweep_info_wide_m3,
                                  sweep_info_wide_m4};
    static const InfoV narrow[5] = {sweep_info_m0, sweep_info_m1, sweep_info_m2, sweep_info_m3, sweep_info_m4};
    if (mode < 0 || mode > 4) return hipErrorInvalidValue;
    if (variant == 2) return lat[mode](D, ct_bytes, device, out);
    if (variant == 0) {
        const hipError_t e = wide[mode](D, ct_bytes, device, out);
        if (e == hipSuccess) return e;
    }
    return narrow[mode](D, ct_bytes, variant == 1 ? 0 : variant, device, out);
}
inline hipError_t sweep_launch(int D, int ct_bytes, int mode, int impl, const SweepArgs& a, int npairs,
                               hipStream_t stream)
{
    typedef hipError_t (*LaunchW)(int, int, const SweepArgs&, int, hipStream_t);
    typedef hipError_t (*LaunchV)(int, int, int, const SweepArgs&, int, hipStream_t);
    static const LaunchW lat[5] = {sweep_launch_lat_m0, sweep_launch_lat_m1, sweep_launch_lat_m2, sweep_launch_lat_m3,
                                   sweep_launch_lat_m4};
    static const LaunchW wide[5] = {sweep_launch_wide_m0, sweep_launch_wide_m1, sweep_launch_wide_m2,
                                    sweep_launch_wide_m3, sweep_launch_wide_m4};
    static const LaunchV narrow[5] = {sweep_launch_m0, sweep_launch_m1, sweep_launch_m2, sweep_launch_m3,
                                      sweep_launch_m4};
    if (mode < 0 || mode > 4) return hipErrorInvalidValue;
    if (impl == 2) return lat[mode](D, ct_bytes, a, npairs, stream);
    if (impl == 1) return wide[mode](D, ct_bytes, a, npairs, stream);
    return narrow[mode](D, ct_bytes, impl, a, npairs, stream);
}
hipError_t lr_rows_launch(const uint32_t* rec, const uint32_t* nb, int16_t* out, int16_t* wta, int G, int H, int W,
                          int D, int minD, int minX1, int maxX1, int disp12, const uint32_t* guard, hipStream_t stream);

struct EwArgs {
    const uint8_t* cost;
    size_t cost_pair;
    uint8_t* out;
    size_t out_pair, out_slot;
    int H, W1, P1, P2;
    int nrb;
    int wpb;
    int prio;
};
hipError_t ew_launch(int D, int ct_bytes, int vl, EwArgs a, int npairs, hipStream_t stream);

struct EwPatchArgs {
    const uint8_t* cost;
    size_t cost_pair;
    uint16_t* part;
    size_t part_pair;
    uint8_t* st;
    size_t st_pair;
    int H, W1, nwg, cw, P1, P2;
    const uint32_t* guard;
    unsigned long long* fixes;
    int atom;
};
struct BandPatchArgs {
    const uint8_t* cost;
    size_t cost_pair;
    uint16_t* part;
    size_t part_pair;
    const uint8_t* vst;
    size_t vst_pair;
    int H, W1, nband, band_h, P1, P2;
    int nbx;
    const uint32_t* guard;
    unsigned long long* fixes;
};
hipError_t band_patch_launch(int D, int ct_bytes, const BandPatchArgs& a, int npairs, hipStream_t stream);

constexpr int kPatchMaxChunks = 8;
constexpr int patch_max_strips(int D) { return 1 + kPatchMaxChunks * (D % 32 == 0 ? 4 : 8) * 8; }
hipError_t ew_patch_launch(int D, int ct_bytes, const EwPatchArgs& a, int npairs, hipStream_t stream);

}
```

Measured before the change: 6808.

## Use interleaved disparity packing in SGM sweep registers to cheapen neighbor min

Adds an interleaved register layout for u8 cost volumes: each packed 32-bit word holds disparities k and k+NP instead of 2k and 2k+1. With this layout the d±1 neighbor minimum in the path step uses whole adjacent words instead of per-word alignbit shuffles. Costs are permuted into this layout on load, and results are converted back to plain order on store. When the flag is set, the 8-direction line path also keeps the partial buffer in interleaved form so the E/W patch can skip conversions. This adds byte-permute work at load and store, makes WTA lookup and guess initialisation layout-aware, and disables the carry path in the E/W patch when interleaving is on.

```diff
diff --git a/stereo_match_amd/csrc/sm_api.hip b/stereo_match_amd/csrc/sm_api.hip
--- a/stereo_match_amd/csrc/sm_api.hip
+++ b/stereo_match_amd/csrc/sm_api.hip
@@ -637,6 +637,7 @@
     size_t st_pair = 0;
     int ewarm = 0;
     int ewguess = 0;
+    int part_il = 0;
     int nband = 1, band_h = 0, vwarm = 0, vguess = 0;
     uint8_t* vst = nullptr;
     size_t vst_pair = 0;
@@ -784,6 +785,7 @@
         a.st_pair = j.st_pair;
         a.ewarm = j.ewarm;
         a.ewguess = j.ewguess;
+        a.part_il = j.part_il;
         a.nband = nb;
         a.band_h = j.band_h;
         a.vwarm = j.vwarm;
@@ -1015,6 +1017,8 @@
     j.st = (uint8_t*)bs.st.p;
     j.ewarm = ew_warmup(ctx, n);
     j.ewguess = ctx->tune_ew_guess;
+    j.part_il = SWEEP_IL && n.ndirs == 8 && et == 1 && n.D != 256 && f.si.dpl % 2 == 0 &&
+                f.si.dpl == (n.D % 32 == 0 ? n.D / 16 : n.D / 8) ? 1 : 0;
     if (j.nband > 1 && ctx->tune_ew_warmup <= 0 && et == 2) j.ewarm = 54;
     if (j.nband > 1) {
         j.band_h = (g.H + j.nband - 1) / j.nband;
@@ -1054,6 +1058,7 @@
         pa.guard = gflag;
         pa.fixes = reinterpret_cast<unsigned long long*>((uint32_t*)ctx->sweep_err.p + ERR_EW_REPAIRS);
         pa.atom = EW_PATCH_ATOM && et == 2 && 5 * path_max(n) < 65536 ? 1 : 0;
+        pa.part_il = j.part_il;
         auto ew_patch = [&](hipStream_t st) -> int {
             const hipError_t e = smk::ew_patch_launch(n.D, (int)et, pa, G, st);
             if (e == hipErrorInvalidValue) return fail(ctx, SM_E_UNSUPPORTED, "E/W patch: numDisparities %d not built", n.D);
diff --git a/stereo_match_amd/csrc/sm_ew.hpp b/stereo_match_amd/csrc/sm_ew.hpp
--- a/stereo_match_amd/csrc/sm_ew.hpp
+++ b/stereo_match_amd/csrc/sm_ew.hpp
@@ -131,6 +131,7 @@
     const rsrc_t rs = make_rsrc(a.st + pair * a.st_pair, a.st_pair);
     const uint32_t P1p = (uint32_t)a.P1 * 0x10001u, P2p = (uint32_t)a.P2 * 0x10001u;
     const uint32_t eL = g == 0 ? EDGE : 0u, eR = g == VL - 1 ? EDGE : 0u;
+    const bool pil = !ATOM && a.part_il != 0;
     auto soff = [&](int k, int dir, int which) -> uint32_t {
         return (((((uint32_t)y * (uint32_t)nwg + (uint32_t)k) * 2u + (uint32_t)dir) * 2u + (uint32_t)which) *
                     (uint32_t)D + (uint32_t)(g * DPL)) * (uint32_t)sizeof(CT);
@@ -193,6 +194,12 @@
                 unpack_ct_pk<CT, DPL>(cc[u], C2[0]);
 #pragma unroll
                 for (int q = 0; q < NP; q++) pv_[q] = ATOM ? 0u : pb[u].w[q];
+                if (pil) {
+                    uint32_t t[NP];
+                    pk_to_plain<NP, true>(pv_, t);
+#pragma unroll
+                    for (int q = 0; q < NP; q++) pv_[q] = t[q];
+                }
 #pragma unroll
                 for (int q = 0; q < NP; q++) C2[1][q] = C2[0][q];
                 sweep_step2n<VL, NP, H16, 2>(Lq, mq, C2, P1p, P2p, eL, eR, Ln, mn);
@@ -215,6 +222,12 @@
                     } else {
                         P[q] = pk_add(pk_sub(pv_[q], Ln[0][q]), Ln[1][q]);
                     }
+                }
+                if (pil) {
+                    uint32_t t[NP];
+                    pk_from_plain<NP, true>(P, t);
+#pragma unroll
+                    for (int q = 0; q < NP; q++) P[q] = t[q];
                 }
                 if constexpr (!ATOM) bstore_n<uint32_t, NP>(rp, cell(c) * 2u, P);
 #pragma unroll
@@ -397,7 +410,7 @@
             if (lane == 0) openm[wave][ch] = open;
             if (open && first_open == nwg) first_open = i0 + __builtin_ctzll(open);
         }
-        if (first_open < nwg && !EW_PATCH_NO_CARRY && D % 128 == 0 && EW_PATCH_B64) {
+        if (first_open < nwg && !EW_PATCH_NO_CARRY && D % 128 == 0 && EW_PATCH_B64 && !pil) {
             order_partial();
             bool carry = false;
             uint32_t T[NPW];
diff --git a/stereo_match_amd/csrc/sm_pk.hpp b/stereo_match_amd/csrc/sm_pk.hpp
--- a/stereo_match_amd/csrc/sm_pk.hpp
+++ b/stereo_match_amd/csrc/sm_pk.hpp
@@ -81,6 +81,54 @@
     return pkw(__builtin_elementwise_add_sat(pkv(a), pkv(b)));
 }
 
+template <int NP, bool IL>
+__device__ __forceinline__ constexpr int pk_disp(int k, int h)
+{
+    return IL ? k + h * NP : 2 * k + h;
+}
+template <int NP, bool IL>
+__device__ __forceinline__ constexpr int pk_slot(int r)
+{
+    return IL ? (r < NP ? 2 * r : 2 * (r - NP) + 1) : r;
+}
+__device__ __forceinline__ uint32_t pk_halves(uint32_t lo_src, int lo_half, uint32_t hi_src, int hi_half)
+{
+    return __builtin_amdgcn_perm(hi_src, lo_src, ((hi_half ? 0x0706u : 0x0504u) << 16) | (lo_half ? 0x0302u : 0x0100u));
+}
+template <int NP, bool IL>
+__device__ __forceinline__ void pk_to_plain(const uint32_t (&w)[NP], uint32_t (&o)[NP])
+{
+#pragma unroll
+    for (int j = 0; j < NP; j++) {
+        if constexpr (IL) {
+            const int s0 = pk_slot<NP, true>(2 * j), s1 = pk_slot<NP, true>(2 * j + 1);
+            o[j] = pk_halves(w[s0 >> 1], s0 & 1, w[s1 >> 1], s1 & 1);
+        } else {
+            o[j] = w[j];
+        }
+    }
+}
+template <int NP, bool IL>
+__device__ __forceinline__ void pk_from_plain(const uint32_t (&p)[NP], uint32_t (&w)[NP])
+{
+#pragma unroll
+    for (int k = 0; k < NP; k++) {
+        if constexpr (IL) w[k] = pk_halves(p[k >> 1], k & 1, p[(k + NP) >> 1], (k + NP) & 1);
+        else w[k] = p[k];
+    }
+}
+template <bool H16>
+__device__ __forceinline__ uint32_t pk_min_halves(uint32_t w)
+{
+    if constexpr (H16) {
+        const auto v = __builtin_bit_cast(_Float16 __attribute__((ext_vector_type(2))), w);
+        return __builtin_bit_cast(uint32_t, __builtin_elementwise_minimum(v, __builtin_shufflevector(v, v, 1, 0)));
+    } else {
+        const pk16 v = pkv(w);
+        return pkw(__builtin_elementwise_min(v, __builtin_shufflevector(v, v, 1, 0)));
+    }
+}
+
 __device__ __forceinline__ uint32_t pk_window_push(uint32_t u, uint32_t s)
 {
     uint32_t r;
@@ -148,11 +196,28 @@
     return group_min<VL>(::min(mn & 0xFFFFu, mn >> 16));
 }
 
-template <int VL, int NP, bool H16, bool DS = false>
+template <int VL, int NP, bool H16, int ND, bool DS = false, bool IL = false>
+__device__ __forceinline__ void sweep_step2n(const uint32_t (&Lp)[ND][NP], const uint32_t (&mmp)[ND],
+                                             const uint32_t (&C)[ND][NP], uint32_t P1p, uint32_t P2p, uint32_t eL,
+                                             uint32_t eR, uint32_t (&Ln)[ND][NP], uint32_t (&mn)[ND]);
+
+template <int VL, int NP, bool H16, bool DS = false, bool IL = false>
 __device__ __forceinline__ uint32_t sweep_step2(const uint32_t (&Lp)[NP], uint32_t mmp, const uint32_t (&C)[NP],
                                                 uint32_t P1p, uint32_t P2p, uint32_t eL, uint32_t eR,
                                                 uint32_t (&Ln)[NP])
 {
+    if constexpr (IL) {
+        uint32_t Lp1[1][NP], m1[1] = {mmp}, C1[1][NP], Ln1[1][NP], mn1[1];
+#pragma unroll
+        for (int k = 0; k < NP; k++) {
+            Lp1[0][k] = Lp[k];
+            C1[0][k] = C[k];
+        }
+        sweep_step2n<VL, NP, H16, 1, DS, true>(Lp1, m1, C1, P1p, P2p, eL, eR, Ln1, mn1);
+#pragma unroll
+        for (int k = 0; k < NP; k++) Ln[k] = Ln1[0][k];
+        return mn1[0];
+    }
     static_assert(!DS || H16, "deferred subtraction (sweep_step2n): census f16 form only");
     constexpr uint32_t EDGE = H16 ? 0x7BFF7BFFu : (kBig | (kBig << 16));
     uint32_t lm, lq;
@@ -232,7 +297,7 @@
     }
 }
 
-template <int VL, int NP, bool H16, int ND, bool DS = false>
+template <int VL, int NP, bool H16, int ND, bool DS, bool IL>
 __device__ __forceinline__ void sweep_step2n(const uint32_t (&Lp)[ND][NP], const uint32_t (&mmp)[ND],
                                              const uint32_t (&C)[ND][NP], uint32_t P1p, uint32_t P2p, uint32_t eL,
                                              uint32_t eR, uint32_t (&Ln)[ND][NP], uint32_t (&mn)[ND])
@@ -261,21 +326,35 @@
 #pragma unroll
     for (int n = 0; n < ND; n++) {
         dl[n] = H16 ? h2add(mmp[n], P2p) : pk_add(mmp[n], P2p);
-        a1[n] = __builtin_amdgcn_alignbit(Lp[n][0], lm[n], 16);
+        a1[n] = __builtin_amdgcn_alignbit(Lp[n][IL ? NP - 1 : 0], lm[n], 16);
     }
     uint32_t v[ND][NP];
-#pragma unroll
-    for (int k = 0; k < NP; k++) {
-#pragma unroll
-        for (int n = 0; n < ND; n++)
-            v[n][k] = __builtin_amdgcn_alignbit(k + 1 < NP ? Lp[n][k + 1] : lq[n], Lp[n][k], 16);
-    }
-#pragma unroll
-    for (int k = NP - 1; k >= 0; k--) {
-#pragma unroll
-        for (int n = 0; n < ND; n++) {
-            const uint32_t lo = k == 0 ? a1[n] : v[n][k - 1];
-            v[n][k] = H16 ? h2min(lo, v[n][k]) : pk_min(lo, v[n][k]);
+    if constexpr (IL) {
+        uint32_t a2[ND];
+#pragma unroll
+        for (int n = 0; n < ND; n++) a2[n] = __builtin_amdgcn_alignbit(lq[n], Lp[n][0], 16);
+#pragma unroll
+        for (int k = 0; k < NP; k++) {
+#pragma unroll
+            for (int n = 0; n < ND; n++) {
+                const uint32_t lo = k == 0 ? a1[n] : Lp[n][k - 1], hi = k == NP - 1 ? a2[n] : Lp[n][k + 1];
+                v[n][k] = H16 ? h2min(lo, hi) : pk_min(lo, hi);
+            }
+        }
+    } else {
+#pragma unroll
+        for (int k = 0; k < NP; k++) {
+#pragma unroll
+            for (int n = 0; n < ND; n++)
+                v[n][k] = __builtin_amdgcn_alignbit(k + 1 < NP ? Lp[n][k + 1] : lq[n], Lp[n][k], 16);
+        }
+#pragma unroll
+        for (int k = NP - 1; k >= 0; k--) {
+#pragma unroll
+            for (int n = 0; n < ND; n++) {
+                const uint32_t lo = k == 0 ? a1[n] : v[n][k - 1];
+                v[n][k] = H16 ? h2min(lo, v[n][k]) : pk_min(lo, v[n][k]);
+            }
         }
     }
     if constexpr (H16) {
@@ -328,7 +407,8 @@
             for (int n = 0; n < ND; n++) mn[n] = k + 1 < NP ? h2min3(mn[n], Ln[n][k], Ln[n][k + 1]) : h2min(mn[n], Ln[n][k]);
         }
 #pragma unroll
-        for (int n = 0; n < ND; n++) mn[n] = h2min(mn[n], __builtin_amdgcn_alignbit(mn[n], mn[n], 16));
+        for (int n = 0; n < ND; n++)
+            mn[n] = IL ? pk_min_halves<true>(mn[n]) : h2min(mn[n], __builtin_amdgcn_alignbit(mn[n], mn[n], 16));
     } else {
 #pragma unroll
         for (int k = 1; k < NP; k++) {
@@ -336,7 +416,8 @@
             for (int n = 0; n < ND; n++) mn[n] = pk_min(mn[n], Ln[n][k]);
         }
 #pragma unroll
-        for (int n = 0; n < ND; n++) mn[n] = pk_min(mn[n], __builtin_amdgcn_alignbit(mn[n], mn[n], 16));
+        for (int n = 0; n < ND; n++)
+            mn[n] = IL ? pk_min_halves<false>(mn[n]) : pk_min(mn[n], __builtin_amdgcn_alignbit(mn[n], mn[n], 16));
     }
     group_min_n<VL, ND>(mn);
 }
@@ -370,4 +451,30 @@
     }
 }
 
-}
+template <typename CT, int DPL, bool IL>
+__device__ __forceinline__ void unpack_vol_pk(const RawBytes<DPL * (int)sizeof(CT)>& r, uint32_t (&C)[DPL / 2])
+{
+    constexpr int NP = DPL / 2;
+    if constexpr (!IL) {
+        unpack_ct_pk<CT, DPL>(r, C);
+    } else if constexpr (sizeof(CT) == 2) {
+        uint32_t p[NP];
+        unpack_ct_pk<CT, DPL>(r, p);
+        pk_from_plain<NP, true>(p, C);
+    } else {
+#pragma unroll
+        for (int k = 0; k < NP; k++)
+            C[k] = __builtin_amdgcn_perm(r.w[(k + NP) >> 2], r.w[k >> 2],
+                                         0x0c000c00u | (uint32_t)(k & 3) | ((uint32_t)(4 + ((k + NP) & 3)) << 16));
+    }
+}
+
+template <typename LT, int NP, bool IL, int AUX = 0>
+__device__ __forceinline__ void store_vol_pk(rsrc_t r, uint32_t off, const uint32_t (&w)[NP])
+{
+    uint32_t p[NP];
+    pk_to_plain<NP, IL>(w, p);
+    store_pk<LT, NP, AUX>(r, off, p);
+}
+
+}
diff --git a/stereo_match_amd/csrc/sm_sweep.hpp b/stereo_match_amd/csrc/sm_sweep.hpp
--- a/stereo_match_amd/csrc/sm_sweep.hpp
+++ b/stereo_match_amd/csrc/sm_sweep.hpp
@@ -57,6 +57,11 @@
 #ifndef SWEEP_LDS_FIRST
 #define SWEEP_LDS_FIRST 1
 #endif
+template <typename CT, int DPL>
+constexpr bool sweep_il()
+{
+    return SWEEP_IL && sizeof(CT) == 1 && DPL % 2 == 0 && !SWEEP_U32;
+}
 
 constexpr int kNarrowNcw = 7;
 #ifndef SWEEP_LAT_NCW
@@ -349,6 +354,8 @@
     constexpr int LPW = G::LPW, NCW = G::NCW, HB = G::HB, NCOL = G::NCOL, COLS = G::COLS, CW = G::CW, D = G::D;
     constexpr int NG = G::NG, SNG = G::SNG, PF = G::PF, HM = G::HM, HW = G::HW;
     constexpr int CB = DPL * (int)sizeof(CT);
+    constexpr bool IL = sweep_il<CT, DPL>();
+    constexpr int NPW = DPL / 2 > 0 ? DPL / 2 : 1;
     __shared__ __attribute__((aligned(16))) uint16_t lv[2][2][COLS][D];
     __shared__ uint32_t lmin[2][2][COLS];
     __shared__ __attribute__((aligned(16))) uint16_t srow[WTA ? NCW - 2 : 1][WTA ? LPW : 1][WTA ? D : 2];
@@ -384,8 +391,10 @@
     for (int i = threadIdx.x; i < 2 * 2 * COLS * D / 2; i += NTH) {
         uint32_t v = 0;
         if (vguess) {
-            const int q = (i / (D / 2)) % COLS, d0 = 2 * (i % (D / 2));
-            if (in_domain_slot(q)) v = (uint32_t)(d0 % 5 + 3 * (q & 1)) | ((uint32_t)((d0 + 1) % 5 + 3 * (q & 1)) << 16);
+            const int q = (i / (D / 2)) % COLS, wi = i % (D / 2);
+            const int d0 = IL ? wi / NPW * DPL + pk_disp<NPW, IL>(wi % NPW, 0) : 2 * wi;
+            const int d1 = IL ? wi / NPW * DPL + pk_disp<NPW, IL>(wi % NPW, 1) : 2 * wi + 1;
+            if (in_domain_slot(q)) v = (uint32_t)(d0 % 5 + 3 * (q & 1)) | ((uint32_t)(d1 % 5 + 3 * (q & 1)) << 16);
         }
         reinterpret_cast<uint32_t*>(&lv[0][0][0][0])[i] = v;
     }
@@ -617,8 +626,9 @@
                 if (a.ewguess && jlo == 0) {
 #pragma unroll
                     for (int i = 0; i < NP; i++) {
-                        const uint32_t d0 = (uint32_t)(g * DPL + 2 * i);
-                        Lp[i] = ((d0 * 7u + (uint32_t)y) % 61u) | ((((d0 + 1u) * 7u + (uint32_t)y) % 61u) << 16);
+                        const uint32_t d0 = (uint32_t)(g * DPL + pk_disp<NP, IL>(i, 0));
+                        const uint32_t d1 = (uint32_t)(g * DPL + pk_disp<NP, IL>(i, 1));
+                        Lp[i] = ((d0 * 7u + (uint32_t)y) % 61u) | (((d1 * 7u + (uint32_t)y) % 61u) << 16);
                     }
                     uint32_t m = Lp[0];
 #pragma unroll
@@ -634,14 +644,14 @@
 #pragma unroll
                         for (int q = 0; q < RawBytes<CB>::WORDS; q++) asm volatile("" : "+v"(cr[k].w[q]) : "v"(mm));
                         uint32_t C[1][NP];
-                        unpack_ct_pk<CT, DPL>(cr[k], C[0]);
+                        unpack_vol_pk<CT, DPL, IL>(cr[k], C[0]);
 #pragma unroll
                         for (int i = 0; i < NP; i++) asm volatile("" : "+v"(C[0][i])::"memory");
                         cr[k].load(rc, coff_at(j + LPF));
                         uint32_t Lq[1][NP], mq[1] = {mm}, Ln[1][NP], mn[1];
 #pragma unroll
                         for (int i = 0; i < NP; i++) Lq[0][i] = Lp[i];
-                        sweep_step2n<VL, NP, H16, 1, DSL>(Lq, mq, C, P1p, P2p, eL, eR, Ln, mn);
+                        sweep_step2n<VL, NP, H16, 1, DSL, IL>(Lq, mq, C, P1p, P2p, eL, eR, Ln, mn);
 #pragma unroll
                         for (int i = 0; i < NP; i++) Lp[i] = Ln[0][i];
                         if constexpr (DSL && RING != 0) {
@@ -681,12 +691,12 @@
                 uint32_t sv[NP];
                 for (int c = 0; c < wch; c++) chunk(c * LPF, std::integral_constant<int, 0>{});
                 min0(sv);
-                store_pk<CT, NP>(rs, so, sv);
+                store_vol_pk<CT, NP, IL>(rs, so, sv);
                 for (int c = 0; c < half; c++) chunk(w + c * LPF, std::integral_constant<int, 1>{});
                 lds_get_pk<NP>(rp + (CW / 2) * rstep, old);
                 for (int c = 0; c < half; c++) chunk(w + (half + c) * LPF, std::integral_constant<int, 2>{});
                 min0(sv);
-                store_pk<CT, NP>(rs, yl ? so + (uint32_t)(D * sizeof(CT)) : kOOB, sv);
+                store_vol_pk<CT, NP, IL>(rs, yl ? so + (uint32_t)(D * sizeof(CT)) : kOOB, sv);
                 __builtin_amdgcn_fence(__ATOMIC_RELEASE, "workgroup", "local");
                 __hip_atomic_store(&linecnt[li], (uint32_t)(t + 1), __ATOMIC_RELAXED, __HIP_MEMORY_SCOPE_WORKGROUP);
             }
@@ -842,6 +852,7 @@
         constexpr bool SAT = sizeof(CT) == 2;
         constexpr bool H16 = !SAT && SWEEP_H16;
         constexpr bool DS = H16 && SWEEP_DS;
+        const bool pil = IL && (MODE == 3 || MODE == 4) && a.part_il != 0;
         static_assert(!DS || SWEEP_STEPN, "deferred subtraction runs the stage-wise steps");
         auto run = [&](auto role_c) {
             constexpr int ROLE = decltype(role_c)::value;
@@ -875,8 +886,8 @@
                 const uint32_t o = (uint32_t)(3 * ((c + 1) & 1));
 #pragma unroll
                 for (int i = 0; i < NP; i++) {
-                    const int d0 = g * DPL + 2 * i;
-                    LVp[i] = ((uint32_t)(d0 % 5) + o) | (((uint32_t)((d0 + 1) % 5) + o) << 16);
+                    const int d0 = g * DPL + pk_disp<NP, IL>(i, 0), d1 = g * DPL + pk_disp<NP, IL>(i, 1);
+                    LVp[i] = ((uint32_t)(d0 % 5) + o) | (((uint32_t)(d1 % 5) + o) << 16);
                 }
                 mVl = o * 0x10001u;
             }
@@ -892,18 +903,20 @@
                     uint32_t v[NP];
 #pragma unroll
                     for (int i = 0; i < NP; i++) v[i] = pk_sub(sV[i], mV_);
-                    store_pk<CT, NP>(rv, off(0), v);
+                    store_vol_pk<CT, NP, IL>(rv, off(0), v);
 #pragma unroll
                     for (int i = 0; i < NP; i++) v[i] = pk_sub(sA[i], mA_);
-                    store_pk<CT, NP>(rv, off(1), v);
+                    store_vol_pk<CT, NP, IL>(rv, off(1), v);
 #pragma unroll
                     for (int i = 0; i < NP; i++) v[i] = pk_sub(sB[i], mB_);
-                    store_pk<CT, NP>(rv, off(2), v);
+                    store_vol_pk<CT, NP, IL>(rv, off(2), v);
                 }
             };
             uint32_t dpk[NP];
 #pragma unroll
-            for (int i = 0; i < NP; i++) dpk[i] = (uint32_t)(g * DPL + 2 * i + 1) * 0x10001u + 0x10000u;
+            for (int i = 0; i < NP; i++)
+                dpk[i] = (uint32_t)(g * DPL + pk_disp<NP, IL>(i, 0) + 1) * 0x10001u +
+                         ((uint32_t)(pk_disp<NP, IL>(i, 1) - pk_disp<NP, IL>(i, 0)) << 16);
             if constexpr (SWEEP_DYNPRIO && !OWN) __builtin_amdgcn_s_setprio(PRIO_HI);
             for (int b = 0; b < nblk; b++) {
 #pragma unroll
@@ -917,12 +930,20 @@
                     const uint32_t e = live ? cell(y) : NONE;
                     uint32_t C[NS][NP], Ein[NP], Win[NP], Pin[NP];
 #pragma unroll
-                    for (int h = 0; h < NS; h++) unpack_ct_pk<CT, DPL>(rcs[k][h], C[h]);
+                    for (int h = 0; h < NS; h++) unpack_vol_pk<CT, DPL, IL>(rcs[k][h], C[h]);
                     if constexpr (OWN && EWIN) {
-                        unpack_ct_pk<CT, DPL>(re_[k], Ein);
-                        unpack_ct_pk<CT, DPL>(rw_[k], Win);
-                    }
-                    if constexpr (OWN && PARTR) unpack_ct_pk<uint16_t, DPL>(rp_[k], Pin);
+                        unpack_vol_pk<CT, DPL, IL>(re_[k], Ein);
+                        unpack_vol_pk<CT, DPL, IL>(rw_[k], Win);
+                    }
+                    if constexpr (OWN && PARTR) {
+                        if (pil) {
+#pragma unroll
+                            for (int i = 0; i < NP; i++) Pin[i] = rp_[k].w[i];
+                        } else {
+                            unpack_vol_pk<uint16_t, DPL, IL>(rp_[k], Pin);
+                            if constexpr (IL) asm volatile("");
+                        }
+                    }
 #pragma unroll
                     for (int i = 0; i < NP; i++) {
 #pragma unroll
@@ -948,7 +969,7 @@
                     if constexpr (SWEEP_LDS_FIRST && MODE == 1) __builtin_amdgcn_sched_barrier(0);
                     uint32_t nV[NP], nA[NS][NP], nB[NS][NP], mnV = 0, mnA[NS], mnB[NS];
                     auto step = [&](const uint32_t(&Lp)[NP], uint32_t m, const uint32_t(&Ch)[NP], uint32_t(&Ln)[NP]) {
-                        return sweep_step2<VL, NP, H16, DS>(Lp, m, Ch, P1p, P2p, eL, eR, Ln);
+                        return sweep_step2<VL, NP, H16, DS, IL>(Lp, m, Ch, P1p, P2p, eL, eR, Ln);
                     };
                     if constexpr (OWN) {
                         if constexpr (SWEEP_STEPN) {
@@ -958,7 +979,7 @@
                                 Lp1[0][i] = LVp[i];
                                 C1[0][i] = C[0][i];
                             }
-                            sweep_step2n<VL, NP, H16, 1, DS>(Lp1, m1, C1, P1p, P2p, eL, eR, Ln1, mn1);
+                            sweep_step2n<VL, NP, H16, 1, DS, IL>(Lp1, m1, C1, P1p, P2p, eL, eR, Ln1, mn1);
 #pragma unroll
                             for (int i = 0; i < NP; i++) nV[i] = Ln1[0][i];
                             mnV = mn1[0];
@@ -976,7 +997,7 @@
                         }
                         m2[0] = mA[0];
                         m2[1] = mB[0];
-                        sweep_step2n<VL, NP, H16, 2, DS>(Lp2, m2, C2, P1p, P2p, eL, eR, Ln2, mn2);
+                        sweep_step2n<VL, NP, H16, 2, DS, IL>(Lp2, m2, C2, P1p, P2p, eL, eR, Ln2, mn2);
 #pragma unroll
                         for (int i = 0; i < NP; i++) {
                             nA[0][i] = Ln2[0][i];
@@ -998,7 +1019,7 @@
                                 mn_in[h] = mB[h];
                             }
                         }
-                        sweep_step2n<VL, NP, H16, NS, DS>(Lpn, mn_in, C, P1p, P2p, eL, eR, Lnn, mnn);
+                        sweep_step2n<VL, NP, H16, NS, DS, IL>(Lpn, mn_in, C, P1p, P2p, eL, eR, Lnn, mnn);
 #pragma unroll
                         for (int h = 0; h < NS; h++) {
 #pragma unroll
@@ -1137,7 +1158,7 @@
 #pragma unroll
                                 for (int i = 0; i < NP; i++) out[i] = pk_sub(out[i], offs);
                             }
-                            bstore_n<uint32_t, NP, SWEEP_STREAM_AUX>(rp, boff(e, 2), out);
+                            store_vol_pk<uint16_t, NP, IL, SWEEP_STREAM_AUX>(rp, boff(e, 2), out);
                         } else if constexpr (MODE == 3) {
                           const int u = s - wrows;
                           if (u >= 0) {
@@ -1157,6 +1178,13 @@
                             if constexpr (DS) {
 #pragma unroll
                                 for (int i = 0; i < NP; i++) out[i] = pk_sub(out[i], offs);
+                            }
+                            if (!pil) {
+                                if constexpr (IL) asm volatile("");
+                                uint32_t pl[NP];
+                                pk_to_plain<NP, IL>(out, pl);
+#pragma unroll
+                                for (int i = 0; i < NP; i++) out[i] = pl[i];
                             }
                             bstore_n<uint32_t, NP, SWEEP_STREAM_AUX>(rp, boff(e, 2), out);
                             __builtin_amdgcn_fence(__ATOMIC_RELEASE, "workgroup", "local");
@@ -1189,8 +1217,9 @@
                                 if (pad) {
 #pragma unroll
                                     for (int i = 0; i < NP; i++) {
-                                        const int d0 = g * DPL + 2 * i;
-                                        Sp[i] |= (d0 >= a.Dv ? 0x0000FFFFu : 0u) | (d0 + 1 >= a.Dv ? 0xFFFF0000u : 0u);
+                                        const int d0 = g * DPL + pk_disp<NP, IL>(i, 0);
+                                        constexpr int dh = IL ? NP : 1;
+                                        Sp[i] |= (d0 >= a.Dv ? 0x0000FFFFu : 0u) | (d0 + dh >= a.Dv ? 0xFFFF0000u : 0u);
                                     }
                                 }
                             } else {
@@ -1219,15 +1248,25 @@
                             uint32_t key = 0xFFFFFFFFu;
 #pragma unroll
                             for (int i = 0; i < NP; i++)
-                                key = min(key, min((Sp[i] << 16) | wta_rank(g * DPL + 2 * i, MODE == 1),
-                                                   (Sp[i] & 0xFFFF0000u) | wta_rank(g * DPL + 2 * i + 1, MODE == 1)));
+                                key = min(key, min((Sp[i] << 16) | wta_rank(g * DPL + pk_disp<NP, IL>(i, 0), MODE == 1),
+                                                   (Sp[i] & 0xFFFF0000u) | wta_rank(g * DPL + pk_disp<NP, IL>(i, 1), MODE == 1)));
                             asm volatile("" ::: "memory");
                             lds_put_pk<NP>(&srow[(wave - 1) % (NCW - 2)][kl][g * DPL], Sp);
                             asm volatile("" ::: "memory");
                             key = group_min<VL>(key);
                             const uint32_t minS = key >> 16;
                             const int best = wta_unrank(key & 0xFFFF, MODE == 1);
-                            const int bm = max(best - 1, 0), bq = min(best + 1, D - 1);
+                            auto srow_at = [&](int d) -> int {
+                                if constexpr (!IL) return d;
+                                else if constexpr ((DPL & (DPL - 1)) == 0 && NP > 1) {
+                                    uint32_t hb, ro, r;
+                                    asm("v_bfe_u32 %0, %1, %2, 1" : "=v"(hb) : "v"(d), "n"(__builtin_ctz(NP)));
+                                    asm("v_lshl_or_b32 %0, %1, 1, %2" : "=v"(ro) : "v"(d), "v"(hb));
+                                    asm("v_bfi_b32 %0, %1, %2, %3" : "=v"(r) : "n"(DPL - 1), "v"(ro), "v"(d));
+                                    return (int)r;
+                                } else return d / DPL * DPL + pk_slot<NP, IL>(d % DPL);
+                            };
+                            const int bm = srow_at(max(best - 1, 0)), bq = srow_at(min(best + 1, D - 1));
                             const uint32_t Sm = srow[(wave - 1) % (NCW - 2)][kl][bm];
                             const uint32_t Sq = srow[(wave - 1) % (NCW - 2)][kl][bq];
                             const uint32_t bm1p = (uint32_t)best * 0x10001u;
diff --git a/stereo_match_amd/csrc/sm_sweep_host.hpp b/stereo_match_amd/csrc/sm_sweep_host.hpp
--- a/stereo_match_amd/csrc/sm_sweep_host.hpp
+++ b/stereo_match_amd/csrc/sm_sweep_host.hpp
@@ -6,6 +6,10 @@
 
 #ifndef SWEEP_STATS
 #define SWEEP_STATS 0
+#endif
+
+#ifndef SWEEP_IL
+#define SWEEP_IL 1
 #endif
 
 struct SweepArgs {
@@ -37,6 +41,7 @@
     uint8_t* vst;
     size_t vst_pair;
     int xcd_per, xcd_total;
+    int part_il;
 };
 
 
@@ -144,6 +149,7 @@
     const uint32_t* guard;
     unsigned long long* fixes;
     int atom;
+    int part_il;
 };
 struct BandPatchArgs {
     const uint8_t* cost;
```

New measurement: 6931, median of 6. 1.02x the previous value.
